# QuanjianSong/UniVST

Measured on AMD Instinct MI355X. Metric: stylized frames/sec, SD-v1.5 16x512x512 @50 DDIM steps, higher is better.
Workload: dtype f16; 1 GPU; sd15_unet_three_branch_pnp_transfer_16x512x512_50ddim; frames=16, branches=3, schedule_steps=53 (wrapping modulo 50), masks=moving disc, blended on steps 0..45, parallelism=single, weights=random-init SD-v1.5 architecture (859M + 201M temporal params), fp16

## Files before the change

### include/univst.h

```cpp
#ifndef UNIVST_H
#define UNIVST_H
#include <stdint.h>
#ifdef __cplusplus
extern "C" {
#endif

#define UNIVST_OK 0
#define UNIVST_ERR_ARG (-1)
#define UNIVST_ERR_HIP (-2)
#define UNIVST_ERR_UNSUPPORTED (-3)
#define UNIVST_ERR_STATE (-4)

#define UNIVST_F16 0
#define UNIVST_F32 1

const char* univst_last_error(void);
#define UNIVST_ABI_VERSION 3
int univst_abi_version(void);

typedef struct univst_unet univst_unet;

typedef struct {
    int in_channels, out_channels;
    int block_out_channels[4];
// ... 27 lines not shown
                                     int64_t off_recv_first, int64_t nbytes);
int univst_unet_set_comm(univst_unet* h, int rank, int world, void* comm_ws, int64_t comm_ws_bytes,
                         univst_allreduce_fn ar, univst_kv_exchange_fn kv, void* user);

typedef struct univst_comm univst_comm;
int univst_comm_create(int rank, int world, int64_t ws_bytes, univst_comm** out);
int univst_comm_handle_bytes(void);
int univst_comm_export(univst_comm* c, void* handle_out);
int univst_comm_connect(univst_comm* c, const void* handles);
int univst_comm_connect_local(univst_comm* c, univst_comm* const* all);
int univst_comm_connect_emulated(univst_comm* c, double link_gbps, double latency_us);
int univst_comm_query(univst_comm* c, const char* name, double* out);
int univst_comm_destroy(univst_comm* c);
int univst_comm_allreduce_f32(univst_comm* c, void* buf, int n, void* stream);
int univst_comm_status(univst_comm* c);
int univst_unet_set_comm_native(univst_unet* h, univst_comm* comm);

int univst_unet_set_option(univst_unet* h, const char* name, int value);
int univst_unet_query(univst_unet* h, const char* name, double* out);

typedef struct univst_vae univst_vae;
typedef struct {
    int in_channels, out_channels, latent_channels;
    int block_out_channels[4];
    int layers_per_block;
    int norm_num_groups;
} univst_vae_cfg;
int univst_vae_create(const univst_vae_cfg* cfg, univst_vae** out);
int univst_vae_destroy(univst_vae* h);
int univst_vae_load_tensor(univst_vae* h, const char* key, const void* dev_ptr, int dtype, const int64_t* shape, int ndim, void* stream);
int univst_vae_finalize(univst_vae* h, void* stream);
int univst_vae_decode(univst_vae* h, const void* z, int64_t imgs, int num_frames, int lat_h, int lat_w, void* out, void* stream);
int univst_vae_encode(univst_vae* h, const void* x, int64_t imgs, int H, int W, void* moments, void* stream);

typedef struct univst_klvae univst_klvae;
typedef struct {
    int in_channels, out_channels, latent_channels;
    int block_out_channels[4];
    int layers_per_block;
    int norm_num_groups;
    int use_quant_conv, use_post_quant_conv;
    int64_t attn_score_bytes, pass_bytes;
} univst_klvae_cfg;
int univst_klvae_create(const univst_klvae_cfg* cfg, univst_klvae** out);
int univst_klvae_destroy(univst_klvae* h);
int univst_klvae_load_tensor(univst_klvae* h, const char* key, const void* dev_ptr, int dtype, const int64_t* shape, int ndim, void* stream);
int univst_klvae_finalize(univst_klvae* h, void* stream);
int univst_klvae_decode(univst_klvae* h, const void* z, int64_t imgs, int lat_h, int lat_w, void* out, void* stream);
int univst_klvae_encode(univst_klvae* h, const void* x, int64_t imgs, int H, int W, void* moments, void* stream);
int univst_klvae_query(univst_klvae* h, const char* name, double* out);

typedef struct univst_raft univst_raft;
int univst_raft_create(univst_raft** out);
int univst_raft_destroy(univst_raft* h);
int univst_raft_load_tensor(univst_raft* h, const char* key, const void* dev_ptr, int dtype, const int64_t* shape, int ndim, void* stream);
int univst_raft_forward(univst_raft* h, const uint8_t* img1, const uint8_t* img2, int H, int W, float* flow, void* stream);
int univst_raft_encode(univst_raft* h, const uint8_t* img1, const uint8_t* img2, int H, int W, void* fmap, float* hidden, void* context, void* stream);
int univst_raft_gru(univst_raft* h, float* hidden, const void* context, const void* motion, int fh, int fw, void* stream);
int64_t univst_raft_pyramid_floats(int fh, int fw);
int univst_raft_corr_pyramid(const void* fmap1, const void* fmap2, int fh, int fw, float* pyramid, void* stream);
int univst_raft_corr_lookup(const float* pyramid, const float* coords, int fh, int fw, float* out_f32, void* out_f16, void* stream);
int univst_raft_convex_upsample(const float* flow, const void* mask, int fh, int fw, float* out, void* stream);

typedef struct univst_clip univst_clip;
typedef struct {
    int vocab_size;
    int hidden_size;
    int intermediate_size;
    int num_layers;
    int num_heads;
    int max_positions;
    int hidden_act;
    float layer_norm_eps;
    int projection_dim;
    int eos_token_id;
} univst_clip_cfg;
int univst_clip_create(const univst_clip_cfg* cfg, univst_clip** out);
int univst_clip_destroy(univst_clip* h);
int univst_clip_load_tensor(univst_clip* h, const char* key, const void* dev_ptr, int dtype, const int64_t* shape, int ndim, void* stream);
int univst_clip_finalize(univst_clip* h, void* stream);
int univst_clip_encode(univst_clip* h, const int64_t* ids, int B, int S, void* last_hidden, void* hidden_states, void* pooled, void* stream);
int univst_clip_query(univst_clip* h, const char* name, double* out);
int univst_clip_attention(const void* qkv, int B, int S, int heads, void* out, void* stream);

typedef struct univst_t5 univst_t5;
typedef struct {
    int vocab_size;
    int d_model;
    int d_ff;
    int num_layers;
    int num_heads;
    int d_kv;
    int num_buckets;
    int max_distance;
    float layer_norm_eps;
} univst_t5_cfg;
int univst_t5_create(const univst_t5_cfg* cfg, univst_t5** out);
int univst_t5_destroy(univst_t5* h);
int univst_t5_load_tensor(univst_t5* h, const char* key, const void* dev_ptr, int dtype, const int64_t* shape, int ndim, void* stream);
int univst_t5_finalize(univst_t5* h, void* stream);
int univst_t5_encode(univst_t5* h, const int64_t* ids, int B, int S, void* last_hidden, void* stream);
int univst_t5_query(univst_t5* h, const char* name, double* out);
int univst_t5_attention(const void* qkv, const float* bias_table, int B, int S, int heads, void* out, void* stream);
int univst_debug_t5_buckets(int num_buckets, int max_distance, int n, int* out);

typedef struct univst_motion univst_motion;
typedef struct {
    int channels;
    int num_heads;
    int num_blocks;
    int attn_per_block;
    int norm_groups;
    int max_len;
    int position_encoding;
    float gn_eps;
    float ln_eps;
} univst_motion_cfg;
int univst_motion_create(const univst_motion_cfg* cfg, univst_motion** out);
int univst_motion_destroy(univst_motion* h);
int univst_motion_load_tensor(univst_motion* h, const char* key, const void* dev_ptr, int dtype, const int64_t* shape, int ndim, void* stream);
int univst_motion_finalize(univst_motion* h, void* stream);
int univst_motion_forward(univst_motion* h, const void* X, void* Y, int B, int F, int N, void* stream);
int univst_motion_query(univst_motion* h, const char* name, double* out);
int univst_temporal_attention(const void* qkv, int64_t ldx, const void* pe_qkv, int B, int F, int N, int heads, int head_dim, void* out, int64_t ldo,
                              void* stream);

int univst_linear(const void* X, int64_t ldx, const void* W, const void* bias, const void* residual, int64_t ldr,
                  void* Y, int64_t ldy, int M, int N, int K, int geglu, void* stream);
int univst_geglu_xres_permute(const void* in, void* out, int rows, int cols, void* stream);
int univst_linear_gated(const void* X, int64_t ldx, const void* W, const void* bias, const void* residual, int64_t ldr, void* Y, int64_t ldy,
                        int M, int N, int K, int act, const void* gate, int64_t ld_gate, int rows_per_gate, void* stream);
int univst_linear_ln(const void* X, int64_t ldx, const void* W, const void* bias, const void* residual, int64_t ldr,
                     void* Y, int64_t ldy, int M, int N, int K, int geglu, const float* ln_stats, float ln_eps,
                     const float* ln_wsum, const float* ln_bias, float* stats_out, void* stream);
int64_t univst_attn2_fused_workspace_bytes(int B, int heads, int head_dim);
int univst_attn2_fused(const void* X, int64_t ldx, const float* ln_stats, float ln_eps, const float* ln_wsum, const float* ln_bias,
                       const void* Wq_frag, int q_prescaled, const void* kv, int B, int T, int64_t rows_per_branch, const void* Wo_frag,
                       const void* bias_o, const void* residual, int64_t ldr, void* Y, int64_t ldy, int64_t M, int C, int heads,
                       float* stats_out, void* workspace, void* stream);
int univst_attn12_fused(const void* attn_out, int64_t ldx, const void* Wp_frag, const void* bias_p, const void* residual_in, int64_t ldr_in, float ln_eps,
                        const float* ln_wsum, const float* ln_bias, const void* Wq_frag, int q_prescaled, const void* kv, int B, int T,
                        int64_t rows_per_branch, const void* Wo_frag, const void* bias_o, void* Y, int64_t ldy, int64_t M, int C, int heads,
                        float* stats_out, void* workspace, void* stream);
int univst_frag_pack(const void* W, void* out, int N, int K, void* stream);
int univst_conv_nhwc(const void* X1, const void* X2, int C1, int C2, int imgs, int Hs, int Ws, int upsample, int stride,
                     int taps, const void* W, const void* bias, const void* rowbias, int rows_per_rowbias,
                     const void* residual, void* Y, int Cout, void* stream);
int univst_conv_nhwc_tapinner(const void* X1, const void* X2, int C1, int C2, int imgs, int Hs, int Ws, int upsample, int stride,
                              const void* W, const void* bias, const void* rowbias, int rows_per_rowbias,
                              const void* residual, void* Y, int Cout, void* stream);
int univst_conv3x3_patch(const void* X1, const void* X2, int C1, int C2, int imgs, int Hs, int Ws, int upsample, const void* W32,
                         const void* bias, const void* rowbias, int rows_per_rowbias, const void* residual, void* Y, int Cout,
                         void* stream);
int univst_groupnorm_fold_linear(const void* X, int C, int64_t rows, int rows_per_stat, int groups, float eps, const void* gamma, const void* beta,
                                 const void* W, const void* bias, int N, void* W_sets, float* bias32, void* workspace, void* stream);
int univst_linear_sets(const void* X, int64_t ldx, const void* W_sets, const float* bias32, int rows_per_set, const void* residual, int64_t ldr,
                       void* Y, int64_t ldy, int M, int N, int K, float* stats_out, void* stream);
int64_t univst_groupnorm_workspace_bytes(int64_t rows, int rows_per_stat, int groups);
int univst_groupnorm_nhwc(const void* X1, const void* X2, int C1, int C2, int64_t rows, int rows_per_stat, int groups,
                          float eps, const void* gamma, const void* beta, int silu, void* Y, void* workspace,
                          void* stream);
int univst_layernorm(const void* X, void* Y, const void* gamma, const void* beta, int64_t rows, int C, float eps,
                     void* stream);
int univst_attention(const void* q, int64_t ldq, const void* k, const void* v, int64_t ldkv, void* out, int64_t ldo,
                     const int32_t* src_idx, const int32_t* src_cnt, const float* src_logw, int nsrc, int BF, int Nq, int Nkv,
                     int heads, int head_dim, int q_prescaled, void* stream);
int univst_attention_phase(const void* q, int64_t ldq, const void* k, const void* v, int64_t ldkv, void* out, int64_t ldo,
                           const int32_t* src_idx, const int32_t* src_cnt, const float* src_logw, int nsrc, int BF, int Nq, int Nkv,
                           int heads, int head_dim, int q_prescaled, float* state_out, const float* state_in, void* stream);
typedef struct {
    const void *to_q, *to_q_bias, *to_k, *to_k_bias, *to_v, *to_v_bias;
    const void *norm_q, *norm_k;
    const void *add_q, *add_q_bias, *add_k, *add_k_bias, *add_v, *add_v_bias;
    const void *norm_added_q, *norm_added_k;
    const void *to_out, *to_out_bias, *to_add_out, *to_add_out_bias;
} univst_sd3_attn_weights;
typedef struct {
    const void *res_img, *gate_img, *res_txt, *gate_txt;
    int64_t ld_gate_img, ld_gate_txt;
} univst_sd3_gated_residual;
int univst_sd3_shift_window(int idx, double eta1, double eta2, int* active, float* beta);
int univst_sd3_joint_attention(const univst_sd3_attn_weights* w, const void* hidden, const void* enc, int B, int N, int Nt, int Cin,
                               int heads, int head_dim, int clip_length, int shift, float beta, float rms_eps,
                               void* out_img, void* out_txt, const univst_sd3_gated_residual* gated_residual ,
                               univst_comm* comm , void* stream);
int univst_sd3_adain_shift(void* qkv, int64_t ld, int F, int N, int C, int heads, float alpha, float beta, float gamma, void* ws,
                           void* stream);
int univst_rmsnorm_heads(void* x, int64_t ld, int64_t rows, int heads, int head_dim, const void* weight, float eps, void* stream);
int univst_adaln_modulate(const void* x, void* y, const void* scale, const void* shift, int64_t ld_mod, int64_t rows, int64_t rows_per_batch,
                          int C, float eps, void* y2, const void* scale2, const void* shift2, void* stream);
int univst_gate_residual(const void* x, const void* gate, int64_t ld_gate, const void* y, void* out, int64_t rows, int64_t rows_per_batch, int C,
                         void* stream);
#define UNIVST_ACT_SILU 0
#define UNIVST_ACT_GELU_TANH 1
#define UNIVST_ACT_NONE (-1)
int univst_activation(const void* x, void* out, int64_t n, int act, void* stream);
int univst_timestep_embedding(const float* t, void* out, int B, int dim, int flip_sin_to_cos, float downscale_freq_shift, float max_period,
                              void* stream);
int univst_sd3_patchify(const void* latents, void* rows, int B, int C, int H, int W, int patch, void* stream);
int univst_sd3_unpatchify(const void* rows, void* latents, int B, int C, int H, int W, int patch, void* stream);
int univst_axpbypcz(const void* x, const void* y, const void* z, void* out, float a, float b, float c, int64_t n, void* stream);

int univst_attention_adain_shift(void* qkv, int64_t ld, int F, int N, int C, float alpha, float beta, float gamma,
                                 void* stats_ws, void* stream);
int univst_latent_adain(const void* cnt, const void* sty, void* out, int C, int F, int HW, void* stream);
int univst_latent_adain_stats(const void* cnt, float* stats2c, int C, int F, int HW, void* stream);
int univst_latent_adain_apply(const void* cnt, const void* sty, const float* stats2c, int64_t n_total, void* out, int C,
                              int F, int HW, void* stream);
int univst_axpby(const void* x, const void* eps, void* out, float cx, float ce, int64_t n, void* stream);
int univst_mask_blend(const void* a, const void* b, const void* m, void* out, int C, int64_t FHW, void* stream);
int univst_mask_resize(const uint8_t* mask, void* out, int F, int H, int W, int h, int w, void* stream);

int64_t univst_maskprop_workspace_bytes(int hw, int Nsrc, int C);
int univst_maskprop_frame(const float* feat_tar, const float* feat_src, const float* segs_src, float* segs_tar, int hw,
                          int Nsrc, int C, int ncls, float temperature, int topk, void* workspace, void* stream);
int univst_maskprop_finalize(const float* segs, uint8_t* mask_out, int ncls, int h, int w, int H, int W, void* workspace,
                             void* stream);

int univst_warp_accumulate(const uint8_t* key, const uint8_t* now, const float* fwd, const float* bwd, float* acc, int H,
                           int W, float threshold, void* stream);
int univst_warp_window_key(uint8_t* frames, const float* const* flows, int nn, int F, int H, int W, int key, int r, float threshold,
                           void* stream);
int univst_latent_window_smooth(void* x0, const float* lflow, int C, int F, int h, int w, int r, float thr, void* stream);
int univst_accumulate_u8(const uint8_t* frame, float* acc, int64_t n, void* stream);
int univst_window_store(const float* acc, float weight, uint8_t* dst, int64_t n, void* stream);

#define UNIVST_PROFILE_CLASSES 13
int univst_profile_enable(int on);
int univst_profile_collect(double* ms, int64_t* count, double* flops, double* bytes, int nclasses);
int univst_profile_collect_aux(double* aux_bytes, int nclasses);
int univst_profile_symbols(int cls, char* buf, int n);

int univst_debug_tr16(float* out256, void* stream);
int univst_debug_delay_us(double us, void* stream);

#define UNIVST_PLAN_BIAS 1
#define UNIVST_PLAN_RESIDUAL 2
#define UNIVST_PLAN_ROWBIAS 4
#define UNIVST_PLAN_LN_STATS 8
#define UNIVST_PLAN_STATS_OUT 16
#define UNIVST_PLAN_ACT 32
#define UNIVST_PLAN_GATE 64
#define UNIVST_PLAN_W32_ONLY 128
#define UNIVST_PLAN_W32 256
#define UNIVST_PLAN_GN_OUT 512
#define UNIVST_PLAN_TAPINNER 1024
#define UNIVST_PLAN_Y_UNALIGNED 2048
#define UNIVST_PLAN_WORKSPACE 4096
#define UNIVST_PLAN_GEOM_3X3 0
#define UNIVST_PLAN_GEOM_PAD_END 1
#define UNIVST_PLAN_GEOM_FRAME 2
int univst_debug_gemm_plan(int ncu, int mode, int M, int N, int K, int geglu, int flags, int rows_per_set, int C1, int C2, int Hs, int Ws, int upsample,
                           int stride, int taps, int geom, char* buf, int n);
#define UNIVST_PLAN_SRC_LOGW 1
#define UNIVST_PLAN_EXTRA_KEYS 2
int univst_debug_attention_plan(int BF, int heads, int Nq, int Nkv, int nsrc, int d, int q_prescaled, int flags, int phase, char* buf, int n);

#define UNIVST_GN_PLAN_INTS 16
int univst_debug_groupnorm_plan(int C1, int C2, int64_t rows, int rows_per_stat, int G, int has_fold, int world, int has_producer_stats, int* out_ints);

#ifdef __cplusplus
}
#endif
#endif
```

### univst_amd/_native.py

```python
import ctypes as C
import os
from typing import Optional

import torch

_LIB_PATH = os.environ.get("UNIVST_LIB") or os.path.join(os.path.dirname(os.path.abspath(__file__)), "lib", "libunivst_hip.so")
_lib = None


class UnetCfg(C.Structure):
    _fields_ = [("in_channels", C.c_int), ("out_channels", C.c_int), ("block_out_channels", C.c_int * 4),
                ("layers_per_block", C.c_int), ("cross_attention_dim", C.c_int), ("attention_heads", C.c_int * 4),
                ("norm_num_groups", C.c_int), ("norm_eps", C.c_float), ("flip_sin_to_cos", C.c_int),
                ("freq_shift", C.c_float)]


class ClipCfg(C.Structure):
    _fields_ = [("vocab_size", C.c_int), ("hidden_size", C.c_int), ("intermediate_size", C.c_int), ("num_layers", C.c_int), ("num_heads", C.c_int),
                ("max_positions", C.c_int), ("hidden_act", C.c_int), ("layer_norm_eps", C.c_float), ("projection_dim", C.c_int), ("eos_token_id", C.c_int)]


class T5Cfg(C.Structure):
    _fields_ = [("vocab_size", C.c_int), ("d_model", C.c_int), ("d_ff", C.c_int), ("num_layers", C.c_int), ("num_heads", C.c_int), ("d_kv", C.c_int),
                ("num_buckets", C.c_int), ("max_distance", C.c_int), ("layer_norm_eps", C.c_float)]


class MotionCfg(C.Structure):
    _fields_ = [("channels", C.c_int), ("num_heads", C.c_int), ("num_blocks", C.c_int), ("attn_per_block", C.c_int), ("norm_groups", C.c_int),
                ("max_len", C.c_int), ("position_encoding", C.c_int), ("gn_eps", C.c_float), ("ln_eps", C.c_float)]


class VaeCfg(C.Structure):
    _fields_ = [("in_channels", C.c_int), ("out_channels", C.c_int), ("latent_channels", C.c_int), ("block_out_channels", C.c_int * 4),
                ("layers_per_block", C.c_int), ("norm_num_groups", C.c_int)]


class KlVaeCfg(C.Structure):
    _fields_ = [("in_channels", C.c_int), ("out_channels", C.c_int), ("latent_channels", C.c_int), ("block_out_channels", C.c_int * 4),
                ("layers_per_block", C.c_int), ("norm_num_groups", C.c_int), ("use_quant_conv", C.c_int), ("use_post_quant_conv", C.c_int),
                ("attn_score_bytes", C.c_int64), ("pass_bytes", C.c_int64)]


class PnP(C.Structure):
    _fields_ = [("registered", C.c_int), ("idx", C.c_int), ("eta1", C.c_float), ("eta2", C.c_float),
                ("alpha", C.c_float), ("gamma", C.c_float)]


class Sd3AttnWeights(C.Structure):
    _NAMES = ("to_q", "to_q_bias", "to_k", "to_k_bias", "to_v", "to_v_bias", "norm_q", "norm_k", "add_q", "add_q_bias", "add_k", "add_k_bias",
              "add_v", "add_v_bias", "norm_added_q", "norm_added_k", "to_out", "to_out_bias", "to_add_out", "to_add_out_bias")
    _fields_ = [(n, C.c_void_p) for n in _NAMES]


class Sd3GatedResidual(C.Structure):
    _fields_ = [("res_img", C.c_void_p), ("gate_img", C.c_void_p), ("res_txt", C.c_void_p), ("gate_txt", C.c_void_p), ("ld_gate_img", C.c_int64),
                ("ld_gate_txt", C.c_int64)]


ALLREDUCE_FN = C.CFUNCTYPE(C.c_int, C.c_void_p, C.c_int64, C.c_int)
KVEXCHANGE_FN = C.CFUNCTYPE(C.c_int, C.c_void_p, C.c_int64, C.c_int64, C.c_int64, C.c_int64, C.c_int64)

_P, _I, _L, _F = C.c_void_p, C.c_int, C.c_int64, C.c_float
SIGNATURES = {
    "univst_last_error": (C.c_char_p, []),
    "univst_abi_version": (_I, []),
    "univst_sd3_shift_window": (_I, [_I, C.c_double, C.c_double, C.POINTER(_I), C.POINTER(_F)]),
    "univst_unet_create": (_I, [C.POINTER(UnetCfg), C.POINTER(_P)]),
    "univst_unet_destroy": (_I, [_P]),
    "univst_unet_load_tensor": (_I, [_P, C.c_char_p, _P, _I, C.POINTER(_L), _I, _P]),
    "univst_unet_finalize": (_I, [_P, _P]),
    "univst_unet_reserve": (_I, [_P, _I, _I, _I, _I]),
    "univst_unet_forward": (_I, [_P, _P, _F, _P, _I, _I, _I, _I, _I, C.POINTER(PnP), _P, _P, _I, _P]),
    "univst_unet_set_comm": (_I, [_P, _I, _I, _P, _L, ALLREDUCE_FN, KVEXCHANGE_FN, _P]),
    "univst_unet_set_option": (_I, [_P, C.c_char_p, _I]),
    "univst_unet_query": (_I, [_P, C.c_char_p, C.POINTER(C.c_double)]),
    "univst_comm_create": (_I, [_I, _I, _L, C.POINTER(_P)]),
    "univst_comm_handle_bytes": (_I, []),
    "univst_comm_export": (_I, [_P, _P]),
    "univst_comm_connect": (_I, [_P, _P]),
    "univst_comm_connect_local": (_I, [_P, C.POINTER(_P)]),
    "univst_comm_connect_emulated": (_I, [_P, C.c_double, C.c_double]),
    "univst_comm_query": (_I, [_P, C.c_char_p, C.POINTER(C.c_double)]),
    "univst_comm_destroy": (_I, [_P]),
    "univst_comm_allreduce_f32": (_I, [_P, _P, _I, _P]),
    "univst_comm_status": (_I, [_P]),
    "univst_unet_set_comm_native": (_I, [_P, _P]),
    "univst_linear": (_I, [_P, _L, _P, _P, _P, _L, _P, _L, _I, _I, _I, _I, _P]),
    "univst_linear_ln": (_I, [_P, _L, _P, _P, _P, _L, _P, _L, _I, _I, _I, _I, _P, _F, _P, _P, _P, _P]),
    "univst_geglu_xres_permute": (_I, [_P, _P, _I, _I, _P]),
    "univst_frag_pack": (_I, [_P, _P, _I, _I, _P]),
    "univst_vae_create": (_I, [_P, C.POINTER(_P)]),
    "univst_vae_destroy": (_I, [_P]),
    "univst_vae_load_tensor": (_I, [_P, C.c_char_p, _P, _I, C.POINTER(C.c_int64), _I, _P]),
    "univst_vae_finalize": (_I, [_P, _P]),
    "univst_vae_decode": (_I, [_P, _P, _L, _I, _I, _I, _P, _P]),
    "univst_vae_encode": (_I, [_P, _P, _L, _I, _I, _P, _P]),
    "univst_klvae_create": (_I, [_P, C.POINTER(_P)]),
    "univst_klvae_destroy": (_I, [_P]),
    "univst_klvae_load_tensor": (_I, [_P, C.c_char_p, _P, _I, C.POINTER(C.c_int64), _I, _P]),
    "univst_klvae_finalize": (_I, [_P, _P]),
    "univst_klvae_decode": (_I, [_P, _P, _L, _I, _I, _P, _P]),
    "univst_klvae_encode": (_I, [_P, _P, _L, _I, _I, _P, _P]),
    "univst_klvae_query": (_I, [_P, C.c_char_p, C.POINTER(C.c_double)]),
    "univst_clip_create": (_I, [_P, C.POINTER(_P)]),
    "univst_clip_destroy": (_I, [_P]),
    "univst_clip_load_tensor": (_I, [_P, C.c_char_p, _P, _I, C.POINTER(C.c_int64), _I, _P]),
    "univst_clip_finalize": (_I, [_P, _P]),
    "univst_clip_encode": (_I, [_P, _P, _I, _I, _P, _P, _P, _P]),
    "univst_clip_query": (_I, [_P, C.c_char_p, C.POINTER(C.c_double)]),
    "univst_clip_attention": (_I, [_P, _I, _I, _I, _P, _P]),
    "univst_t5_create": (_I, [_P, C.POINTER(_P)]),
    "univst_t5_destroy": (_I, [_P]),
    "univst_t5_load_tensor": (_I, [_P, C.c_char_p, _P, _I, C.POINTER(C.c_int64), _I, _P]),
    "univst_t5_finalize": (_I, [_P, _P]),
    "univst_t5_encode": (_I, [_P, _P, _I, _I, _P, _P]),
    "univst_t5_query": (_I, [_P, C.c_char_p, C.POINTER(C.c_double)]),
    "univst_motion_create": (_I, [_P, C.POINTER(_P)]),
    "univst_motion_destroy": (_I, [_P]),
    "univst_motion_load_tensor": (_I, [_P, C.c_char_p, _P, _I, C.POINTER(C.c_int64), _I, _P]),
    "univst_motion_finalize": (_I, [_P, _P]),
    "univst_motion_forward": (_I, [_P, _P, _P, _I, _I, _I, _P]),
    "univst_motion_query": (_I, [_P, C.c_char_p, C.POINTER(C.c_double)]),
    "univst_temporal_attention": (_I, [_P, C.c_int64, _P, _I, _I, _I, _I, _I, _P, C.c_int64, _P]),
    "univst_t5_attention": (_I, [_P, _P, _I, _I, _I, _P, _P]),
    "univst_debug_t5_buckets": (_I, [_I, _I, _I, C.POINTER(_I)]),
    "univst_raft_create": (_I, [C.POINTER(_P)]),
    "univst_raft_destroy": (_I, [_P]),
    "univst_raft_load_tensor": (_I, [_P, C.c_char_p, _P, _I, C.POINTER(C.c_int64), _I, _P]),
    "univst_raft_forward": (_I, [_P, _P, _P, _I, _I, _P, _P]),
    "univst_raft_encode": (_I, [_P, _P, _P, _I, _I, _P, _P, _P, _P]),
    "univst_raft_gru": (_I, [_P, _P, _P, _P, _I, _I, _P]),
    "univst_raft_pyramid_floats": (_L, [_I, _I]),
    "univst_raft_corr_pyramid": (_I, [_P, _P, _I, _I, _P, _P]),
    "univst_raft_corr_lookup": (_I, [_P, _P, _I, _I, _P, _P, _P]),
    "univst_raft_convex_upsample": (_I, [_P, _P, _I, _I, _P, _P]),
    "univst_attn2_fused_workspace_bytes": (_L, [_I, _I, _I]),
    "univst_attn12_fused": (_I, [_P, _L, _P, _P, _P, _L, _F, _P, _P, _P, _I, _P, _I, _I, _L, _P, _P, _P, _L, _L, _I, _I, _P, _P, _P]),
    "univst_attn2_fused": (_I, [_P, _L, _P, _F, _P, _P, _P, _I, _P, _I, _I, _L, _P, _P, _P, _L, _P, _L, _L, _I, _I, _P, _P, _P]),
    "univst_conv_nhwc": (_I, [_P, _P, _I, _I, _I, _I, _I, _I, _I, _I, _P, _P, _P, _I, _P, _P, _I, _P]),
    "univst_conv_nhwc_tapinner": (_I, [_P, _P, _I, _I, _I, _I, _I, _I, _I, _P, _P, _P, _I, _P, _P, _I, _P]),
    "univst_conv3x3_patch": (_I, [_P, _P, _I, _I, _I, _I, _I, _I, _P, _P, _P, _I, _P, _P, _I, _P]),
    "univst_groupnorm_fold_linear": (_I, [_P, _I, _L, _I, _I, _F, _P, _P, _P, _P, _I, _P, _P, _P, _P]),
    "univst_linear_sets": (_I, [_P, _L, _P, _P, _I, _P, _L, _P, _L, _I, _I, _I, _P, _P]),
    "univst_groupnorm_workspace_bytes": (_L, [_L, _I, _I]),
    "univst_groupnorm_nhwc": (_I, [_P, _P, _I, _I, _L, _I, _I, _F, _P, _P, _I, _P, _P, _P]),
    "univst_layernorm": (_I, [_P, _P, _P, _P, _L, _I, _F, _P]),
    "univst_attention": (_I, [_P, _L, _P, _P, _L, _P, _L, _P, _P, _P, _I, _I, _I, _I, _I, _I, _I, _P]),
    "univst_attention_phase": (_I, [_P, _L, _P, _P, _L, _P, _L, _P, _P, _P, _I, _I, _I, _I, _I, _I, _I, _P, _P, _P]),
    "univst_sd3_joint_attention": (_I, [C.POINTER(Sd3AttnWeights), _P, _P, _I, _I, _I, _I, _I, _I, _I, _I, _F, _F, _P, _P,
                                        C.POINTER(Sd3GatedResidual), _P, _P]),
    "univst_sd3_adain_shift": (_I, [_P, _L, _I, _I, _I, _I, _F, _F, _F, _P, _P]),
    "univst_rmsnorm_heads": (_I, [_P, _L, _L, _I, _I, _P, _F, _P]),
    "univst_linear_gated": (_I, [_P, _L, _P, _P, _P, _L, _P, _L, _I, _I, _I, _I, _P, _L, _I, _P]),
    "univst_adaln_modulate": (_I, [_P, _P, _P, _P, _L, _L, _L, _I, _F, _P, _P, _P, _P]),
    "univst_gate_residual": (_I, [_P, _P, _L, _P, _P, _L, _L, _I, _P]),
    "univst_activation": (_I, [_P, _P, _L, _I, _P]),
    "univst_timestep_embedding": (_I, [_P, _P, _I, _I, _I, _F, _F, _P]),
    "univst_sd3_patchify": (_I, [_P, _P, _I, _I, _I, _I, _I, _P]),
    "univst_sd3_unpatchify": (_I, [_P, _P, _I, _I, _I, _I, _I, _P]),
    "univst_axpbypcz": (_I, [_P, _P, _P, _P, _F, _F, _F, _L, _P]),
    "univst_attention_adain_shift": (_I, [_P, _L, _I, _I, _I, _F, _F, _F, _P, _P]),
    "univst_latent_adain": (_I, [_P, _P, _P, _I, _I, _I, _P]),
    "univst_latent_adain_stats": (_I, [_P, _P, _I, _I, _I, _P]),
    "univst_latent_adain_apply": (_I, [_P, _P, _P, _L, _P, _I, _I, _I, _P]),
    "univst_axpby": (_I, [_P, _P, _P, _F, _F, _L, _P]),
    "univst_mask_blend": (_I, [_P, _P, _P, _P, _I, _L, _P]),
    "univst_mask_resize": (_I, [_P, _P, _I, _I, _I, _I, _I, _P]),
    "univst_maskprop_workspace_bytes": (_L, [_I, _I, _I]),
    "univst_maskprop_frame": (_I, [_P, _P, _P, _P, _I, _I, _I, _I, _F, _I, _P, _P]),
    "univst_maskprop_finalize": (_I, [_P, _P, _I, _I, _I, _I, _I, _P, _P]),
    "univst_warp_accumulate": (_I, [_P, _P, _P, _P, _P, _I, _I, _F, _P]),
    "univst_warp_window_key": (_I, [_P, _P, _I, _I, _I, _I, _I, _I, _F, _P]),
    "univst_latent_window_smooth": (_I, [_P, _P, _I, _I, _I, _I, _I, _F, _P]),
    "univst_accumulate_u8": (_I, [_P, _P, _L, _P]),
    "univst_window_store": (_I, [_P, _F, _P, _L, _P]),
    "univst_debug_tr16": (_I, [_P, _P]),
    "univst_debug_delay_us": (_I, [C.c_double, _P]),
    "univst_debug_gemm_plan": (_I, [_I] * 16 + [C.c_char_p, _I]),
    "univst_debug_attention_plan": (_I, [_I] * 9 + [C.c_char_p, _I]),
    "univst_debug_groupnorm_plan": (_I, [_I, _I, _L, _I, _I, _I, _I, _I, _P]),
    "univst_profile_enable": (_I, [_I]),
    "univst_profile_symbols": (_I, [_I, C.c_char_p, _I]),
    "univst_profile_collect": (_I, [C.POINTER(C.c_double), C.POINTER(_L), C.POINTER(C.c_double), C.POINTER(C.c_double), _I]),
    "univst_profile_collect_aux": (_I, [C.POINTER(C.c_double), _I]),
}


ABI_VERSION = 3


def lib_path() -> str:
    return _LIB_PATH


def load():
    global _lib
    if _lib is None:
        if not os.path.exists(_LIB_PATH):
            raise RuntimeError(f"{_LIB_PATH} not found: build it with `python __graft_entry__.py build` (or `make`); "
                               "univst_amd has no CPU or eager-PyTorch fallback")
        lib = C.CDLL(_LIB_PATH)
        for name, (res, args) in SIGNATURES.items():
            fn = getattr(lib, name)
            fn.restype = res
            fn.argtypes = args
        if lib.univst_abi_version() != ABI_VERSION:
            raise RuntimeError(f"{_LIB_PATH} has ABI version {lib.univst_abi_version()}, this binding was written against {ABI_VERSION} "
                               "(include/univst.h UNIVST_ABI_VERSION): rebuild the library (`make`)")
        _lib = lib
    return _lib


def check(rc: int, what: str = ""):
    if rc != 0:
        msg = load().univst_last_error().decode(errors="replace")
        raise RuntimeError(f"libunivst_hip {what} failed (code {rc}): {msg}")


def stream_ptr() -> int:
    return torch.cuda.current_stream().cuda_stream


def ptr(t: Optional[torch.Tensor]):
    return None if t is None else t.data_ptr()


def _f16(t: torch.Tensor, name="tensor"):
    if not (t.is_cuda and t.dtype == torch.float16 and t.is_contiguous()):
        raise ValueError(f"{name}: expected a contiguous fp16 CUDA/HIP tensor, got {t.dtype} {t.device} "
                         f"contiguous={t.is_contiguous()}")
    return t


def temporal_attention(qkv, B, F, N, heads, head_dim, pe_qkv=None, out=None):
    Cw = heads * head_dim
    if out is None:
        out = torch.empty(qkv.shape[0], Cw, device=qkv.device, dtype=torch.float16)
    for name, t in (("qkv", qkv), ("out", out)):
        if not (t.is_cuda and t.dtype == torch.float16 and t.dim() == 2 and t.stride(1) == 1):
            raise ValueError(f"temporal_attention: {name} must be fp16 CUDA/HIP rows with contiguous columns, got {t.dtype} {t.device} strides {t.stride()}")
    if qkv.shape[0] < B * F * N or out.shape[0] < B * F * N:
        raise ValueError(f"temporal_attention: B*F*N = {B * F * N} rows, qkv has {qkv.shape[0]} and out {out.shape[0]}")
    if pe_qkv is not None:
        _f16(pe_qkv, "pe_qkv")
        if tuple(pe_qkv.shape) != (F, 3 * Cw):
            raise ValueError(f"temporal_attention: pe_qkv must be [F, 3*heads*head_dim] = [{F}, {3 * Cw}], got {tuple(pe_qkv.shape)}")
    check(load().univst_temporal_attention(ptr(qkv), qkv.stride(0), ptr(pe_qkv), B, F, N, heads, head_dim, ptr(out), out.stride(0), stream_ptr()),
          "temporal_attention")
    return out


def linear(x, w, bias=None, residual=None, geglu=False, out=None):
    _f16(x), _f16(w)
    M, K = x.shape
    N = w.shape[0]
    No = N // 2 if geglu else N
    if out is None:
        out = torch.empty(M, No, device=x.device, dtype=torch.float16)
    check(load().univst_linear(ptr(x), K, ptr(w), ptr(bias), ptr(residual), No, ptr(out), No, M, N, K, int(geglu),
                               stream_ptr()), "linear")
    return out


def linear_gated(x, w, bias=None, residual=None, act=None, gate=None, rows_per_gate=1, out=None):
    _f16(x), _f16(w)
    M, K = x.shape
    N = w.shape[0]
    if out is None:
        out = torch.empty(M, N, device=x.device, dtype=torch.float16)
    check(load().univst_linear_gated(ptr(x), K, ptr(w), ptr(bias), ptr(residual), N, ptr(out), N, M, N, K, -1 if act is None else act,
                                     ptr(gate), 0 if gate is None else _mod_ld(gate), rows_per_gate, stream_ptr()), "linear_gated")
    return out


def geglu_xres_permute(w):
    _f16(w)
    w = w.contiguous()
    out = torch.empty_like(w)
    check(load().univst_geglu_xres_permute(ptr(w), ptr(out), w.shape[0], 1 if w.dim() == 1 else w.shape[1], stream_ptr()), "geglu_xres_permute")
    return out


def frag_pack(w):
    _f16(w)
    w = w.contiguous()
    out = torch.empty_like(w)
    check(load().univst_frag_pack(ptr(w), ptr(out), w.shape[0], w.shape[1], stream_ptr()), "frag_pack")
    return out


def attn2_fused(x, wq_frag, kv, wo_frag, bias_o, rows_per_branch, heads, residual=None, ln=None, q_prescaled=False, stats_out=None, out=None,
                eps=1e-5):
    _f16(x), _f16(wq_frag), _f16(kv), _f16(wo_frag)
    M, C_ = x.shape
    B = -(-M // rows_per_branch)
    T = kv.shape[0] // B
    residual = x if residual is None else residual
    out = torch.empty(M, C_, device=x.device, dtype=torch.float16) if out is None else out
    st, ws, lb = ln if ln is not None else (None, None, None)
    for t in (st, ws, lb, stats_out):
        assert t is None or (t.dtype == torch.float32 and t.is_contiguous())
    wsb = torch.empty(max(int(load().univst_attn2_fused_workspace_bytes(B, heads, C_ // heads)), 16), device=x.device, dtype=torch.uint8)
    check(load().univst_attn2_fused(ptr(x), x.stride(0), ptr(st), eps, ptr(ws), ptr(lb), ptr(wq_frag), int(q_prescaled), ptr(kv), B, T,
                                    rows_per_branch, ptr(wo_frag), ptr(bias_o), ptr(residual), residual.stride(0), ptr(out), out.stride(0), M, C_,
                                    heads, ptr(stats_out), ptr(wsb), stream_ptr()), "attn2_fused")
    return out


def attn12_fused(attn_out, wp_frag, bias_p, residual_in, wq_frag, wsum, lnb, kv, wo_frag, bias_o, rows_per_branch, heads, q_prescaled=False, stats_out=None,
                 eps=1e-5):
    _f16(attn_out), _f16(wp_frag), _f16(residual_in), _f16(wq_frag), _f16(kv), _f16(wo_frag)
    M, C_ = attn_out.shape
    B = -(-M // rows_per_branch)
    T = kv.shape[0] // B
    out = torch.empty(M, C_, device=attn_out.device, dtype=torch.float16)
    wsb = torch.empty(max(int(load().univst_attn2_fused_workspace_bytes(B, heads, C_ // heads)), 16), device=attn_out.device, dtype=torch.uint8)
    check(load().univst_attn12_fused(ptr(attn_out), attn_out.stride(0), ptr(wp_frag), ptr(bias_p), ptr(residual_in), residual_in.stride(0), eps, ptr(wsum), ptr(lnb),
                                     ptr(wq_frag), int(q_prescaled), ptr(kv), B, T, rows_per_branch, ptr(wo_frag), ptr(bias_o), ptr(out), out.stride(0), M, C_, heads,
                                     ptr(stats_out), ptr(wsb), stream_ptr()), "attn12_fused")
    return out


def linear_ln(x, w, bias=None, residual=None, geglu=False, out=None, ln=None, stats_out=None, eps=1e-5):
    _f16(x), _f16(w)
    M, K = x.shape
    N = w.shape[0]
    No = N // 2 if geglu else N
    if out is None:
        out = torch.empty(M, No, device=x.device, dtype=torch.float16)
    st, ws, lb = ln if ln is not None else (None, None, None)
    for t in (st, ws, lb, stats_out):
        assert t is None or (t.dtype == torch.float32 and t.is_contiguous())
    check(load().univst_linear_ln(ptr(x), K, ptr(w), ptr(bias), ptr(residual), No, ptr(out), No, M, N, K, int(geglu), ptr(st), eps,
                                  ptr(ws), ptr(lb), ptr(stats_out), stream_ptr()), "linear_ln")
    return out


def conv_nhwc(x1, w, bias=None, x2=None, upsample=False, stride=1, rowbias=None, rows_per_rowbias=1, residual=None):
    _f16(x1), _f16(w)
    imgs, Hs, Ws, C1 = x1.shape
    C2 = 0 if x2 is None else x2.shape[-1]
    Cout, taps, _ = w.shape
    He, We = (Hs * 2, Ws * 2) if upsample else (Hs, Ws)
    Ho = (He - 1) // stride + 1 if taps == 9 else He
    Wo = (We - 1) // stride + 1 if taps == 9 else We
    out = torch.empty(imgs, Ho, Wo, Cout, device=x1.device, dtype=torch.float16)
    check(load().univst_conv_nhwc(ptr(x1), ptr(x2), C1, C2, imgs, Hs, Ws, int(upsample), stride, taps, ptr(w), ptr(bias),
                                  ptr(rowbias), rows_per_rowbias, ptr(residual), ptr(out), Cout, stream_ptr()), "conv_nhwc")
    return out


def conv_nhwc_tapinner(x1, w_ti, bias=None, x2=None, upsample=False, stride=1, rowbias=None, rows_per_rowbias=1, residual=None):
    _f16(x1), _f16(w_ti)
    imgs, Hs, Ws, C1 = x1.shape
    C2 = 0 if x2 is None else x2.shape[-1]
    Cout = w_ti.shape[0]
    He, We = (Hs * 2, Ws * 2) if upsample else (Hs, Ws)
    Ho, Wo = (He - 1) // stride + 1, (We - 1) // stride + 1
    out = torch.empty(imgs, Ho, Wo, Cout, device=x1.device, dtype=torch.float16)
    check(load().univst_conv_nhwc_tapinner(ptr(x1), ptr(x2), C1, C2, imgs, Hs, Ws, int(upsample), stride, ptr(w_ti), ptr(bias),
                                           ptr(rowbias), rows_per_rowbias, ptr(residual), ptr(out), Cout, stream_ptr()), "conv_tapinner")
    return out


def conv3x3_patch(x1, w_t32, bias=None, x2=None, rowbias=None, rows_per_rowbias=1, residual=None, upsample=False):
    _f16(x1), _f16(w_t32)
    imgs, Hs, Ws, C1 = x1.shape
    C2 = 0 if x2 is None else x2.shape[-1]
    Cout = w_t32.shape[0]
    He, We = (Hs * 2, Ws * 2) if upsample else (Hs, Ws)
    out = torch.empty(imgs, He, We, Cout, device=x1.device, dtype=torch.float16)
    check(load().univst_conv3x3_patch(ptr(x1), ptr(x2), C1, C2, imgs, Hs, Ws, int(upsample), ptr(w_t32), ptr(bias), ptr(rowbias), rows_per_rowbias,
                                      ptr(residual), ptr(out), Cout, stream_ptr()), "conv3x3_patch")
    return out


def groupnorm_fold_linear(x, gamma, beta, groups, eps, rows_per_stat, w, bias=None):
    _f16(x), _f16(w)
    rows, C_ = x.shape
    S, N = rows // rows_per_stat, w.shape[0]
    ws = torch.empty(max(1, load().univst_groupnorm_workspace_bytes(rows, rows_per_stat, groups) // 4), device=x.device, dtype=torch.float32)
    wsets = torch.empty(S, N, C_, device=x.device, dtype=torch.float16)
    b32 = torch.empty(S, N, device=x.device, dtype=torch.float32)
    check(load().univst_groupnorm_fold_linear(ptr(x), C_, rows, rows_per_stat, groups, eps, ptr(gamma), ptr(beta), ptr(w), ptr(bias), N, ptr(wsets), ptr(b32),
                                              ptr(ws), stream_ptr()), "groupnorm_fold_linear")
    return wsets, b32


def linear_sets(x, wsets, bias32, rows_per_set, residual=None, stats_out=None):
    _f16(x), _f16(wsets)
    M, K = x.shape
    N = wsets.shape[1]
    out = torch.empty(M, N, device=x.device, dtype=torch.float16)
    check(load().univst_linear_sets(ptr(x), K, ptr(wsets), ptr(bias32), rows_per_set, ptr(residual), N, ptr(out), N, M, N, K, ptr(stats_out), stream_ptr()), "linear_sets")
    return out


def groupnorm_nhwc(x1, gamma, beta, groups, eps, rows_per_stat, silu=False, x2=None):
    _f16(x1)
    C1 = x1.shape[-1]
    C2 = 0 if x2 is None else x2.shape[-1]
    rows = x1.numel() // C1
    ws = torch.empty(max(1, load().univst_groupnorm_workspace_bytes(rows, rows_per_stat, groups) // 4), device=x1.device,
                     dtype=torch.float32)
    out = torch.empty(*x1.shape[:-1], C1 + C2, device=x1.device, dtype=torch.float16)
    check(load().univst_groupnorm_nhwc(ptr(x1), ptr(x2), C1, C2, rows, rows_per_stat, groups, eps, ptr(gamma), ptr(beta),
                                       int(silu), ptr(out), ptr(ws), stream_ptr()), "groupnorm")
    return out


def layernorm(x, gamma, beta, eps=1e-5):
    _f16(x)
    C_ = x.shape[-1]
    out = torch.empty_like(x)
    check(load().univst_layernorm(ptr(x), ptr(out), ptr(gamma), ptr(beta), x.numel() // C_, C_, eps, stream_ptr()),
          "layernorm")
    return out


def attention(q, k, v, src_idx, heads, ldq=None, ldkv=None, Nq=None, Nkv=None, C_=None, src_cnt=None, src_logw=None, q_prescaled=False):
    BF, Nq_, Cq = q.shape
    C_ = C_ or Cq
    out = torch.empty(BF, Nq_, C_, device=q.device, dtype=torch.float16)
    check(load().univst_attention(ptr(q), ldq or q.stride(1), ptr(k), ptr(v), ldkv or k.stride(1), ptr(out), C_,
                                  ptr(src_idx), ptr(src_cnt), ptr(src_logw), src_idx.shape[1], BF, Nq_, Nkv or k.shape[1], heads, C_ // heads,
                                  int(bool(q_prescaled)), stream_ptr()), "attention")
    return out


def attention_phase(q, k, v, src_idx, src_cnt, heads, out=None, state_out=None, state_in=None, ldq=None, ldkv=None, Nq=None, Nkv=None, C_=None, src_logw=None,
                    q_prescaled=False):
    BF, Nq_, Cq = q.shape[0], (Nq or q.shape[1]), q.shape[2]
    C_ = C_ or Cq
    if out is None:
        out = torch.empty(BF, Nq_, C_, device=q.device, dtype=torch.float16)
    first = state_in is None
    if first and state_out is None:
        state_out = torch.empty(BF, heads, Nq_, 2, device=q.device, dtype=torch.float32)
    check(load().univst_attention_phase(ptr(q), ldq or q.stride(1), ptr(k), ptr(v), ldkv or k.stride(1), ptr(out), C_,
                                        ptr(src_idx), ptr(src_cnt), ptr(src_logw), src_idx.shape[1], BF, Nq_, Nkv or k.shape[1], heads, C_ // heads,
                                        int(bool(q_prescaled)), ptr(state_out) if first else None, None if first else ptr(state_in), stream_ptr()), "attention_phase")
    return (out, state_out) if first else out


_SD3_KEYS = {"to_q": "to_q.weight", "to_q_bias": "to_q.bias", "to_k": "to_k.weight", "to_k_bias": "to_k.bias", "to_v": "to_v.weight",
             "to_v_bias": "to_v.bias", "norm_q": "norm_q.weight", "norm_k": "norm_k.weight", "add_q": "add_q_proj.weight",
             "add_q_bias": "add_q_proj.bias", "add_k": "add_k_proj.weight", "add_k_bias": "add_k_proj.bias", "add_v": "add_v_proj.weight",
             "add_v_bias": "add_v_proj.bias", "norm_added_q": "norm_added_q.weight", "norm_added_k": "norm_added_k.weight",
             "to_out": "to_out.0.weight", "to_out_bias": "to_out.0.bias", "to_add_out": "to_add_out.weight", "to_add_out_bias": "to_add_out.bias"}


class Sd3AttnParams(dict):

    def __init__(self, state, device):
        super().__init__()
        t = {k: state[v].detach().to(device=device, dtype=torch.float16).contiguous() for k, v in _SD3_KEYS.items() if state.get(v) is not None}
        for trio in (("to_q", "to_k", "to_v"), ("add_q", "add_k", "add_v")):
            for suf in ("", "_bias"):
                names = [n + suf for n in trio]
                if all(n in t for n in names) and len({tuple(t[n].shape) for n in names}) == 1:
                    fused = torch.cat([t[n] for n in names]).contiguous()
                    rows = t[names[0]].shape[0]
                    for i, n in enumerate(names):
                        t[n] = fused[i * rows:(i + 1) * rows]
        self.update(t)


def sd3_joint_attention(params, hidden, enc, heads, clip_length=16, shift=False, idx=-1, eta1=0.0, eta2=0.6, rms_eps=1e-6, fuse=None, comm=None):
    _f16(hidden)
    B, N, Cin = hidden.shape
    keep = params if isinstance(params, Sd3AttnParams) else Sd3AttnParams(params, hidden.device)
    w = Sd3AttnWeights(**{k: (keep[k].data_ptr() if k in keep else None) for k in Sd3AttnWeights._NAMES})
    inner = keep["to_q"].shape[0]
    out_i = torch.empty_like(hidden)
    Nt = 0
    out_t = None
    if enc is not None:
        _f16(enc)
        Nt = enc.shape[1]
        out_t = torch.empty(B, Nt, Cin if "to_add_out" in keep else inner, device=hidden.device, dtype=torch.float16)
    gr = None
    if fuse is not None:
        gt = fuse.get("gate_txt")
        gr = Sd3GatedResidual(ptr(_f16(fuse["res_img"])), ptr(fuse["gate_img"]), ptr(fuse.get("res_txt")), ptr(gt), _mod_ld(fuse["gate_img"]),
                              0 if gt is None else _mod_ld(gt))
    active = bool(shift) and idx >= eta1 * 50 and idx <= eta2 * 50
    beta = ((0.9 - 0.1) / (eta1 * 50 - eta2 * 50) * (idx - eta2 * 50) + 0.1) if active else 0.0
    check(load().univst_sd3_joint_attention(C.byref(w), ptr(hidden), ptr(enc), B, N, Nt, Cin, heads, inner // heads, clip_length, int(active),
                                            float(beta), rms_eps, ptr(out_i), ptr(out_t), C.byref(gr) if gr is not None else None,
                                            comm, stream_ptr()), "sd3_joint_attention")
    return (out_i, out_t) if enc is not None else out_i


def sd3_adain_shift_(qkv, F, N, C_, heads, alpha, beta, gamma):
    _f16(qkv)
    ws = torch.empty(4 * F * 2 * C_ + 2 * F * 2 * heads, device=qkv.device, dtype=torch.float32)
    check(load().univst_sd3_adain_shift(ptr(qkv), qkv.shape[-1], F, N, C_, heads, alpha, beta, gamma, ptr(ws), stream_ptr()), "sd3_adain_shift")
    return qkv


def rmsnorm_heads_(x, heads, weight, eps=1e-6):
    _f16(x)
    rows, Cc = x.shape
    check(load().univst_rmsnorm_heads(ptr(x), x.stride(0), rows, heads, Cc // heads, ptr(weight), eps, stream_ptr()), "rmsnorm_heads")
    return x


def _mod_ld(*ts):
    ld = ts[0].stride(0)
    for t in ts:
        if not (t.is_cuda and t.dtype == torch.float16):
            raise ValueError(f"modulation operand: expected an fp16 CUDA/HIP tensor, got {t.dtype} {t.device}")
        if t.dim() != 2 or t.stride(1) != 1 or t.stride(0) != ld:
            raise ValueError("modulation operands must be [B, C] row views with a common row stride")
    return ld


def adaln_modulate(x, scale, shift, eps=1e-6, scale2=None, shift2=None):
    _f16(x)
    B, N, Cc = x.shape
    if not x.is_contiguous():
        raise ValueError("adaln_modulate: x must be contiguous")
    two = scale2 is not None
    ld = _mod_ld(scale, shift, *([scale2, shift2] if two else []))
    out = torch.empty_like(x)
    out2 = torch.empty_like(x) if two else None
    check(load().univst_adaln_modulate(ptr(x), ptr(out), ptr(scale), ptr(shift), ld, B * N, N, Cc, eps, ptr(out2), ptr(scale2), ptr(shift2),
                                       stream_ptr()), "adaln_modulate")
    return (out, out2) if two else out
# ... 136 lines not shown
```

### univst_amd/csrc/abi.hip

```cpp
#include <math.h>
#include <stdarg.h>
#include <stdlib.h>
#include <string.h>

#include <new>

#include "../../include/univst.h"
#include "comm.h"
#include "kernels.h"
#include "unet.h"
#include "vae.h"
#include "raft.h"
#include "clip.h"
#include "t5.h"
#include "motion.h"

static thread_local char g_err[1024] = "";
void uv_set_error(const char* fmt, ...) {
    va_list ap;
    va_start(ap, fmt);
    vsnprintf(g_err, sizeof(g_err), fmt, ap);
    va_end(ap);
}
const char* uv_get_error() { return g_err; }
// ... 418 lines not shown
    delete h;
    return UV_OK;
}
int univst_raft_load_tensor(univst_raft* h, const char* key, const void* p, int dtype, const int64_t* shape, int ndim, void* s) {
    UV_REQUIRE(h, "null handle");
    return h->impl.load_tensor(key, p, dtype, shape, ndim, S(s));
}
int univst_raft_forward(univst_raft* h, const uint8_t* img1, const uint8_t* img2, int Hh, int W, float* flow, void* s) {
    UV_REQUIRE(h && img1 && img2 && flow, "raft_forward: null argument");
    return h->impl.forward(img1, img2, Hh, W, flow, S(s));
}
int univst_raft_encode(univst_raft* h, const uint8_t* img1, const uint8_t* img2, int Hh, int W, void* fmap, float* hidden, void* context, void* s) {
    UV_REQUIRE(h && img1 && img2, "raft_encode: null argument");
    int rc = h->impl.encode(img1, img2, Hh, W, S(s));
    if (rc) return rc;
    const size_t N = (size_t)(Hh / 8) * (W / 8);
    if (fmap) UV_HIP(hipMemcpyAsync(fmap, h->impl.fmap, 2 * N * 256 * 2, hipMemcpyDeviceToDevice, S(s)));
    if (hidden) UV_HIP(hipMemcpyAsync(hidden, h->impl.h32, N * 128 * 4, hipMemcpyDeviceToDevice, S(s)));
    if (context) UV_HIP(hipMemcpyAsync(context, h->impl.ctx16, N * 128 * 2, hipMemcpyDeviceToDevice, S(s)));
    return UV_OK;
}
int univst_raft_gru(univst_raft* h, float* hidden, const void* context, const void* motion, int fh, int fw, void* s) {
    UV_REQUIRE(h && hidden && context && motion, "raft_gru: null argument");
    UV_REQUIRE(fh >= 16 && fw >= 16 && fh <= 512 && fw <= 512, "raft_gru: feature map %d x %d (at least 16 x 16)", fh, fw);
    if (!h->impl.finalized) {
        int rc = h->impl.finalize(S(s));
        if (rc) return rc;
    }
    int rc = h->impl.reserve(fh * 8, fw * 8);
    if (rc) return rc;
    return h->impl.gru(hidden, h->impl.h16, H(context), H(motion), fh, fw, S(s));
}
int64_t univst_raft_pyramid_floats(int fh, int fw) { return fh > 0 && fw > 0 ? uv_raft_pyramid_floats(fh, fw) : 0; }
int univst_raft_corr_pyramid(const void* f1, const void* f2, int fh, int fw, float* pyr, void* s) {
    UV_REQUIRE(f1 && f2 && pyr, "raft_corr_pyramid: null argument");
    return uv_raft_corr_pyramid(H(f1), H(f2), fh, fw, pyr, S(s));
}
int univst_raft_corr_lookup(const float* pyr, const float* coords, int fh, int fw, float* out32, void* out16, void* s) {
    UV_REQUIRE(pyr && coords, "raft_corr_lookup: null argument");
    return uv_raft_corr_lookup(pyr, coords, fh, fw, out32, HM(out16), S(s));
}
int univst_raft_convex_upsample(const float* flow, const void* mask, int fh, int fw, float* out, void* s) {
    UV_REQUIRE(flow && mask && out, "raft_convex_upsample: null argument");
    return uv_raft_convex_upsample(flow, 0, H(mask), fh, fw, out, S(s));
}
int univst_frag_pack(const void* W, void* out, int N, int K, void* s) {
    UV_REQUIRE(W && out, "frag_pack: null argument");
    return uv_launch_frag_pack(H(W), HM(out), N, K, S(s));
}
int64_t univst_attn2_fused_workspace_bytes(int B, int heads, int head_dim) { return uv_attn2_kvf_halfs(B, heads, head_dim) * (int64_t)sizeof(half_t); }
int univst_attn2_fused(const void* X, int64_t ldx, const float* ln_stats, float ln_eps, const float* ln_wsum, const float* ln_bias, const void* Wq_frag,
                       int q_prescaled, const void* kv, int B, int T, int64_t rows_per_branch, const void* Wo_frag, const void* bias_o,
                       const void* residual, int64_t ldr, void* Y, int64_t ldy, int64_t M, int C, int heads, float* stats_out, void* workspace,
                       void* s) {
    UV_REQUIRE(X && Wq_frag && kv && Wo_frag && residual && Y && workspace, "attn2_fused: null argument");
    UV_REQUIRE(B >= 1 && M >= 1 && M <= (int64_t)B * rows_per_branch && M < (1LL << 31) && C % 160 == 0 && heads > 0 && C % heads == 0,
               "attn2_fused: M=%lld rows exceed B=%d branches of %lld rows (or bad C / heads)", (long long)M, B, (long long)rows_per_branch);
    UV_REQUIRE(!ln_stats || (ln_wsum && ln_bias), "attn2_fused: a folded LayerNorm needs ln_wsum and ln_bias");
    UV_REQUIRE(uv_attn2_fused_ok(C, heads, (int)rows_per_branch, T), "attn2_fused: C=%d heads=%d rows_per_branch=%lld keys=%d is not a shape this kernel serves "
               "(C = 320, 8 heads, rows per branch a multiple of 64, <= 80 keys)", C, heads, (long long)rows_per_branch, T);
    int rc = uv_launch_kv_frag_pack(H(kv), HM(workspace), B, T, C, heads, S(s));
    if (rc) return rc;
    Attn2Params p;
    p.X = H(X); p.ldx = ldx; p.M = (int)M;
    p.ln_stats = ln_stats; p.ln_slots = C / 160; p.ln_eps = ln_eps; p.ln_wsum = ln_wsum; p.ln_bias = ln_bias;
    p.Wq_f = H(Wq_frag); p.kvf = H(workspace);
    p.rows_per_branch = (int)rows_per_branch; p.heads = heads; p.Nkv = T;
    p.q_prescaled = q_prescaled; p.scale_log2e = 1.4426950408889634f / sqrtf((float)(C / heads));
    p.Wo_f = H(Wo_frag); p.bias_o = H(bias_o);
    p.R = H(residual); p.ldr = ldr;
    p.Y = HM(Y); p.ldy = ldy;
    p.stats_out = stats_out;
    return uv_launch_attn2_fused(p, C, S(s));
}
int univst_attn12_fused(const void* attn_out, int64_t ldx, const void* Wp_frag, const void* bias_p, const void* residual_in, int64_t ldr_in, float ln_eps,
                        const float* ln_wsum, const float* ln_bias, const void* Wq_frag, int q_prescaled, const void* kv, int B, int T, int64_t rows_per_branch,
                        const void* Wo_frag, const void* bias_o, void* Y, int64_t ldy, int64_t M, int C, int heads, float* stats_out, void* workspace, void* s) {
    UV_REQUIRE(attn_out && Wp_frag && residual_in && ln_wsum && ln_bias && Wq_frag && kv && Wo_frag && Y && workspace, "attn12_fused: null argument");
    UV_REQUIRE(B >= 1 && M >= 1 && M <= (int64_t)B * rows_per_branch && M < (1LL << 31) && heads > 0 && C % heads == 0, "attn12_fused: M=%lld rows exceed B=%d branches of %lld rows",
               (long long)M, B, (long long)rows_per_branch);
    UV_REQUIRE(uv_attn2_fused_ok(C, heads, (int)rows_per_branch, T), "attn12_fused: C=%d heads=%d rows_per_branch=%lld keys=%d is not a shape this kernel serves "
               "(C = 320, 8 heads, rows per branch a multiple of 64, <= 80 keys)", C, heads, (long long)rows_per_branch, T);
    int rc = uv_launch_kv_frag_pack(H(kv), HM(workspace), B, T, C, heads, S(s));
    if (rc) return rc;
    Attn2Params p;
    p.X = H(attn_out); p.ldx = ldx; p.M = (int)M;
    p.Wp_f = H(Wp_frag); p.bias_p = H(bias_p); p.Rp = H(residual_in); p.ldrp = ldr_in;
    p.ln_slots = C / 160; p.ln_eps = ln_eps; p.ln_wsum = ln_wsum; p.ln_bias = ln_bias;
    p.Wq_f = H(Wq_frag); p.kvf = H(workspace);
    p.rows_per_branch = (int)rows_per_branch; p.heads = heads; p.Nkv = T;
    p.q_prescaled = q_prescaled; p.scale_log2e = 1.4426950408889634f / sqrtf((float)(C / heads));
    p.Wo_f = H(Wo_frag); p.bias_o = H(bias_o);
    p.Y = HM(Y); p.ldy = ldy;
    p.stats_out = stats_out;
    return uv_launch_attn2_fused(p, C, S(s));
}
int univst_linear_ln(const void* X, int64_t ldx, const void* W, const void* bias, const void* R, int64_t ldr, void* Y, int64_t ldy,
                     int M, int N, int K, int geglu, const float* ln_stats, float ln_eps, const float* ln_wsum, const float* ln_bias,
                     float* stats_out, void* s) {
    UV_REQUIRE(X && W && Y, "linear_ln: null argument");
    UV_REQUIRE(!ln_stats || (ln_wsum && ln_bias && K % 160 == 0 && !bias), "linear_ln: a folded LayerNorm needs wsum, lnb (which holds the bias) and K %% 160 == 0");
    UV_REQUIRE((!stats_out || uv_linear_fold_producer_ok(M, N, K)) && (!ln_stats || geglu == 2 || uv_linear_fold_consumer_ok(M, N, K, geglu != 0)),
               "linear_ln: M=%d N=%d K=%d is not taken by the direct 256x320 path (N %% 320 == 0 and >= 150 tiles) nor by the 128-wide path without split-K", M, N, K);
    GemmParams g;
    g.X = H(X); g.ldx = ldx; g.W = H(W); g.bias = H(bias); g.R = H(R); g.ldr = ldr; g.Y = HM(Y); g.ldy = ldy;
    g.M = M; g.N = N; g.K = K; g.geglu = geglu;
    g.ln_stats = ln_stats; g.ln_slots = K / 160; g.ln_eps = ln_eps; g.ln_wsum = ln_wsum; g.ln_bias = ln_bias; g.stats_out = stats_out;
    return uv_launch_gemm(g, 0, S(s));
}
int univst_conv_nhwc(const void* X1, const void* X2, int C1, int C2, int imgs, int Hs, int Ws, int up, int stride, int taps,
                     const void* W, const void* bias, const void* rowbias, int rows_per_rb, const void* R, void* Y, int Cout,
                     void* s) {
    UV_REQUIRE(X1 && W && Y, "conv: null argument");
    UV_REQUIRE((X2 != nullptr) == (C2 > 0), "conv: X2/C2 mismatch");
    UV_REQUIRE(stride == 1 || stride == 2, "conv: stride %d", stride);
    GemmParams g;
    g.X = H(X1); g.X2 = H(X2); g.C1 = C1; g.C2 = C2; g.Hs = Hs; g.Ws = Ws; g.up = up ? 1 : 0; g.stride = stride; g.taps = taps;
    const int He = Hs << g.up, We = Ws << g.up;
    g.Ho = taps == 9 ? (He - 1) / stride + 1 : He;
    g.Wo = taps == 9 ? (We - 1) / stride + 1 : We;
    g.M = imgs * g.Ho * g.Wo; g.N = Cout; g.K = taps * (C1 + C2);
    g.W = H(W); g.bias = H(bias); g.rowbias = H(rowbias); g.rows_per_rb = rows_per_rb > 0 ? rows_per_rb : 1;
    g.R = H(R); g.ldr = Cout; g.Y = HM(Y); g.ldy = Cout;
    return uv_launch_gemm(g, 1, S(s));
}
int univst_conv_nhwc_tapinner(const void* X1, const void* X2, int C1, int C2, int imgs, int Hs, int Ws, int up, int stride,
                              const void* W, const void* bias, const void* rowbias, int rows_per_rb, const void* R, void* Y, int Cout,
                              void* s) {
    UV_REQUIRE(X1 && W && Y, "conv: null argument");
    UV_REQUIRE((X2 != nullptr) == (C2 > 0), "conv: X2/C2 mismatch");
    GemmParams g;
    g.X = H(X1); g.X2 = H(X2); g.C1 = C1; g.C2 = C2; g.Hs = Hs; g.Ws = Ws; g.up = up ? 1 : 0; g.stride = stride; g.taps = 9; g.korder = 1;
    const int He = Hs << g.up, We = Ws << g.up;
    g.Ho = (He - 1) / stride + 1;
    g.Wo = (We - 1) / stride + 1;
    g.M = imgs * g.Ho * g.Wo; g.N = Cout; g.K = 9 * (C1 + C2);
    g.W = H(W); g.bias = H(bias); g.rowbias = H(rowbias); g.rows_per_rb = rows_per_rb > 0 ? rows_per_rb : 1;
    g.R = H(R); g.ldr = Cout; g.Y = HM(Y); g.ldy = Cout;
    return uv_launch_gemm(g, 1, S(s));
}
int univst_conv3x3_patch(const void* X1, const void* X2, int C1, int C2, int imgs, int Hs, int Ws, int upsample, const void* W32,
                         const void* bias, const void* rowbias, int rows_per_rb, const void* R, void* Y, int Cout, void* s) {
    UV_REQUIRE(X1 && W32 && Y, "conv3x3_patch: null argument");
    UV_REQUIRE((X2 != nullptr) == (C2 > 0), "conv3x3_patch: X2/C2 mismatch");
    GemmParams g;
    g.X = H(X1); g.X2 = H(X2); g.C1 = C1; g.C2 = C2; g.Hs = Hs; g.Ws = Ws; g.up = upsample ? 1 : 0; g.stride = 1; g.taps = 9;
    g.Ho = Hs << g.up; g.Wo = Ws << g.up;
    g.M = imgs * g.Ho * g.Wo; g.N = Cout; g.K = 9 * (C1 + C2);
    g.W = nullptr; g.W32 = H(W32);
    g.bias = H(bias); g.rowbias = H(rowbias); g.rows_per_rb = rows_per_rb > 0 ? rows_per_rb : 1;
    g.R = H(R); g.ldr = Cout; g.Y = HM(Y); g.ldy = Cout;
    return uv_launch_gemm(g, 1, S(s));
}
int univst_groupnorm_fold_linear(const void* X, int C, int64_t rows, int rows_per_stat, int groups, float eps, const void* gamma, const void* beta,
                                 const void* W, const void* bias, int N, void* W_sets, float* bias32, void* ws, void* s) {
    UV_REQUIRE(X && gamma && beta && W && W_sets && bias32 && ws && N > 0, "groupnorm_fold_linear: null argument");
    UvGnFold f;
    f.W = H(W); f.bias = H(bias); f.N = N; f.W_out = HM(W_sets); f.bias32 = bias32;
    return uv_launch_groupnorm(H(X), nullptr, C, 0, rows, rows_per_stat, groups, eps, H(gamma), H(beta), 0, nullptr, (float*)ws, S(s), nullptr, nullptr, nullptr, &f);
}
int univst_linear_sets(const void* X, int64_t ldx, const void* W_sets, const float* bias32, int rows_per_set, const void* R, int64_t ldr, void* Y, int64_t ldy,
                       int M, int N, int K, float* stats_out, void* s) {
    UV_REQUIRE(X && W_sets && bias32 && Y && rows_per_set > 0, "linear_sets: null argument");
    GemmParams g;
    g.X = H(X); g.ldx = ldx; g.W = H(W_sets); g.bias32 = bias32; g.w_rows_per_set = rows_per_set;
    g.R = H(R); g.ldr = ldr; g.Y = HM(Y); g.ldy = ldy; g.M = M; g.N = N; g.K = K; g.stats_out = stats_out;
    UV_REQUIRE(uv_linear_takes_big_direct(M, N, K, ldx), "linear_sets: M=%d N=%d K=%d is not a problem the direct 256x320 path takes (N %% 320 == 0, >= 150 tiles)", M, N, K);
    return uv_launch_gemm(g, 0, S(s));
}
int64_t univst_groupnorm_workspace_bytes(int64_t rows, int rows_per_stat, int groups) {
    if (rows_per_stat <= 0) return 0;
    return (int64_t)uv_groupnorm_workspace_floats((int)(rows / rows_per_stat), groups) * 4;
}
int univst_groupnorm_nhwc(const void* X1, const void* X2, int C1, int C2, int64_t rows, int rows_per_stat, int groups, float eps,
                          const void* gamma, const void* beta, int silu, void* Y, void* ws, void* s) {
    UV_REQUIRE(X1 && gamma && beta && Y && ws, "groupnorm: null argument");
    return uv_launch_groupnorm(H(X1), H(X2), C1, C2, rows, rows_per_stat, groups, eps, H(gamma), H(beta), silu, HM(Y), (float*)ws,
                               S(s));
}
int univst_layernorm(const void* X, void* Y, const void* gamma, const void* beta, int64_t rows, int C, float eps, void* s) {
    UV_REQUIRE(X && Y && gamma && beta, "layernorm: null argument");
    return uv_launch_layernorm(H(X), C, HM(Y), C, H(gamma), H(beta), rows, C, eps, S(s));
}
int univst_attention(const void* q, int64_t ldq, const void* k, const void* v, int64_t ldkv, void* out, int64_t ldo,
                     const int32_t* src_idx, const int32_t* src_cnt, const float* src_logw, int nsrc, int BF, int Nq, int Nkv, int heads,
                     int d, int q_prescaled, void* s) {
    UV_REQUIRE(q && k && v && out && src_idx, "attention: null argument");
    AttnParams a;
    a.src_cnt = src_cnt;
    a.src_logw = src_logw;
    a.q = H(q); a.k = H(k); a.v = H(v); a.o = HM(out); a.ldq = ldq; a.ldkv = ldkv; a.ldo = ldo; a.src_idx = src_idx; a.nsrc = nsrc;
    a.BF = BF; a.Nq = Nq; a.Nkv = Nkv; a.heads = heads; a.d = d;
    a.scale_log2e = 1.4426950408889634f / sqrtf((float)d);
    a.q_prescaled = q_prescaled != 0;
    return uv_launch_attention(a, S(s));
}
int univst_attention_phase(const void* q, int64_t ldq, const void* k, const void* v, int64_t ldkv, void* out, int64_t ldo,
                           const int32_t* src_idx, const int32_t* src_cnt, const float* src_logw, int nsrc, int BF, int Nq, int Nkv, int heads,
                           int d, int q_prescaled, float* state_out, const float* state_in, void* s) {
    UV_REQUIRE(q && k && v && out && src_idx && src_cnt, "attention_phase: null argument (src_cnt is required: a phase may leave a frame without sources)");
    UV_REQUIRE((state_out != nullptr) != (state_in != nullptr), "attention_phase: exactly one of state_out (first phase) / state_in (second phase)");
    AttnParams a;
    a.src_cnt = src_cnt;
    a.src_logw = src_logw;
    a.q = H(q); a.k = H(k); a.v = H(v); a.o = HM(out); a.ldq = ldq; a.ldkv = ldkv; a.ldo = ldo; a.src_idx = src_idx; a.nsrc = nsrc;
    a.BF = BF; a.Nq = Nq; a.Nkv = Nkv; a.heads = heads; a.d = d;
    a.scale_log2e = 1.4426950408889634f / sqrtf((float)d);
    a.q_prescaled = q_prescaled != 0;
    a.state_out = state_out;
    a.state_in = state_in;
    return uv_launch_attention(a, S(s));
}
int univst_attention_adain_shift(void* qkv, int64_t ld, int F, int N, int C, float alpha, float beta, float gamma, void* ws, void* s) {
    UV_REQUIRE(qkv && ws, "adain_shift: null argument");
    float* w = (float*)ws;
    return uv_launch_adain_shift(HM(qkv), ld, F, N, C, w, w + (long)F * 2 * C, alpha, beta, gamma, S(s));
}
int univst_latent_adain(const void* cnt, const void* sty, void* out, int C, int F, int HW, void* s) {
    UV_REQUIRE(cnt && sty && out, "latent_adain: null argument");
    return uv_launch_latent_adain(H(cnt), H(sty), HM(out), C, F, HW, S(s));
}
int univst_latent_adain_stats(const void* cnt, float* stats, int C, int F, int HW, void* s) {
    UV_REQUIRE(cnt && stats, "latent_adain_stats: null argument");
    return uv_launch_latent_adain_stats(H(cnt), stats, C, F, HW, S(s));
}
int univst_latent_adain_apply(const void* cnt, const void* sty, const float* stats, int64_t n_total, void* out, int C, int F, int HW,
                              void* s) {
    UV_REQUIRE(cnt && sty && stats && out && n_total > 0, "latent_adain_apply: bad argument");
    return uv_launch_latent_adain_apply(H(cnt), H(sty), stats, n_total, HM(out), C, F, HW, S(s));
}
int univst_axpby(const void* x, const void* e, void* out, float cx, float ce, int64_t n, void* s) {
    UV_REQUIRE(x && e && out, "axpby: null argument");
    return uv_launch_axpby(H(x), H(e), HM(out), cx, ce, n, S(s));
}
int univst_mask_blend(const void* a, const void* b, const void* m, void* out, int C, int64_t FHW, void* s) {
    UV_REQUIRE(a && b && out, "mask_blend: null argument");
    return uv_launch_mask_blend(H(a), H(b), H(m), HM(out), C, FHW, S(s));
}
int univst_mask_resize(const uint8_t* mask, void* out, int F, int Hh, int W, int h, int w, void* s) {
    UV_REQUIRE(mask && out, "mask_resize: null argument");
    return uv_launch_mask_resize(mask, HM(out), F, Hh, W, h, w, S(s));
}
int univst_debug_tr16(float* out, void* s) { return uv_launch_tr16_probe(out, S(s)); }
int univst_debug_delay_us(double us, void* s) { return uv_launch_delay_us(us, S(s)); }
int univst_debug_gemm_plan(int ncu, int mode, int M, int N, int K, int geglu, int flags, int rows_per_set, int C1, int C2, int Hs, int Ws, int upsample,
                           int stride, int taps, int geom, char* buf, int n) {
    UV_REQUIRE(buf && n > 0 && ncu > 0, "debug_gemm_plan: null buffer or ncu <= 0");
    if (M == 0 && N == 0) {
        snprintf(buf, (size_t)n, "%s", uv_gemm_plan_symbols().c_str());
        return UV_OK;
    }
    alignas(16) static float arena[8];
    half_t* const h = (half_t*)arena;
    auto on = [&](int bit) { return (flags & bit) != 0; };
    GemmParams g;
    g.X = h; g.Y = on(UNIVST_PLAN_Y_UNALIGNED) ? h + 4 : h;
    g.W = on(UNIVST_PLAN_W32_ONLY) ? nullptr : h;
    g.W32 = on(UNIVST_PLAN_W32_ONLY) || on(UNIVST_PLAN_W32) ? h : nullptr;
    g.N = N; g.geglu = geglu;
    const int No = geglu ? N / 2 : N;
    if (mode == 0) {
        g.M = M; g.K = K; g.ldx = K;
    } else {
        g.C1 = C1; g.C2 = C2; g.X2 = C2 ? h : nullptr; g.Hs = Hs; g.Ws = Ws; g.up = upsample ? 1 : 0; g.stride = stride; g.taps = taps;
        const int He = Hs << g.up, We = Ws << g.up;
        if (geom == UNIVST_PLAN_GEOM_FRAME) {
            g.tapw = 1; g.pady = 1; g.padx = 0; g.Ho = He; g.Wo = We;
        } else if (geom == UNIVST_PLAN_GEOM_PAD_END) {
            g.tapw = 3; g.pady = g.padx = 0; g.Ho = (He + 1 - 3) / stride + 1; g.Wo = (We + 1 - 3) / stride + 1;
        } else {
            g.Ho = (He - 1) / stride + 1; g.Wo = (We - 1) / stride + 1;
        }
        g.M = M * g.Ho * g.Wo; g.K = taps * (C1 + C2);
        g.korder = on(UNIVST_PLAN_TAPINNER) ? 1 : 0;
    }
    g.ldy = No; g.ldr = No;
    if (on(UNIVST_PLAN_BIAS)) g.bias = h;
    if (on(UNIVST_PLAN_RESIDUAL)) g.R = h;
    if (on(UNIVST_PLAN_ROWBIAS)) g.rowbias = h;
    if (on(UNIVST_PLAN_LN_STATS)) { g.ln_stats = arena; g.ln_wsum = arena; g.ln_bias = arena; g.ln_slots = g.K / 160; }
    if (on(UNIVST_PLAN_STATS_OUT)) g.stats_out = arena;
    if (on(UNIVST_PLAN_ACT)) g.act = 1;
    if (on(UNIVST_PLAN_GATE)) { g.gate = h; g.ld_gate = N; }
    if (on(UNIVST_PLAN_GN_OUT)) { g.gn_out = arena; g.gn_gw = 10; g.gn_G = N / 10; }
    if (on(UNIVST_PLAN_WORKSPACE)) { g.partial = arena; g.partial_bytes = UV_SPLITK_WS_BYTES; }
    if (rows_per_set > 0) { g.w_rows_per_set = rows_per_set; g.bias32 = arena; }
    return uv_gemm_plan_text(g, mode, ncu, buf, n);
}
int univst_debug_attention_plan(int BF, int heads, int Nq, int Nkv, int nsrc, int d, int q_prescaled, int flags, int phase, char* buf, int n) {
    UV_REQUIRE(buf && n > 0 && phase >= 0 && phase <= 2, "debug_attention_plan: null buffer or phase outside 0..2");
    if (Nq == 0 && Nkv == 0) {
        snprintf(buf, (size_t)n, "%s", uv_attention_plan_symbols().c_str());
        return UV_OK;
    }
    alignas(16) static float arena[8];
    half_t* const h = (half_t*)arena;
    AttnParams a;
    a.q = a.k = a.v = h; a.o = h; a.ldq = a.ldkv = a.ldo = (long)heads * d; a.src_idx = (const int*)arena;
    a.nsrc = nsrc; a.BF = BF; a.Nq = Nq; a.Nkv = Nkv; a.heads = heads; a.d = d; a.q_prescaled = q_prescaled != 0;
    if (flags & UNIVST_PLAN_SRC_LOGW) a.src_logw = arena;
    if (flags & UNIVST_PLAN_EXTRA_KEYS) { a.kx = a.vx = h; a.x_idx = (const int*)arena; a.ldkv_x = a.ldkv; a.Nkv_x = 77; }
    if (phase == 1) a.state_out = arena;
    if (phase == 2) a.state_in = arena;
    return uv_attention_plan_text(a, buf, n);
}
int univst_debug_groupnorm_plan(int C1, int C2, int64_t rows, int rows_per_stat, int G, int has_fold, int world, int has_producer_stats, int* out_ints) {
    UV_REQUIRE(out_ints, "debug_groupnorm_plan: null output");
    const GnPlan pl = uv_groupnorm_plan(C1, C2, rows, rows_per_stat, G, has_fold, world, has_producer_stats != 0);
    if (pl.rc != UV_OK) {
        uv_set_error("%s", pl.err);
        return pl.rc;
    }
    const int v[UNIVST_GN_PLAN_INTS] = {pl.route, pl.fold, pl.sharded, pl.block, pl.TR, pl.nchunk, pl.rpc, pl.nblk, pl.rpb, pl.lds_stats, pl.lds_tail,
                                        (int)pl.stats_grid[0], (int)pl.stats_grid[1], (int)pl.reduce_grid, (int)pl.tail_grid[0], (int)pl.tail_grid[1]};
    for (int i = 0; i < UNIVST_GN_PLAN_INTS; ++i) out_ints[i] = v[i];
    return UV_OK;
}
int univst_profile_enable(int on) {
    uv_prof_enable(on);
    return UV_OK;
}
int univst_profile_symbols(int cls, char* buf, int n) {
    UV_REQUIRE(buf && n > 0, "profile_symbols: null buffer");
    const std::string sy = uv_prof_symbols(cls);
    snprintf(buf, (size_t)n, "%s", sy.c_str());
    return UV_OK;
}
int univst_profile_collect(double* ms, int64_t* count, double* flops, double* bytes, int ncls) {
    UV_REQUIRE(ms && count && flops && bytes && ncls >= 1 && ncls <= 16, "profile_collect: bad arguments");
    long c[16];
    int rc = uv_prof_collect(ms, c, flops, bytes, ncls);
    for (int i = 0; i < ncls; ++i) count[i] = c[i];
    return rc;
}

int univst_profile_collect_aux(double* aux_bytes, int ncls) {
    UV_REQUIRE(aux_bytes && ncls >= 1 && ncls <= 16, "profile_collect_aux: bad arguments");
    uv_prof_aux(aux_bytes, ncls);
    return UV_OK;
}

int64_t univst_maskprop_workspace_bytes(int hw, int Nsrc, int C) { return uv_maskprop_workspace_bytes(hw, Nsrc, C); }
int univst_maskprop_frame(const float* feat_tar, const float* feat_src, const float* segs_src, float* segs_tar, int hw, int Nsrc,
                          int C, int ncls, float T, int topk, void* ws, void* s) {
    UV_REQUIRE(feat_tar && feat_src && segs_src && segs_tar && ws, "maskprop_frame: null argument");
    return uv_launch_maskprop_frame(feat_tar, feat_src, segs_src, segs_tar, hw, Nsrc, C, ncls, T, topk, ws, S(s));
}
int univst_maskprop_finalize(const float* segs, uint8_t* out, int ncls, int h, int w, int Hh, int W, void* ws, void* s) {
    UV_REQUIRE(segs && out && ws, "maskprop_finalize: null argument");
    return uv_launch_maskprop_finalize(segs, out, ncls, h, w, Hh, W, ws, S(s));
}
int univst_warp_accumulate(const uint8_t* key, const uint8_t* now, const float* fwd, const float* bwd, float* acc, int Hh, int W,
                           float thr, void* s) {
    UV_REQUIRE(key && now && fwd && bwd && acc, "warp_accumulate: null argument");
    return uv_launch_warp_accumulate(key, now, fwd, bwd, acc, Hh, W, thr, S(s));
}
int univst_warp_window_key(uint8_t* frames, const float* const* flows, int nn, int F, int Hh, int W, int key, int r, float thr, void* s) {
    UV_REQUIRE(frames, "warp_window_key: null argument");
    return uv_launch_warp_window_key(frames, flows, nn, F, Hh, W, key, r, thr, S(s));
}
int univst_latent_window_smooth(void* x0, const float* lflow, int C, int F, int h, int w, int r, float thr, void* s) {
    UV_REQUIRE(x0 && lflow, "latent_window_smooth: null argument");
    return uv_launch_latent_window_smooth(HM(x0), lflow, C, F, h, w, r, thr, S(s));
}
int univst_accumulate_u8(const uint8_t* f, float* acc, int64_t n, void* s) {
    UV_REQUIRE(f && acc, "accumulate_u8: null argument");
    return uv_launch_accumulate_u8(f, acc, n, S(s));
}
int univst_window_store(const float* acc, float weight, uint8_t* dst, int64_t n, void* s) {
    UV_REQUIRE(acc && dst && weight > 0.f, "window_store: bad argument");
    return uv_launch_window_store(acc, weight, dst, n, S(s));
}

}
```

### univst_amd/csrc/gemm.hip

```cpp
#include <string.h>

#include "common.h"
#include "kernels.h"

namespace {

__device__ __attribute__((aligned(256))) half_t uv_zero_page[128];

constexpr int EPC_LNB = 320, EPC_HALFS = 640, EPC_ROWST = 960, EPC_TOTAL = 960 + 512;
template <int LNF>
__device__ __forceinline__ void epi_const_stage(const GemmParams& p, int m0, int n0, int bmb, int tid, float* epc) {
    half_t* hb = reinterpret_cast<half_t*>(epc + EPC_HALFS);
    if (tid < 320) {
        const int n = n0 + tid;
        const bool ok = n < p.N;
        hb[tid] = (p.bias && ok) ? p.bias[n] : (half_t)0.f;
        hb[320 + tid] = (p.bias2 && ok) ? p.bias2[n] : (half_t)0.f;
        if (LNF != 2) epc[EPC_LNB + tid] = (p.bias32 && ok) ? p.bias32[(long)(p.w_rows_per_set ? m0 / p.w_rows_per_set : 0) * p.N + n] : 0.f;
        if (LNF == 2) {
            epc[tid] = ok ? p.ln_wsum[n] : 0.f;
            epc[EPC_LNB + tid] = ok ? p.ln_bias[n] : 0.f;
        }
    }
    if (LNF == 2 && tid < bmb) {
// ... 24 lines not shown
#pragma unroll
            for (int i = 0; i < NF; i += 2) {
                const int nx = nb + i * 16 + g * 4;
                const int ng = nx + 16;
                if (ng >= p.N) continue;
                const int no = nb / 2 + (i / 2) * 16 + g * 4;
                h4 o, bx = {0, 0, 0, 0}, bg = {0, 0, 0, 0};
                if (LNF == 2) {
                    const float* cc = cf + cn + i * 16 + g * 4;
                    const f4 wx = *reinterpret_cast<const f4*>(cc), wg = *reinterpret_cast<const f4*>(cc + 16);
                    const f4 cx = *reinterpret_cast<const f4*>(cc + EPC_LNB), cg = *reinterpret_cast<const f4*>(cc + EPC_LNB + 16);
                    float xv[4], gv[4];
#pragma unroll
                    for (int r = 0; r < 4; ++r) {
                        xv[r] = fmaf(ln.y, fmaf(-ln.x, wx[r], col[i][r]), cx[r]);
                        gv[r] = fmaf(ln.y, fmaf(-ln.x, wg[r], col[i + 1][r]), cg[r]);
                    }
#pragma unroll
                    for (int r = 0; r < 4; r += 2) {
                        const f2 y = geglu_erf2(f2{xv[r], xv[r + 1]}, f2{gv[r], gv[r + 1]});
                        o[r] = (half_t)y.x;
                        o[r + 1] = (half_t)y.y;
                    }
                    *reinterpret_cast<h4*>(p.Y + (long)m * p.ldy + no) = o;
                    continue;
                }
                if (p.bias) {
                    if constexpr (CL) {
                        bx = *reinterpret_cast<const h4*>(hb + i * 16 + g * 4);
                        bg = *reinterpret_cast<const h4*>(hb + i * 16 + g * 4 + 16);
                    } else {
                        bx = *reinterpret_cast<const h4*>(p.bias + nx);
                        bg = *reinterpret_cast<const h4*>(p.bias + ng);
                    }
                }
#pragma unroll
                for (int r = 0; r < 4; r += 2) {
                    const f2 y = geglu_erf2(f2{col[i][r] + (float)bx[r], col[i][r + 1] + (float)bx[r + 1]},
                                            f2{col[i + 1][r] + (float)bg[r], col[i + 1][r + 1] + (float)bg[r + 1]});
                    o[r] = (half_t)y.x;
                    o[r + 1] = (half_t)y.y;
                }
                *reinterpret_cast<h4*>(p.Y + (long)m * p.ldy + no) = o;
            }
        }
        return;
    }
    h4 hres[NF];
#pragma unroll
    for (int i = 0; i < NF; ++i) {
        const int n = nb + i * 16 + g * 4;
        hres[i] = (p.R && n + 3 < p.N) ? *reinterpret_cast<const h4*>(p.R + (long)m * p.ldr + n) : h4{0, 0, 0, 0};
    }
#pragma unroll
    for (int i = 0; i < NF; ++i) {
        const int n = nb + i * 16 + g * 4;
        if (n >= p.N) continue;
        float v[4];
#pragma unroll
        for (int r = 0; r < 4; ++r) v[r] = col[i][r];
        if (n + 3 < p.N) {
            if (LNF == 2) {
                f4 ws, cb;
                if constexpr (CL) {
                    ws = *reinterpret_cast<const f4*>(cf + cn + i * 16 + g * 4);
                    cb = *reinterpret_cast<const f4*>(cf + EPC_LNB + cn + i * 16 + g * 4);
                } else {
                    ws = *reinterpret_cast<const f4*>(p.ln_wsum + n);
                    cb = *reinterpret_cast<const f4*>(p.ln_bias + n);
                }
#pragma unroll
                for (int r = 0; r < 4; ++r) v[r] = fmaf(ln.y, fmaf(-ln.x, ws[r], v[r]), cb[r]);
            }
            if (p.bias) {
                h4 bv;
                if constexpr (CL) bv = *reinterpret_cast<const h4*>(hb + i * 16 + g * 4);
                else bv = *reinterpret_cast<const h4*>(p.bias + n);
#pragma unroll
                for (int r = 0; r < 4; ++r) v[r] += (float)bv[r];
            }
            if (rbias) {
                h4 bv = *reinterpret_cast<const h4*>(rbias + n);
#pragma unroll
                for (int r = 0; r < 4; ++r) v[r] += (float)bv[r];
            }
            if constexpr (LNF == 3) {
                if (p.act) {
#pragma unroll
                    for (int r = 0; r < 4; ++r) v[r] = gelu_tanh_f(v[r]);
                }
                if (p.gate) {
                    const h4 gv = *reinterpret_cast<const h4*>(p.gate + (long)(m / p.rows_per_gate) * p.ld_gate + n);
#pragma unroll
                    for (int r = 0; r < 4; ++r) v[r] *= (float)gv[r];
                }
            }
            if (p.R) {
                const h4 rv = hres[i];
#pragma unroll
                for (int r = 0; r < 4; ++r) v[r] += (float)rv[r];
            }
            h4 o;
            if (p.bias2) {
                h4 bv;
                if constexpr (CL) bv = *reinterpret_cast<const h4*>(hb + 320 + i * 16 + g * 4);
                else bv = *reinterpret_cast<const h4*>(p.bias2 + n);
#pragma unroll
                for (int r = 0; r < 4; ++r) o[r] = (half_t)((float)(half_t)v[r] + (float)bv[r]);
            } else {
#pragma unroll
                for (int r = 0; r < 4; ++r) o[r] = (half_t)v[r];
            }
            if constexpr (LNF == 1 && !CL) {
                if (st) {
#pragma unroll
                    for (int r = 0; r < 4; ++r) {
                        const float t = (float)o[r];
                        st->x += t;
                        st->y = fmaf(t, t, st->y);
                    }
                }
            }
            *reinterpret_cast<h4*>(p.Y + (long)m * p.ldy + n) = o;
        } else {
            for (int r = 0; r < 4 && n + r < p.N; ++r) {
                float t = v[r];
                if (p.bias) t += (float)p.bias[n + r];
                if (rbias) t += (float)rbias[n + r];
                if constexpr (LNF == 3) {
                    if (p.act) t = gelu_tanh_f(t);
                    if (p.gate) t *= (float)p.gate[(long)(m / p.rows_per_gate) * p.ld_gate + n + r];
                }
                if (p.R) t += (float)p.R[(long)m * p.ldr + n + r];
                half_t o = (half_t)t;
                if (p.bias2) o = (half_t)((float)o + (float)p.bias2[n + r]);
                p.Y[(long)m * p.ldy + n + r] = o;
            }
        }
    }
}

typedef __fp16 fh2 __attribute__((ext_vector_type(2)));
__device__ __forceinline__ float row16_sum(float v) {
#define UV_ROW_SHR_ADD(n) v += __builtin_bit_cast(float, __builtin_amdgcn_update_dpp(0, __builtin_bit_cast(int, v), 0x110 + (n), 0xf, 0xf, true))
    UV_ROW_SHR_ADD(1);
    UV_ROW_SHR_ADD(2);
    UV_ROW_SHR_ADD(4);
    UV_ROW_SHR_ADD(8);
#undef UV_ROW_SHR_ADD
    return v;
}
constexpr int EPI_LDW = 164;
constexpr int EPI_STAT_SCRATCH = 90112;
template <int MJ, int LNF = 0>
__device__ __forceinline__ void gemm_epilogue_lds(const GemmParams& p, const f4 (&acc)[10][MJ], float* slab, int mw, int nb, int lane,
                                                  const float* cf, int cn, int rw = 0, float2* scratch = nullptr, half_t* hs = nullptr) {
    const int l15 = lane & 15, g = lane >> 4;
    const half_t* hb = reinterpret_cast<const half_t*>(cf + EPC_HALFS) + cn;
#pragma unroll
    for (int j = 0; j < MJ; ++j) {
#pragma unroll
        for (int i = 0; i < 10; ++i) *reinterpret_cast<f4*>(&slab[l15 * EPI_LDW + i * 16 + g * 4]) = acc[i][j];
        __builtin_amdgcn_fence(__ATOMIC_RELEASE, "wavefront");
        __builtin_amdgcn_wave_barrier();
        const int mrow0 = mw + j * 16;
        if (!p.geglu) {
            h8 rres[5];
            const bool hoist_rb = !p.R && p.rowbias;
            if (p.R || hoist_rb) {
#pragma unroll
                for (int it = 0; it < 5; ++it) {
                    const int id = it * 64 + lane;
                    const int row = id / 20, c = (id - row * 20) * 8;
                    const int m = mrow0 + row < p.M ? mrow0 + row : p.M - 1;
                    const half_t* src = p.R ? p.R + (long)m * p.ldr : p.rowbias + (long)(m / p.rows_per_rb) * (p.ldrb ? p.ldrb : p.N);
                    rres[it] = nb + c < p.N ? *reinterpret_cast<const h8*>(src + nb + c) : h8{0, 0, 0, 0, 0, 0, 0, 0};
                }
            }
#pragma unroll
            for (int it = 0; it < 5; ++it) {
                const int id = it * 64 + lane;
                const int row = id / 20, c = (id - row * 20) * 8;
                const int m = mrow0 + row, n = nb + c;
                const f4 v0 = *reinterpret_cast<const f4*>(&slab[row * EPI_LDW + c]);
                const f4 v1 = *reinterpret_cast<const f4*>(&slab[row * EPI_LDW + c + 4]);
                if (m >= p.M || n >= p.N) continue;
                float v[8] = {v0[0], v0[1], v0[2], v0[3], v1[0], v1[1], v1[2], v1[3]};
                if (LNF == 2) {
                    const float2 ln = reinterpret_cast<const float2*>(cf + EPC_ROWST)[rw + j * 16 + row];
                    const f4 w0 = *reinterpret_cast<const f4*>(cf + cn + c), w1 = *reinterpret_cast<const f4*>(cf + cn + c + 4);
                    const f4 c0 = *reinterpret_cast<const f4*>(cf + EPC_LNB + cn + c), c1 = *reinterpret_cast<const f4*>(cf + EPC_LNB + cn + c + 4);
                    const float ws[8] = {w0[0], w0[1], w0[2], w0[3], w1[0], w1[1], w1[2], w1[3]};
                    const float cb[8] = {c0[0], c0[1], c0[2], c0[3], c1[0], c1[1], c1[2], c1[3]};
#pragma unroll
                    for (int r = 0; r < 8; ++r) v[r] = fmaf(ln.y, fmaf(-ln.x, ws[r], v[r]), cb[r]);
                }
                if (p.bias) {
                    const h8 bv = *reinterpret_cast<const h8*>(hb + c);
#pragma unroll
                    for (int r = 0; r < 8; ++r) v[r] += (float)bv[r];
                }
                if (LNF != 2 && p.bias32) {
                    const f4 b0 = *reinterpret_cast<const f4*>(cf + EPC_LNB + cn + c), b1 = *reinterpret_cast<const f4*>(cf + EPC_LNB + cn + c + 4);
                    v[0] += b0[0]; v[1] += b0[1]; v[2] += b0[2]; v[3] += b0[3];
                    v[4] += b1[0]; v[5] += b1[1]; v[6] += b1[2]; v[7] += b1[3];
                }
                if (p.rowbias) {
                    const h8 bv = hoist_rb ? rres[it] : *reinterpret_cast<const h8*>(p.rowbias + (long)(m / p.rows_per_rb) * (p.ldrb ? p.ldrb : p.N) + n);
#pragma unroll
                    for (int r = 0; r < 8; ++r) v[r] += (float)bv[r];
                }
                if constexpr (LNF == 3) {
                    if (p.act) {
#pragma unroll
                        for (int r = 0; r < 8; ++r) v[r] = gelu_tanh_f(v[r]);
                    }
                    if (p.gate) {
                        const h8 gv = *reinterpret_cast<const h8*>(p.gate + (long)(m / p.rows_per_gate) * p.ld_gate + n);
#pragma unroll
                        for (int r = 0; r < 8; ++r) v[r] *= (float)gv[r];
                    }
                }
                if (p.R) {
                    const h8 rv = rres[it];
#pragma unroll
                    for (int r = 0; r < 8; ++r) v[r] += (float)rv[r];
                }
                h8 o;
                if (p.bias2) {
                    const h8 bv = *reinterpret_cast<const h8*>(hb + 320 + c);
#pragma unroll
                    for (int r = 0; r < 8; ++r) o[r] = (half_t)((float)(half_t)v[r] + (float)bv[r]);
                } else {
#pragma unroll
                    for (int r = 0; r < 8; ++r) o[r] = (half_t)v[r];
                }
                *reinterpret_cast<h8*>(p.Y + (long)m * p.ldy + n) = o;
                if (LNF != 1 && p.gn_out) *reinterpret_cast<h8*>(&hs[row * 160 + c]) = o;
                if (LNF == 1) {
                    float s1 = 0.f, s2 = 0.f;
#pragma unroll
                    for (int r = 0; r < 8; ++r) {
                        const float t = (float)o[r];
                        s1 += t;
                        s2 = fmaf(t, t, s2);
                    }
                    scratch[id] = float2{s1, s2};
                }
            }
            if (LNF == 1) {
                __builtin_amdgcn_fence(__ATOMIC_RELEASE, "wavefront");
                __builtin_amdgcn_wave_barrier();
                const int row = lane >> 2, q = lane & 3;
                float s1 = 0.f, s2 = 0.f;
#pragma unroll
                for (int e = 0; e < 5; ++e) {
                    const float2 t = scratch[row * 20 + q * 5 + e];
                    s1 += t.x;
                    s2 += t.y;
                }
                s1 += __shfl_xor(s1, 1, 64);
                s2 += __shfl_xor(s2, 1, 64);
                s1 += __shfl_xor(s1, 2, 64);
                s2 += __shfl_xor(s2, 2, 64);
                const int m = mrow0 + row;
                if (q == 0 && m < p.M) *reinterpret_cast<float2*>(p.stats_out + ((long)m * (p.N / 160) + nb / 160) * 2) = float2{s1, s2};
            }
            if (LNF != 1 && p.gn_out) {
                __builtin_amdgcn_fence(__ATOMIC_RELEASE, "wavefront");
                __builtin_amdgcn_wave_barrier();
                __builtin_amdgcn_fence(__ATOMIC_ACQUIRE, "wavefront");
                const fh2 one2 = {(__fp16)1.f, (__fp16)1.f};
                union { fh2 h[20]; h8 v[5]; } u;
#pragma unroll
                for (int e = 0; e < 5; ++e) u.v[e] = *reinterpret_cast<const h8*>(&hs[l15 * 160 + g * 40 + e * 8]);
                float a1[4] = {0.f, 0.f, 0.f, 0.f}, a2[4] = {0.f, 0.f, 0.f, 0.f};
                const int hp = p.gn_gw >> 1;
#pragma unroll
                for (int k = 0; k < 20; ++k) {
                    const int gi = hp == 5 ? k / 5 : (hp == 10 ? k / 10 : 0);
                    a1[gi] = __builtin_amdgcn_fdot2(u.h[k], one2, a1[gi], false);
                    a2[gi] = __builtin_amdgcn_fdot2(u.h[k], u.h[k], a2[gi], false);
                }
                const int ngpl = 20 / hp;
#pragma unroll
                for (int gi = 0; gi < 4; ++gi) {
                    if (gi < ngpl) {
                        a1[gi] = row16_sum(a1[gi]);
                        a2[gi] = row16_sum(a2[gi]);
                    }
                }
                if (l15 == 15 && mrow0 < p.M) {
                    float2* dst = reinterpret_cast<float2*>(p.gn_out) + (long)(nb / p.gn_gw + g * ngpl) * (p.M >> 4) + (mrow0 >> 4);
#pragma unroll
                    for (int gi = 0; gi < 4; ++gi)
                        if (gi < ngpl) dst[(long)gi * (p.M >> 4)] = float2{a1[gi], a2[gi]};
                }
            }
        } else {
#pragma unroll
            for (int it = 0; it < 3; ++it) {
                const int id = it * 64 + lane;
                if (id >= 160) continue;
                const int row = id / 10, cq = id - row * 10;
                const int cx = (cq >> 1) * 32 + (cq & 1) * 8;
                const int m = mrow0 + row;
                if (m >= p.M) continue;
                const float* sr = &slab[row * EPI_LDW + cx];
                const f4 x0 = *reinterpret_cast<const f4*>(sr), x1 = *reinterpret_cast<const f4*>(sr + 4);
                const f4 g0 = *reinterpret_cast<const f4*>(sr + 16), g1 = *reinterpret_cast<const f4*>(sr + 20);
                float xv[8] = {x0[0], x0[1], x0[2], x0[3], x1[0], x1[1], x1[2], x1[3]};
                float gv[8] = {g0[0], g0[1], g0[2], g0[3], g1[0], g1[1], g1[2], g1[3]};
                if (p.bias) {
                    const h8 bx = *reinterpret_cast<const h8*>(hb + cx);
                    const h8 bg = *reinterpret_cast<const h8*>(hb + cx + 16);
#pragma unroll
                    for (int r = 0; r < 8; ++r) { xv[r] += (float)bx[r]; gv[r] += (float)bg[r]; }
                }
                h8 o;
#pragma unroll
                for (int r = 0; r < 8; r += 2) {
                    const f2 y = geglu_erf2(f2{xv[r], xv[r + 1]}, f2{gv[r], gv[r + 1]});
                    o[r] = (half_t)y.x;
                    o[r + 1] = (half_t)y.y;
                }
                *reinterpret_cast<h8*>(p.Y + (long)m * p.ldy + nb / 2 + cq * 8) = o;
            }
        }
        __builtin_amdgcn_fence(__ATOMIC_ACQUIRE, "wavefront");
        __builtin_amdgcn_wave_barrier();
    }
}


constexpr int GEGLU_SLD = 88;
template <int MJ, int LNF>
__device__ __forceinline__ void gemm_epilogue_geglu_slab(const GemmParams& p, const f4 (&acc)[10][MJ], half_t* slab, int mw, int nb, int lane,
                                                         const float* cf, int cn, int rw) {
    const int l15 = lane & 15, g = lane >> 4;
    const half_t* hb = reinterpret_cast<const half_t*>(cf + EPC_HALFS) + cn;
#pragma unroll
    for (int j = 0; j < MJ; ++j) {
        float2 ln = float2{0.f, 1.f};
        if (LNF == 2) ln = reinterpret_cast<const float2*>(cf + EPC_ROWST)[rw + j * 16 + l15];
#pragma unroll
        for (int i = 0; i < 10; i += 2) {
            float xv[4], gv[4];
            if (LNF == 2) {
                const float* cc = cf + cn + i * 16 + g * 4;
                const f4 wx = *reinterpret_cast<const f4*>(cc), wg = *reinterpret_cast<const f4*>(cc + 16);
                const f4 cx = *reinterpret_cast<const f4*>(cc + EPC_LNB), cg = *reinterpret_cast<const f4*>(cc + EPC_LNB + 16);
#pragma unroll
                for (int r = 0; r < 4; ++r) {
                    xv[r] = fmaf(ln.y, fmaf(-ln.x, wx[r], acc[i][j][r]), cx[r]);
                    gv[r] = fmaf(ln.y, fmaf(-ln.x, wg[r], acc[i + 1][j][r]), cg[r]);
                }
            } else {
                const h4 bx = *reinterpret_cast<const h4*>(hb + i * 16 + g * 4);
                const h4 bg = *reinterpret_cast<const h4*>(hb + i * 16 + g * 4 + 16);
#pragma unroll
                for (int r = 0; r < 4; ++r) {
                    xv[r] = acc[i][j][r] + (float)bx[r];
                    gv[r] = acc[i + 1][j][r] + (float)bg[r];
                }
            }
            h4 o;
#ifdef UV_GEGLU_X1
#pragma unroll
            for (int r = 0; r < 4; r += 2) {
                const f2 y = geglu_erf2(f2{xv[r], xv[r + 1]}, f2{gv[r], gv[r + 1]});
                o[r] = (half_t)y.x;
                o[r + 1] = (half_t)y.y;
            }
#else
            f2 y0, y1;
            geglu_erf2x2(f2{xv[0], xv[1]}, f2{gv[0], gv[1]}, f2{xv[2], xv[3]}, f2{gv[2], gv[3]}, y0, y1);
            o[0] = (half_t)y0.x; o[1] = (half_t)y0.y; o[2] = (half_t)y1.x; o[3] = (half_t)y1.y;
#endif
            *reinterpret_cast<h4*>(&slab[(j * 16 + l15) * GEGLU_SLD + (i / 2) * 16 + g * 4]) = o;
        }
    }
    __builtin_amdgcn_fence(__ATOMIC_RELEASE, "wavefront");
    __builtin_amdgcn_wave_barrier();
    __builtin_amdgcn_fence(__ATOMIC_ACQUIRE, "wavefront");
    constexpr int NCH = MJ * 16 * 10;
#pragma unroll
    for (int it = 0; it < (NCH + 63) / 64; ++it) {
        const int id = it * 64 + lane;
        if (id >= NCH) continue;
        const int row = id / 10, c = id - row * 10;
        const int m = mw + row, n = nb / 2 + c * 8;
        const h8 v = *reinterpret_cast<const h8*>(&slab[row * GEGLU_SLD + c * 8]);
        if (m < p.M && n < p.N / 2) *reinterpret_cast<h8*>(p.Y + (long)m * p.ldy + n) = v;
    }
}

constexpr int XR_BM = 128, XR_BN = 256, XR_K = 320, XR_NKT = XR_K / 64;
constexpr int XR_XS = XR_NKT * XR_BM * 64, XR_WT = XR_BN * 64, XR_SLAB = 16 * 40;
__host__ __device__ inline int geglu_xres_source_row(int n, int N) {
    const int nt = n / 256, wn = (n % 256) / 64, i = (n % 64) / 16, g = (n % 16) / 4, r = n % 4;
    const int h = nt * 128 + wn * 32 + i * 8 + g * 2 + (r & 1);
    return r < 2 ? h : N / 2 + h;
}
template <int LNF>
__global__ __launch_bounds__(512, 2) void geglu_xres_kernel(GemmParams p) {
    __shared__ __attribute__((aligned(16))) half_t smem[XR_XS + 2 * XR_WT + 8 * XR_SLAB];
    half_t* const Xs = smem;
    half_t* const Wb = smem + XR_XS;
    const int tid = threadIdx.x, lane = tid & 63, wave = tid >> 6;
    const int wm = wave >> 2, wn = wave & 3;
    const int l15 = lane & 15, g = lane >> 4;
    half_t* const slab = smem + XR_XS + 2 * XR_WT + wave * XR_SLAB;
    const int m0 = blockIdx.x * XR_BM;
    const int NT = p.N / XR_BN;
    const int wave_u = __builtin_amdgcn_readfirstlane(wave);
    auto glds16 = [&](const half_t* src, half_t* dst) {
        __builtin_amdgcn_global_load_lds((const __attribute__((address_space(1))) void*)src, (__attribute__((address_space(3))) void*)dst, 16, 0, 0);
    };
    const int rb = tid >> 3, kc = (tid & 7) ^ (rb & 7);
#pragma unroll
    for (int kt = 0; kt < XR_NKT; ++kt)
#pragma unroll
        for (int i = 0; i < 2; ++i) {
            const int m = m0 + rb + 64 * i;
            glds16(m < p.M ? p.X + (long)m * p.ldx + kt * 64 + kc * 8 : uv_zero_page, Xs + kt * XR_BM * 64 + (64 * i + wave_u * 8) * 64);
        }
    auto issue_w = [&](int nt, int kt, int buf) {
#pragma unroll
        for (int i = 0; i < 4; ++i) glds16(p.W + (long)(nt * XR_BN + rb + 64 * i) * XR_K + kt * 64 + kc * 8, Wb + buf * XR_WT + (64 * i + wave_u * 8) * 64);
    };
    issue_w(0, 0, 0);
    float2 lnrow[LNF == 2 ? 4 : 1];
    if constexpr (LNF == 2) {
#pragma unroll
        for (int j = 0; j < 4; ++j) {
            const int m = m0 + wm * 64 + j * 16 + l15;
            float s1 = 0.f, s2 = 0.f;
            if (m < p.M) {
                const float2* sp = reinterpret_cast<const float2*>(p.ln_stats) + (long)m * p.ln_slots;
                for (int e = 0; e < p.ln_slots; ++e) {
                    const float2 t = sp[e];
                    s1 += t.x;
                    s2 += t.y;
                }
            }
            const float mean = s1 * (1.f / XR_K);
// ... 408 lines not shown
        woff[i] = (unsigned)(wset + (long)n * p.K + kc * 8);
    }
    const int Cin = p.C1 + p.C2;
    int tap = 0, cc = kc * 8;
    if (MODE == 1) {
        if (p.korder) {
            tap = kt0 % 9;
            cc += (kt0 / 9) * 64;
        } else {
            cc += kt0 * BK;
            tap = cc / Cin;
            cc -= tap * Cin;
        }
    }
    const int wave_u = __builtin_amdgcn_readfirstlane(tid >> 6);
    const half_t* zp = uv_zero_page;
    auto glds16 = [&](const half_t* src, half_t* dst) {
        __builtin_amdgcn_global_load_lds((const __attribute__((address_space(1))) void*)src,
                                         (__attribute__((address_space(3))) void*)dst, 16, 0, 0);
    };
    auto issue_tile = [&](int k0, int buf, int parts = 3) {
        half_t* Xd = smem + buf * TILE + wave_u * 8 * LDSH;
        half_t* Wd = Xd + BMB * LDSH;
        const bool kok = (k0 + kc * 8) < p.K;
        if (!(parts & 1)) {
        } else if (MODE == 0) {
#pragma unroll
            for (int i = 0; i < MJ; ++i) glds16((x_ok[i] && kok) ? p.X + xoff[i] + k0 : zp, Xd + 64 * i * LDSH);
        } else if (fast_conv) {
            const int tap_u = __builtin_amdgcn_readfirstlane(tap);
            const int slab_u = __builtin_amdgcn_readfirstlane(cc - kc * 8);
            const bool src2 = slab_u >= p.C1;
            const half_t* base = src2 ? p.X2 : p.X;
            const int cs = src2 ? p.C2 : p.C1;
            const int ky = tap_u / 3, kx = tap_u - 3 * ky;
            const long delta = (long)(ky * p.Ws + kx) * cs + (src2 ? slab_u - p.C1 : slab_u) + kc * 8;
#pragma unroll
            for (int i = 0; i < MJ; ++i) {
                const bool ok = kok && ((x_mask[i] >> tap_u) & 1u);
                glds16(ok ? base + (long)x_pix0[i] * cs + delta : zp, Xd + 64 * i * LDSH);
            }
        } else {
            const int ky = (p.tapw == 3) ? tap / 3 : tap;
            const int kx = (p.tapw == 3) ? tap - 3 * ky : 0;
            const int He = p.Hs << p.up, We = p.Ws << p.up;
            const bool src2 = cc >= p.C1;
            const half_t* base = src2 ? p.X2 : p.X;
            const int cs = src2 ? p.C2 : p.C1;
            const int co = src2 ? cc - p.C1 : cc;
#pragma unroll
            for (int i = 0; i < MJ; ++i) {
                int iy = x_iy0[i] + ky, ix = x_ix0[i] + kx;
                bool ok = x_ok[i] && kok && iy >= 0 && iy < He && ix >= 0 && ix < We;
                long pix = (long)(x_img[i] + (iy >> p.up)) * p.Ws + (ix >> p.up);
                glds16(ok ? base + pix * cs + co : zp, Xd + 64 * i * LDSH);
            }
        }
        if (!(parts & 2)) return;
#pragma unroll
        for (int i = 0; i < 5; ++i) glds16((w_ok[i] && kok) ? p.W + woff[i] + k0 : zp, Wd + 64 * i * LDSH);
        if (MODE == 1) {
            if (p.korder) {
                if (++tap == 9) { tap = 0; cc += 64; }
            } else {
                cc += BK;
                while (cc >= Cin) { cc -= Cin; ++tap; }
            }
        }
    };

    const int nk = kt1 - kt0;
    issue_tile(kt0 * BK, 0);
    if (p.splits <= 1) epi_const_stage<LNF>(p, m0, n0, BMB, tid, epc);
    f4 acc[NF][MJ];
#pragma unroll
    for (int i = 0; i < NF; ++i)
#pragma unroll
        for (int j = 0; j < MJ; ++j) acc[i][j] = f4{0.f, 0.f, 0.f, 0.f};
    const int sw = l15 & 7;
    for (int kt = 0; kt < nk; ++kt) {
        __syncthreads();
        const bool more = kt + 1 < nk;
        if (more) issue_tile((kt0 + kt + 1) * BK, (kt + 1) & 1, 1);
        const half_t* Xs = smem + (kt & 1) * TILE;
        const half_t* Ws = Xs + BMB * LDSH;
#pragma unroll
        for (int ks = 0; ks < 2; ++ks) {
            if (ks == 1 && more) issue_tile((kt0 + kt + 1) * BK, (kt + 1) & 1, 2);
            const int ch = ((ks * 4 + g) ^ sw) * 8;
            h8 a[NF];
#pragma unroll
            for (int i = 0; i < NF; ++i) a[i] = *reinterpret_cast<const h8*>(&Ws[(wn * 160 + i * 16 + l15) * LDSH + ch]);
#pragma unroll
            for (int j = 0; j < MJ; ++j) {
                h8 b = *reinterpret_cast<const h8*>(&Xs[(wm * 16 * MJ + j * 16 + l15) * LDSH + ch]);
#pragma unroll
                for (int i = 0; i < NF; ++i) acc[i][j] = __builtin_amdgcn_mfma_f32_16x16x32_f16(a[i], b, acc[i][j], 0, 0, 0);
            }
        }
    }
    if (p.splits > 1) {
#pragma unroll
        for (int j = 0; j < MJ; ++j) {
            const int m = m0 + wm * 16 * MJ + j * 16 + l15;
            if (m >= p.M) continue;
            float* row = p.partial + ((long)split * p.M + m) * p.N + n0 + wn * 160 + g * 4;
#pragma unroll
            for (int i = 0; i < NF; ++i) *reinterpret_cast<f4*>(row + i * 16) = acc[i][j];
        }
        return;
    }
    if (p.epi_lds == 3) {
        if constexpr (MODE == 0 && (LNF == 0 || LNF == 2)) {
            __syncthreads();
            gemm_epilogue_geglu_slab<MJ, LNF>(p, acc, smem + wave * (64 * GEGLU_SLD), m0 + wm * 16 * MJ, n0 + wn * 160, lane, epc, wn * 160, wm * 16 * MJ);
        }
        return;
    }
    if (p.epi_lds) {
        __syncthreads();
        gemm_epilogue_lds<MJ, LNF>(p, acc, reinterpret_cast<float*>(smem) + wave * (16 * EPI_LDW), m0 + wm * 16 * MJ, n0 + wn * 160, lane, epc, wn * 160,
                                   wm * 16 * MJ, reinterpret_cast<float2*>(reinterpret_cast<char*>(smem) + EPI_STAT_SCRATCH) + wave * 320,
                                   reinterpret_cast<half_t*>(reinterpret_cast<char*>(smem) + EPI_STAT_SCRATCH) + wave * 2560);
        return;
    }
#pragma unroll
    for (int j = 0; j < MJ; ++j) {
        f4 col[NF];
#pragma unroll
        for (int i = 0; i < NF; ++i) col[i] = acc[i][j];
        gemm_epilogue_row<NF, LNF, true>(p, col, m0 + wm * 16 * MJ + j * 16 + l15, n0 + wn * 160, g, epc, wn * 160,
                                   (LNF == 2) ? reinterpret_cast<const float2*>(epc + EPC_ROWST)[wm * 16 * MJ + j * 16 + l15] : float2{0.f, 1.f});
    }
}


template <int MJ>
__global__ __launch_bounds__(512, 2) void conv_patch_kernel(GemmParams p) {
    constexpr int NF = 10, BMB = 64 * MJ, BNB = 320, LDSH = 64;
    constexpr int PROUNDS = 4;
    constexpr int PBUF = PROUNDS * 512 * 8;
    constexpr int WT = BNB * LDSH;
    __shared__ __attribute__((aligned(16))) half_t smem[2 * PBUF + 2 * WT + 2 * EPC_TOTAL];
    float* const epc = reinterpret_cast<float*>(smem + 2 * PBUF + 2 * WT);
    half_t* const Pb = smem;
    half_t* const Wb = smem + 2 * PBUF;

    const int tid = threadIdx.x;
    const int lane = tid & 63, wave = tid >> 6;
    const int wn = wave & 1, wm = wave >> 1;
    const int l15 = lane & 15, g = lane >> 4;
    const int nt_n = p.N / BNB;
    int lid = xcd_remap(blockIdx.x, gridDim.x);
    const int ntiles = nt_n * ((p.M + BMB - 1) / BMB);
    const int split = lid / ntiles;
    lid -= split * ntiles;
    const int tn = lid % nt_n, tm = lid / nt_n;
    const int m0 = tm * BMB, n0 = tn * BNB;
    const int Wd = p.Wo, PW = Wd + 2, Himg = p.Ho;
    const int rows_total = p.M / Wd;
    const int R = BMB / Wd;
    const int gr0 = m0 / Wd;
    const int r0 = gr0 % Himg;
    const int nsep = (gr0 + R - 1) / Himg - gr0 / Himg;
    const int nprow = R + 2 + nsep;
    const int npieces = nprow * PW * 4;
    const int wave_u = __builtin_amdgcn_readfirstlane(wave);
    const half_t* zp = uv_zero_page;
    auto glds16 = [&](const half_t* src, half_t* dst) {
        __builtin_amdgcn_global_load_lds((const __attribute__((address_space(1))) void*)src,
                                         (__attribute__((address_space(3))) void*)dst, 16, 0, 0);
    };

    int ppix[PROUNDS], pch[PROUNDS];
#pragma unroll
    for (int i = 0; i < PROUNDS; ++i) {
        const int q = i * 512 + tid;
        const int pp = q >> 2, cst = q & 3;
        const int py = pp / PW, px = pp - py * PW;
        const int sq = py - 1 + r0;
        const int seg = sq >= 0 ? sq / (Himg + 1) : 0, pos = sq >= 0 ? sq - seg * (Himg + 1) : Himg;
        const int gr = gr0 - r0 + seg * Himg + pos;
        const bool ok = q < npieces && px >= 1 && px <= Wd && pos != Himg && gr < rows_total;
        const int img = gr / Himg, yy = gr - img * Himg;
        ppix[i] = ok ? (img * p.Hs + (yy >> p.up)) * p.Ws + ((px - 1) >> p.up) : -1;
        pch[i] = (cst ^ (((pp >> 2) & 1) << 1)) * 8;
    }
    auto issue_patch = [&](int slab) {
        const int c0 = slab * 32;
        const bool src2 = c0 >= p.C1;
        const half_t* base = src2 ? p.X2 : p.X;
        const int cs = src2 ? p.C2 : p.C1;
        const int co = src2 ? c0 - p.C1 : c0;
        half_t* dst = Pb + (slab & 1) * PBUF + wave_u * 64 * 8;
#pragma unroll
        for (int i = 0; i < PROUNDS; ++i)
            if (i * 512 < npieces) glds16(ppix[i] >= 0 ? base + (long)ppix[i] * cs + co + pch[i] : zp, dst + i * 512 * 8);
    };
    const int rb = tid >> 3;
    const int kc = (tid & 7) ^ (rb & 7);
    unsigned woff[5];
#pragma unroll
    for (int i = 0; i < 5; ++i) woff[i] = (unsigned)((long)(n0 + rb + 64 * i) * p.K + kc * 8);
    auto issue_w = [&](int t) {
        half_t* dst = Wb + (t & 1) * WT + wave_u * 8 * LDSH;
#pragma unroll
        for (int i = 0; i < 5; ++i) glds16(p.W32 + woff[i] + t * 64, dst + 64 * i * LDSH);
    };

    int pbase[MJ];
#pragma unroll
    for (int j = 0; j < MJ; ++j) {
        const int ml = wm * 16 * MJ + j * 16 + l15;
        const int ry = ml / Wd, rx = ml - ry * Wd;
        const int seps = (gr0 + ry) / Himg - gr0 / Himg;
        pbase[j] = (ry + seps) * PW + rx;
    }

    const int nslab_all = (p.C1 + p.C2) / 32;
    const int s_begin = p.splits > 1 ? split * (p.ktps / 9) * 2 : 0;
    const int s_end = p.splits > 1 ? (s_begin + (p.ktps / 9) * 2 < nslab_all ? s_begin + (p.ktps / 9) * 2 : nslab_all) : nslab_all;
    const int nslab = s_end - s_begin;
    const int T = nslab * 9 / 2;
    const int t_off = s_begin * 9 / 2;
    issue_patch(s_begin);
    if (nslab > 1) issue_patch(s_begin + 1);
    issue_w(t_off);
    if (p.splits <= 1) epi_const_stage<0>(p, m0, n0, BMB, tid, epc);
    f4 acc[NF][MJ];
#pragma unroll
    for (int i = 0; i < NF; ++i)
#pragma unroll
        for (int j = 0; j < MJ; ++j) acc[i][j] = f4{0.f, 0.f, 0.f, 0.f};
    int next_patch = 2;
    int u_slab = s_begin, u_tap = 0;
    const int sw = l15 & 7;
    for (int t = 0; t < T; ++t) {
        __syncthreads();
        if (next_patch < nslab && 9 * (next_patch - 1) <= 2 * t) {
            issue_patch(s_begin + next_patch);
            ++next_patch;
        }
        const half_t* Ws = Wb + ((t_off + t) & 1) * WT;
#pragma unroll
        for (int ks = 0; ks < 2; ++ks) {
            if (ks == 1 && t + 1 < T) issue_w(t_off + t + 1);
            const half_t* Ps = Pb + (u_slab & 1) * PBUF;
            const int ky = u_tap / 3, kx = u_tap - 3 * ky;
            const int delta = ky * PW + kx;
            const int ch = ((ks * 4 + g) ^ sw) * 8;
            h8 a[NF];
#pragma unroll
            for (int i = 0; i < NF; ++i) a[i] = *reinterpret_cast<const h8*>(&Ws[(wn * 160 + i * 16 + l15) * LDSH + ch]);
#pragma unroll
            for (int j = 0; j < MJ; ++j) {
                const int pp = pbase[j] + delta;
                const h8 b = *reinterpret_cast<const h8*>(&Ps[pp * 32 + ((g ^ (((pp >> 2) & 1) << 1)) << 3)]);
#pragma unroll
                for (int i = 0; i < NF; ++i) acc[i][j] = __builtin_amdgcn_mfma_f32_16x16x32_f16(a[i], b, acc[i][j], 0, 0, 0);
            }
            if (++u_tap == 9) { u_tap = 0; ++u_slab; }
        }
    }
    if (p.splits > 1) {
#pragma unroll
        for (int j = 0; j < MJ; ++j) {
            const int m = m0 + wm * 16 * MJ + j * 16 + l15;
            if (m >= p.M) continue;
            float* row = p.partial + ((long)split * p.M + m) * p.N + n0 + wn * 160 + g * 4;
#pragma unroll
            for (int i = 0; i < NF; ++i) *reinterpret_cast<f4*>(row + i * 16) = acc[i][j];
        }
        return;
    }
    if (p.epi_lds) {
        __syncthreads();
        gemm_epilogue_lds<MJ>(p, acc, reinterpret_cast<float*>(smem) + wave * (16 * EPI_LDW), m0 + wm * 16 * MJ, n0 + wn * 160, lane, epc, wn * 160, 0, nullptr,
                              reinterpret_cast<half_t*>(reinterpret_cast<char*>(smem) + EPI_STAT_SCRATCH) + wave * 2560);
        return;
    }
#pragma unroll
    for (int j = 0; j < MJ; ++j) {
        f4 col[NF];
#pragma unroll
        for (int i = 0; i < NF; ++i) col[i] = acc[i][j];
        gemm_epilogue_row<NF, 0, true>(p, col, m0 + wm * 16 * MJ + j * 16 + l15, n0 + wn * 160, g, epc, wn * 160);
    }
}


__global__ __launch_bounds__(256) void linear_small_kernel(const half_t* __restrict__ x, const half_t* __restrict__ W,
                                                           const half_t* __restrict__ b, half_t* __restrict__ y,
                                                           int M, int N, int K, int silu_in) {
    const int lane = threadIdx.x & 63;
    const int n = blockIdx.x * 4 + (threadIdx.x >> 6);
    if (n >= N) return;
    float acc[8];
#pragma unroll
    for (int m = 0; m < 8; ++m) acc[m] = 0.f;
    for (int k = lane * 8; k < K; k += 64 * 8) {
        h8 w = *reinterpret_cast<const h8*>(W + (long)n * K + k);
#pragma unroll
        for (int m = 0; m < 8; ++m) {
            if (m < M) {
                h8 xv = *reinterpret_cast<const h8*>(x + (long)m * K + k);
#pragma unroll
                for (int e = 0; e < 8; ++e) {
                    float xf = (float)xv[e];
                    if (silu_in) xf = silu_f(xf);
                    acc[m] += xf * (float)w[e];
                }
            }
        }
    }
#pragma unroll
    for (int m = 0; m < 8; ++m) {
        float s = wave_sum(acc[m]);
        if (lane == 0 && m < M) y[(long)m * N + n] = (half_t)(s + (b ? (float)b[n] : 0.f));
    }
}

}

int uv_num_cus() {
    static int n = 0;
    if (n == 0) {
        int dev = 0;
        n = 256;
        hipDeviceProp_t pr;
        if (hipGetDevice(&dev) == hipSuccess && hipGetDeviceProperties(&pr, dev) == hipSuccess && pr.multiProcessorCount > 0)
            n = pr.multiProcessorCount;
    }
    return n;
}

struct GemmKernel {
    void (*fn)(GemmParams);
    const char* sym;
};
#define UV_KERNEL(...) {__VA_ARGS__, #__VA_ARGS__}
static const GemmKernel GEMM_KERNELS[] = {
    UV_KERNEL(geglu_xres_kernel<0>),   UV_KERNEL(geglu_xres_kernel<2>),
    UV_KERNEL(conv_patch_kernel<3>),   UV_KERNEL(conv_patch_kernel<4>),
    UV_KERNEL(gemm_big_kernel<0,3,0>), UV_KERNEL(gemm_big_kernel<0,4,0>), UV_KERNEL(gemm_big_kernel<1,3,0>), UV_KERNEL(gemm_big_kernel<1,4,0>),
    UV_KERNEL(gemm_big_kernel<0,3,1>), UV_KERNEL(gemm_big_kernel<0,4,1>), UV_KERNEL(gemm_big_kernel<0,3,2>), UV_KERNEL(gemm_big_kernel<0,4,2>),
    UV_KERNEL(gemm_big_kernel<0,3,3>),
    UV_KERNEL(gemm_kernel<4,0,4,0>),   UV_KERNEL(gemm_kernel<5,0,4,0>),   UV_KERNEL(gemm_kernel<4,1,4,0>),   UV_KERNEL(gemm_kernel<5,1,4,0>),
    UV_KERNEL(gemm_kernel<4,0,2,0>),   UV_KERNEL(gemm_kernel<4,1,2,0>),   UV_KERNEL(gemm_kernel<5,0,4,1>),
    UV_KERNEL(gemm_kernel<4,0,4,2>),   UV_KERNEL(gemm_kernel<5,0,4,2>),   UV_KERNEL(gemm_kernel<4,0,2,2>),
};
#undef UV_KERNEL


static int uv_pick_splits(long ntiles, int nk, long slots, int min_ktps, int max_s, double us_per_ktile, double mn_bytes) {
    int best_s = 1;
    double best = (double)((ntiles + slots - 1) / slots) * nk * us_per_ktile;
    for (int s = 2; s <= max_s; ++s) {
        const int ktps = (nk + s - 1) / s;
        if (ktps < min_ktps) break;
        const double t = (double)((ntiles * s + slots - 1) / slots) * ktps * us_per_ktile + 2.0 * s * mn_bytes / 4.0e6;
        if (t < best * 0.95) { best = t; best_s = s; }
    }
    return best_s;
}

static bool uv_conv_patch_eligible(const GemmParams& p, int bmb) {
    return p.W32 && p.taps == 9 && p.stride == 1 && p.C1 % 32 == 0 && p.C2 % 32 == 0 && (p.C1 + p.C2) % 64 == 0 && p.N % 320 == 0 && (p.Wo % 16 == 0 || 16 % p.Wo == 0) &&
           bmb % p.Wo == 0 && (bmb / p.Wo + 2 + bmb / p.Wo / p.Ho + 1) * (p.Wo + 2) <= 512 && !p.geglu;
}

constexpr long BIG_MIN_TILES = 150;

static bool big_shape_ok(int N, int K, long x_elems, bool ragged = false, int ragged_min = 640) {
    return (N % 320 == 0 || (ragged && N % 8 == 0 && N >= ragged_min)) && (long)N * K < (1L << 31) && x_elems < (1L << 31);
}
static long big_tiles(long M, int N, int rows) { return ((M + rows - 1) / rows) * ((N + 319) / 320); }
static bool big_would_split(long ntiles, int K) { return ntiles < BIG_MIN_TILES && ntiles >= 8 && K >= 128 * 64; }

struct SmallPlan {
    bool nf5, small_m;
    int bn, nt, splits;
};
static SmallPlan small_plan(long M, int N, int K, bool geglu, int mode, bool want_stats, int ncu) {
    SmallPlan sp;
    sp.nf5 = !geglu && (N % 160 == 0) && ((N % 128 != 0) || want_stats);
    sp.bn = sp.nf5 ? 160 : 128;
    sp.nt = (int)(((M + BM_DEFAULT - 1) / BM_DEFAULT) * ((N + sp.bn - 1) / sp.bn));
    sp.small_m = !sp.nf5 && sp.nt < 2 * ncu && M > 64 && (mode == 0 || geglu || (K + 63) / 64 < 16);
    if (sp.small_m) sp.nt = (int)(((M + 63) / 64) * ((N + sp.bn - 1) / sp.bn));
    sp.splits = 1;
    if (!geglu && N % 4 == 0 && sp.nt < 384) {
        const int nk = (K + 63) / 64;
        const int s = uv_pick_splits(sp.nt, nk, 2L * ncu, 4, 16, 1.0, (double)M * N * 4.0);
        if (s >= 2) sp.splits = s;
    }
    return sp;
}


static bool takes_big_direct(long M, int N, int K, long ldx) {
    return big_shape_ok(N, K, M * (ldx ? ldx : (long)K)) && big_tiles(M, N, 256) >= BIG_MIN_TILES && big_tiles(M, N, 192) >= BIG_MIN_TILES;
}
bool uv_linear_takes_big_direct(long M, int N, int K, long ldx) { return takes_big_direct(M, N, K, ldx); }

static bool fold_small_ok(long M, int N, int K, bool want_stats, int ncu) {
    if (big_shape_ok(N, K, M * (long)K) && big_would_split(big_tiles(M, N, 256), K)) return false;
    return small_plan(M, N, K, false, 0, want_stats, ncu).splits == 1;
}
static bool fold_producer_ok(long M, int N, int K, int ncu) {
    if (takes_big_direct(M, N, K, 0)) return true;
    return N % 160 == 0 && K % 8 == 0 && fold_small_ok(M, N, K, true, ncu);
}
static bool fold_consumer_ok(long M, int N, int K, bool geglu, int ncu) {
    if (takes_big_direct(M, N, K, 0)) return true;
    return !geglu && N % 4 == 0 && K % 160 == 0 && fold_small_ok(M, N, K, false, ncu);
}
bool uv_linear_fold_producer_ok(long M, int N, int K) { return fold_producer_ok(M, N, K, uv_num_cus()); }
bool uv_linear_fold_consumer_ok(long M, int N, int K, bool geglu) { return fold_consumer_ok(M, N, K, geglu, uv_num_cus()); }

int uv_launch_geglu_xres_permute(const half_t* in, half_t* out, int rows, int cols, hipStream_t stream) {
    UV_REQUIRE(rows % 256 == 0 && cols >= 1, "geglu_xres_permute: %d rows must be a multiple of 256", rows);
    hipLaunchKernelGGL(geglu_xres_permute_kernel, dim3((unsigned)(((long)rows * cols + 255) / 256)), dim3(256), 0, stream, in, out, rows, cols);
    UV_LAUNCH_CHECK();
    return UV_OK;
}
static bool geglu_xres_ok(int N, int K, long M, long ncu) {
    if (K != XR_K || N % XR_BN != 0) return false;
    if (M <= 0) return true;
    const long blocks = (M + XR_BM - 1) / XR_BM, rounds = (blocks + ncu - 1) / ncu;
    return blocks >= 2 * ncu && blocks * 10 >= rounds * ncu * 8;
}
bool uv_geglu_xres_ok(int N, int K, long M) { return geglu_xres_ok(N, K, M, uv_num_cus()); }

static inline void uv_gemm_bytes(const GemmParams& p, int mode, double* compulsory, double* expanded) {
    const double out = (double)p.M * (p.geglu ? p.N / 2 : p.N), w = (double)p.N * p.K, res = p.R ? (double)p.M * p.N : 0.0;
    const double a_exp = (double)p.M * p.K;
    double a = a_exp;
    if (mode == 1 && p.Ho > 0 && p.Wo > 0) a = (double)(p.M / ((long)p.Ho * p.Wo)) * p.Hs * p.Ws * (p.C1 + p.C2);
    *compulsory = 2.0 * (a + w + out + res);
    *expanded = 2.0 * (a_exp + w + out + res);
}

static GemmParams with_conv_defaults(GemmParams p, int mode) {
    if (mode == 1 && p.tapw == 0) {
        p.tapw = p.taps == 9 ? 3 : 1;
        p.pady = p.padx = p.taps == 9 ? 1 : 0;
    }
    return p;
}

#define PLAN_REQUIRE(cond, ...) UV_PLAN_REQUIRE(pl, cond, __VA_ARGS__)
GemmPlan uv_gemm_plan(const GemmParams& p, int mode, int ncu) {
    GemmPlan pl;
    auto al16 = [](const void* q) { return (reinterpret_cast<uintptr_t>(q) & 15) == 0; };
    PLAN_REQUIRE(p.M > 0 && p.N > 0 && p.K > 0, "gemm: empty problem M=%d N=%d K=%d", p.M, p.N, p.K);
    pl.block = 512;
    pl.flops = 2.0 * p.M * (double)p.N * p.K;
    if (p.geglu == 2) {
        PLAN_REQUIRE(mode == 0 && p.K == XR_K && p.N % XR_BN == 0 && p.ldx % 8 == 0 && p.ldy % 8 == 0 && al16(p.X) && al16(p.W) && al16(p.Y) && al16(p.bias) &&
                     !p.R && !p.rowbias && !p.bias2 && !p.stats_out && !p.act && !p.gate && !p.gn_out && (long)p.M * p.ldx < (1L << 31) &&
                     (!p.ln_stats || (p.ln_wsum && p.ln_bias && p.ln_slots > 0 && !p.bias)),
                     "geglu (X-resident order): needs K = 320, N %% 256 == 0, 16-byte aligned rows, no residual / second bias (M=%d N=%d K=%d)", p.M, p.N, p.K);
        pl.cls = UV_CLS_GEMM_BIG;
        pl.bytes = 2.0 * ((double)p.M * p.K + (double)p.N * p.K + (double)p.M * (p.N / 2));
        pl.prof_sym = true;
        snprintf(pl.sym, sizeof pl.sym, "geglu_xres_kernel<%d>", p.ln_stats ? 2 : 0);
        pl.grid = (p.M + XR_BM - 1) / XR_BM;
        return pl;
    }
    const bool lnf = p.ln_stats || p.stats_out;
    PLAN_REQUIRE(p.K % 8 == 0, "gemm: K=%d must be a multiple of 8", p.K);
    PLAN_REQUIRE(!(p.act || p.gate) || (!p.geglu && !lnf && mode == 0), "gemm: the activation / gate epilogue is for plain linears (no GEGLU, LayerNorm fold, conv)");
    PLAN_REQUIRE(!p.gate || (p.rows_per_gate >= 1 && p.ld_gate % 8 == 0 && p.N % 8 == 0 && al16(p.gate)),
                 "gemm: gate rows must be 16-byte aligned (ld_gate %% 8 == 0, N %% 8 == 0)");
    if (mode == 0) {
        PLAN_REQUIRE(p.ldx % 8 == 0, "gemm: ldx=%ld must be a multiple of 8", p.ldx);
    } else {
        PLAN_REQUIRE(p.C1 % 8 == 0 && p.C2 % 8 == 0, "conv: channel counts must be multiples of 8 (C1=%d C2=%d)", p.C1, p.C2);
        PLAN_REQUIRE((p.taps == 1 && p.tapw == 1) || (p.taps == 9 && p.tapw == 3) || (p.taps == 3 && p.tapw == 1), "conv: taps=%d with %d per row (1x1, 3x3 or the 3x1 frame conv)", p.taps, p.tapw);
        PLAN_REQUIRE(p.K == p.taps * (p.C1 + p.C2), "conv: K=%d != taps*(C1+C2)", p.K);
        const bool sym3 = p.taps == 9 && p.pady == 1 && p.padx == 1;
        PLAN_REQUIRE(!p.korder || (sym3 && p.C1 % 64 == 0 && p.C2 % 64 == 0), "conv: tap-inner k order needs the 3x3 / padding-1 kernel and 64-channel slabs");
        PLAN_REQUIRE(!p.W32 || sym3, "conv: the LDS-patch weight copy is for the 3x3 / padding-1 kernel");
    }
    uv_gemm_bytes(p, mode, &pl.bytes, &pl.aux_bytes);
    const int nk = (p.K + 63) / 64;
    const size_t mn_f32 = (size_t)p.M * p.N * sizeof(float);
    const unsigned reduce_grid = (unsigned)(((long)p.M * (p.N / 4) + 255) / 256);

    const bool conv_rag = mode == 1 && !p.gn_out && p.N % 64 == 0 && p.N >= 256 && (p.N % 320 == 0 || p.N % 320 >= 192);
    const bool ragged = (mode == 0 && !p.geglu && !lnf) || conv_rag;
    const long n256 = big_tiles(p.M, p.N, 256), n192 = big_tiles(p.M, p.N, 192);
    const double c256 = (double)((n256 + ncu - 1) / ncu) * 256.0, c192 = (double)((n192 + ncu - 1) / ncu) * 192.0 * (mode == 1 ? 1.03 : 1.05);
    const bool mmdit_epi = mode == 0 && (p.act || p.gate);
    bool use192 = mmdit_epi || (c192 < c256 && n192 >= BIG_MIN_TILES);
    if (p.w_rows_per_set) {
        PLAN_REQUIRE(mode == 0 && p.bias32 && !p.geglu && !p.ln_stats && !mmdit_epi && p.M % p.w_rows_per_set == 0 && (p.w_rows_per_set % 256 == 0 || p.w_rows_per_set % 192 == 0) &&
                     (long)(p.M / p.w_rows_per_set) * p.N * p.K + (long)p.N * p.K < (1L << 31),
                     "linear: weight sets need a plain linear, an fp32 bias per set and %d rows per set that a 256- or 192-row tile divides", p.w_rows_per_set);
        if (p.w_rows_per_set % (use192 ? 192 : 256) != 0) use192 = !use192;
    }
    const long nblk = use192 ? n192 : n256;
    const long xmax = (mode == 0) ? (long)p.M * p.ldx : (long)p.M * (p.C1 > p.C2 ? p.C1 : p.C2) * 4;
    int bsplits = 1;
    if (!p.geglu && p.N % 320 == 0 && big_would_split(nblk, p.K)) {
        int sp = uv_pick_splits(nblk, nk, ncu, 24, 8, 2.2, (double)p.M * p.N * 4.0);
        while (sp >= 2 && sp * mn_f32 > UV_SPLITK_WS_BYTES) --sp;
        if (sp >= 2 && nblk * sp >= 128) bsplits = sp;
    }
    const bool fills = nblk >= BIG_MIN_TILES || bsplits > 1;
    const bool use_patch = mode == 1 && fills && uv_conv_patch_eligible(p, use192 ? 192 : 256);
    PLAN_REQUIRE(p.W || use_patch, "conv: only the [Cin/32][9][32] weight copy was given but the problem is not eligible for the LDS-patch kernel "
                 "(3x3, stride 1, whole image rows per 256/192-row tile, >= 150 tiles or a reduction long enough for split-K)");
    if (fills && big_shape_ok(p.N, p.K, xmax, ragged, conv_rag ? 256 : 640)) {
        const int mj = use192 ? 3 : 4;
        const int ntn = (p.N + 319) / 320;
        if (mode == 0 && ntn > 4 && (long)p.N * p.K * 2 > (3L << 20)) {
            pl.tile_gn = ntn % 2 == 0 ? 2 : 0;
            pl.tile_gm = 8;
        }
        pl.epi_lds = !p.geglu && p.ldy % 8 == 0 && al16(p.Y) && al16(p.bias) && al16(p.bias2) && al16(p.rowbias) && p.ldrb % 8 == 0 &&
                     (!p.R || (p.ldr % 8 == 0 && al16(p.R)));
        if (p.geglu && mode == 0 && p.ldy % 8 == 0 && al16(p.Y) && al16(p.bias) && p.N % 16 == 0) pl.epi_lds = 3;
        PLAN_REQUIRE(!p.bias32 || (pl.epi_lds == 1 && bsplits <= 1), "linear: the fp32 bias needs the LDS row epilogue of the direct path (16-byte aligned Y / R / bias rows, no split-K)");
        if (bsplits > 1) {
            pl.ktps = (nk + bsplits - 1) / bsplits;
            if (use_patch) pl.ktps = (pl.ktps + 8) / 9 * 9;
            pl.splits = (nk + pl.ktps - 1) / pl.ktps;
            pl.ws_bytes = pl.splits * mn_f32;
        }
        PLAN_REQUIRE(!p.w_rows_per_set || (pl.epi_lds == 1 && pl.splits == 1), "linear: weight sets run on the direct 256x320 path with the LDS epilogue only");
        pl.gn_emit = p.gn_out && pl.epi_lds == 1 && pl.splits == 1 && !p.geglu && !p.stats_out && !p.act && !p.gate && p.N % 320 == 0 && p.M % 16 == 0 &&
                     p.gn_G > 0 && p.gn_gw * p.gn_G == p.N && (p.gn_gw == 10 || p.gn_gw == 20 || p.gn_gw == 40);
        if (lnf && !use_patch) {
            PLAN_REQUIRE(mode == 0 && pl.splits == 1 && (pl.epi_lds || !p.stats_out) && (!p.ln_stats || (p.ln_wsum && p.ln_bias && p.ln_slots > 0)) &&
                         (!p.stats_out || (!p.geglu && p.N % 160 == 0)), "linear: LayerNorm fold on a problem the direct 256x320 path does not take");
            PLAN_REQUIRE(!(p.ln_stats && p.stats_out), "linear: a LayerNorm-folded linear cannot also emit row statistics");
        }
        pl.cls = mode == 0 ? UV_CLS_GEMM_BIG : (use_patch ? UV_CLS_CONV_PATCH : UV_CLS_CONV_BIG);
        pl.prof_sym = true;
        if (use_patch) snprintf(pl.sym, sizeof pl.sym, "conv_patch_kernel<%d>", mj);
        else snprintf(pl.sym, sizeof pl.sym, "gemm_big_kernel<%d,%d,%d>", mode, mj, p.ln_stats ? 2 : (p.stats_out ? 1 : (mmdit_epi ? 3 : 0)));
        pl.grid = (unsigned)(nblk * pl.splits);
        pl.reduce_grid = pl.splits > 1 ? reduce_grid : 0;
        return pl;
    }

    PLAN_REQUIRE(!p.w_rows_per_set && !p.bias32, "linear: weight sets / an fp32 bias exist on the direct 256x320 path only (M=%d N=%d K=%d does not take it)", p.M, p.N, p.K);
    const SmallPlan sp = small_plan(p.M, p.N, p.K, p.geglu != 0, mode, p.stats_out != nullptr, ncu);
    if (lnf) {
        PLAN_REQUIRE(mode == 0 && !p.geglu && !p.act && !p.gate && sp.splits == 1 && !(p.ln_stats && p.stats_out) &&
                     (!p.stats_out || (sp.nf5 && p.N % 160 == 0)) &&
                     (!p.ln_stats || (p.ln_wsum && p.ln_bias && p.ln_slots > 0 && p.N % 4 == 0)),
                     "linear: LayerNorm fold requested for M=%d N=%d K=%d, which neither the direct 256x320 path nor the 128-wide path without split-K takes "
                     "(uv_linear_fold_producer_ok / uv_linear_fold_consumer_ok)", p.M, p.N, p.K);
    }
    if (p.geglu) PLAN_REQUIRE(p.N % 32 == 0, "geglu: N=%d must be a multiple of 32", p.N);
    if (sp.splits >= 2) {
        pl.ktps = (nk + sp.splits - 1) / sp.splits;
        pl.splits = (nk + pl.ktps - 1) / pl.ktps;
        pl.ws_bytes = pl.splits * mn_f32;
        if (!(p.partial && p.partial_bytes >= pl.ws_bytes) && pl.ws_bytes > UV_SPLITK_WS_BYTES) {
            pl.splits = 1;
            pl.ktps = 0;
            pl.ws_bytes = 0;
        }
    }
    pl.cls = mode == 0 ? UV_CLS_GEMM : UV_CLS_CONV;
    snprintf(pl.sym, sizeof pl.sym, "gemm_kernel<%d,%d,%d,%d>", sp.nf5 ? 5 : 4, mode, sp.small_m ? 2 : 4, p.stats_out ? 1 : (p.ln_stats ? 2 : 0));
    pl.grid = (unsigned)(sp.nt * pl.splits);
    pl.block = 256;
    pl.reduce_grid = pl.splits > 1 ? reduce_grid : 0;
    return pl;
}
#undef PLAN_REQUIRE

int uv_launch_gemm(const GemmParams& p0, int mode, hipStream_t stream) {
    GemmParams q = with_conv_defaults(p0, mode);
    const GemmPlan pl = uv_gemm_plan(q, mode, uv_num_cus());
    if (pl.rc != UV_OK) {
        uv_set_error("%s", pl.err);
        return pl.rc;
    }
    const GemmKernel* kern = nullptr;
    for (const GemmKernel& k : GEMM_KERNELS)
        if (!strcmp(k.sym, pl.sym)) kern = &k;
    if (!kern) {
        uv_set_error("gemm: the plan names %s, which the launch table does not hold", pl.sym);
        return UV_ERR_STATE;
    }
    q.splits = pl.splits;
    q.ktps = pl.ktps;
    q.epi_lds = pl.epi_lds;
    q.tile_gn = pl.tile_gn;
    q.tile_gm = pl.tile_gm;
    if (!pl.gn_emit) q.gn_out = nullptr;
    else if (q.gn_emitted) *q.gn_emitted = 1;
    const bool own_ws = pl.ws_bytes && !(q.partial && q.partial_bytes >= pl.ws_bytes);
    if (own_ws) UV_HIP(hipMallocAsync((void**)&q.partial, pl.ws_bytes, stream));
    uv_prof_begin(pl.cls, pl.flops, pl.bytes, stream, pl.prof_sym ? pl.sym : nullptr, pl.aux_bytes);
    hipLaunchKernelGGL(kern->fn, dim3(pl.grid), dim3(pl.block), 0, stream, q);
    if (pl.reduce_grid) hipLaunchKernelGGL(splitk_reduce_kernel, dim3(pl.reduce_grid), dim3(256), 0, stream, q);
    if (own_ws) UV_HIP(hipFreeAsync(q.partial, stream));
    uv_prof_end(stream);
    UV_LAUNCH_CHECK();
    return UV_OK;
}

std::string uv_gemm_plan_symbols() {
    std::string out;
    for (const GemmKernel& k : GEMM_KERNELS) out += (out.empty() ? "" : ";") + std::string(k.sym);
    return out;
}
int uv_gemm_plan_text(const GemmParams& p0, int mode, int ncu, char* buf, int n) {
    const GemmParams p = with_conv_defaults(p0, mode);
    const GemmPlan pl = uv_gemm_plan(p, mode, ncu);
    if (pl.rc != UV_OK) {
        snprintf(buf, (size_t)n, "%s", pl.err);
        uv_set_error("%s", pl.err);
        return pl.rc;
    }
    snprintf(buf, (size_t)n, "%s grid=%u block=%u splits=%d%s big_direct=%d fold_producer=%d fold_consumer=%d geglu_consumer=%d geglu_xres=%d", pl.sym, pl.grid,
             pl.block, pl.splits, pl.reduce_grid ? " +splitk_reduce" : "", (int)takes_big_direct(p.M, p.N, p.K, p.ldx), (int)fold_producer_ok(p.M, p.N, p.K, ncu),
             (int)fold_consumer_ok(p.M, p.N, p.K, false, ncu), (int)fold_consumer_ok(p.M, p.N, p.K, true, ncu), (int)geglu_xres_ok(p.N, p.K, p.M, ncu));
    return UV_OK;
}

int uv_launch_linear_small(const half_t* x, const half_t* W, const half_t* b, half_t* y, int M, int N, int K,
                           int silu_in, hipStream_t stream) {
    UV_REQUIRE(M >= 1 && M <= 8, "linear_small: M=%d must be in 1..8", M);
    UV_REQUIRE(K % 8 == 0, "linear_small: K=%d must be a multiple of 8", K);
    hipLaunchKernelGGL(linear_small_kernel, dim3((N + 3) / 4), dim3(256), 0, stream, x, W, b, y, M, N, K, silu_in);
    UV_LAUNCH_CHECK();
    return UV_OK;
}
```

### univst_amd/csrc/kernels.h

```cpp
#pragma once
#include "common.h"
#include <string>

struct GemmParams {
    const half_t* X = nullptr;
    const half_t* X2 = nullptr;
    const half_t* W = nullptr;
    const half_t* W32 = nullptr;
    half_t* Y = nullptr;
    long ldx = 0, ldy = 0;
    int M = 0, N = 0, K = 0;
    int C1 = 0, C2 = 0, Hs = 1, Ws = 1, up = 0, Ho = 1, Wo = 1, stride = 1, taps = 1;
    int tapw = 0, pady = 0, padx = 0;
    int korder = 0;
    const half_t* bias = nullptr;
    const half_t* rowbias = nullptr;
    int rows_per_rb = 1;
    long ldrb = 0;
    const half_t* R = nullptr;
    long ldr = 0;
    const half_t* bias2 = nullptr;
    int geglu = 0;
    int act = 0;
    const half_t* gate = nullptr;
    long ld_gate = 0;
    int rows_per_gate = 1;
    int epi_lds = 0;
    float* partial = nullptr;
    size_t partial_bytes = 0;
    int splits = 1, ktps = 0;
    int tile_gn = 0, tile_gm = 0;
    int issue_mode = 0;
    float* gn_out = nullptr;
    int gn_G = 0, gn_gw = 0;
    int* gn_emitted = nullptr;
    int w_rows_per_set = 0;
    const float* bias32 = nullptr;
    float* stats_out = nullptr;
    const float* ln_stats = nullptr;
    int ln_slots = 0;
    float ln_eps = 0.f;
    const float* ln_wsum = nullptr;
    const float* ln_bias = nullptr;
};

struct AttnParams {
    const half_t* q = nullptr;
    const half_t* k = nullptr;
    const half_t* v = nullptr;
    half_t* o = nullptr;
    long ldq = 0, ldkv = 0, ldo = 0;
    const int* src_idx = nullptr;
    const int* src_cnt = nullptr;
    const float* src_logw = nullptr;
    int nsrc = 1, BF = 0, Nq = 0, Nkv = 0, heads = 0, d = 0;
    float scale_log2e = 0.f;
    int q_prescaled = 0;
    int order = 1;
    const half_t* kx = nullptr;
    const half_t* vx = nullptr;
    const int* x_idx = nullptr;
    long ldkv_x = 0;
    int Nkv_x = 0;
    float* state_out = nullptr;
    const float* state_in = nullptr;
};

struct Attn2Params {
    const half_t* X = nullptr;
    long ldx = 0;
    int M = 0;
    const float* ln_stats = nullptr;
    int ln_slots = 0;
    float ln_eps = 1e-5f;
    const float* ln_wsum = nullptr;
    const float* ln_bias = nullptr;
    const half_t* Wq_f = nullptr;
    const half_t* kvf = nullptr;
    int rows_per_branch = 0, heads = 0, Nkv = 0;
    int q_prescaled = 0;
    float scale_log2e = 0.f;
    const half_t* Wo_f = nullptr;
    const half_t* bias_o = nullptr;
    const half_t* R = nullptr;
    long ldr = 0;
    half_t* Y = nullptr;
    long ldy = 0;
    float* stats_out = nullptr;
    const half_t* Wp_f = nullptr;
    const half_t* bias_p = nullptr;
    const half_t* Rp = nullptr;
    long ldrp = 0;
#ifdef UV_A2_TRACE
    long long* trace = nullptr;
#endif
};
bool uv_attn2_fused_ok(int C, int heads, int rows_per_branch, int Nkv);
long uv_attn2_kvf_halfs(int B, int heads, int D);
int uv_launch_frag_pack(const half_t* W, half_t* out, int N, int K, hipStream_t s);
int uv_launch_kv_frag_pack(const half_t* kv, half_t* out, int B, int T, int C, int heads, hipStream_t s);
int uv_launch_attn2_fused(const Attn2Params& p, int C, hipStream_t s);

struct UvLaunchPlan {
    int rc = UV_OK;
    char err[400] = "";
    char sym[48] = "";
    unsigned grid = 0, block = 256;
    int cls = 0;
    double flops = 0.0, bytes = 0.0, aux_bytes = 0.0;
};
struct GemmPlan : UvLaunchPlan {
    bool prof_sym = false;
    int splits = 1, ktps = 0, epi_lds = 0, tile_gn = 0, tile_gm = 0;
    bool gn_emit = false;
    size_t ws_bytes = 0;
    unsigned reduce_grid = 0;
};
struct AttnPlan : UvLaunchPlan {};
GemmPlan uv_gemm_plan(const GemmParams& p, int mode, int ncu);
AttnPlan uv_attention_plan(const AttnParams& p);
int uv_gemm_plan_text(const GemmParams& p, int mode, int ncu, char* buf, int n);
int uv_attention_plan_text(const AttnParams& p, char* buf, int n);
std::string uv_gemm_plan_symbols();
std::string uv_attention_plan_symbols();

int uv_num_cus();
int uv_launch_gemm(const GemmParams& p, int mode, hipStream_t stream);
bool uv_linear_takes_big_direct(long M, int N, int K, long ldx = 0);
bool uv_linear_fold_producer_ok(long M, int N, int K);
bool uv_linear_fold_consumer_ok(long M, int N, int K, bool geglu);
bool uv_geglu_xres_ok(int N, int K, long M = 0);
int uv_launch_geglu_xres_permute(const half_t* in, half_t* out, int rows, int cols, hipStream_t stream);
constexpr size_t UV_SPLITK_WS_BYTES = 128u << 20;
int uv_launch_linear_small(const half_t* x, const half_t* W, const half_t* b, half_t* y, int M, int N, int K, int silu_in,
                           hipStream_t stream);
struct UvGnComm {
    int world = 1;
    float* red = nullptr;
    long byte_off = 0;
    int (*allreduce)(void* user, int64_t byte_off, int count_f32) = nullptr;
    void* user = nullptr;
};
int uv_groupnorm_workspace_floats(int S, int G);
struct UvGnFold {
    const half_t* W = nullptr;
    const half_t* bias = nullptr;
    int N = 0;
    half_t* W_out = nullptr;
    float* bias32 = nullptr;
};
enum { UV_GN_SMALL = 0, UV_GN_STREAM = 1, UV_GN_STREAM_PRODUCER = 2 };
struct GnPlan {
    int rc = UV_OK;
    char err[200] = "";
    int route = UV_GN_STREAM;
    bool fold = false;
    bool sharded = false;
    int S = 0;
    int block = 0, TR = 0;
    int nchunk = 0, rpc = 0;
    int nblk = 0, rpb = 0;
    int lds_stats = 0, lds_tail = 0;
    unsigned stats_grid[2] = {0, 0}, reduce_grid = 0, tail_grid[2] = {0, 0};
    double bytes = 0.0;
};
GnPlan uv_groupnorm_plan(int C1, int C2, long rows, int rows_per_stat, int G, int fold_N, int world, bool producer_stats);
int uv_launch_groupnorm(const half_t* s1, const half_t* s2, int C1, int C2, long rows, int rows_per_stat, int G, float eps,
                        const half_t* gamma, const half_t* beta, int silu, half_t* out, float* part, hipStream_t stream,
                        const UvGnComm* comm = nullptr, const float* pre_part = nullptr, const float* pre_part2 = nullptr, const UvGnFold* fold = nullptr);
int uv_launch_layernorm(const half_t* x, long ldx, half_t* y, long ldy, const half_t* gamma, const half_t* beta, long rows,
                        int C, float eps, hipStream_t stream);
int uv_launch_attention(const AttnParams& p, hipStream_t stream);
int uv_launch_tr16_probe(float* out, hipStream_t stream);
int uv_launch_colstats(const half_t* x, long ld, int F, int N, int ncols, float* mean, float* stdv, hipStream_t stream);
int uv_launch_adain_shift(half_t* qkv, long ld, int F, int N, int C, float* mean, float* stdv, float alpha, float beta,
                          float gamma, hipStream_t stream);
int uv_launch_latent_adain(const half_t* cnt, const half_t* sty, half_t* out, int Cl, int F, int HW, hipStream_t stream);
int uv_launch_latent_adain_stats(const half_t* cnt, float* st, int Cl, int F, int HW, hipStream_t stream);
int uv_launch_latent_adain_apply(const half_t* cnt, const half_t* sty, const float* st, long n_total, half_t* out, int Cl, int F, int HW,
                                 hipStream_t stream);
int uv_launch_rows_pack(const half_t* src, long ld, int col0, int width, int N, int B, int frames_per_branch, int frame, half_t* dst, hipStream_t s);
int uv_launch_ncfhw_to_nhwc(const half_t* x, half_t* y, int B, int Cl, int F, int HW, int CP, hipStream_t s);
int uv_launch_nhwc_to_ncfhw(const half_t* x, int ldx, half_t* y, int B, int Cl, int F, int HW, hipStream_t s);
int uv_launch_timestep_embed(float t, half_t* out, int B, int dim, int flip, float shift, hipStream_t s);
int uv_launch_axpby(const half_t* x, const half_t* e, half_t* out, float cx, float ce, long n, hipStream_t s);
int uv_launch_mask_blend(const half_t* a, const half_t* b, const half_t* m, half_t* out, int Cl, long FHW, hipStream_t s);
int uv_launch_mask_resize(const uint8_t* mask, half_t* out, int F, int H, int W, int h, int w, hipStream_t s);
int uv_launch_add_bias_rows(half_t* x, const half_t* b, long rows, int C, hipStream_t s);
int64_t uv_maskprop_workspace_bytes(int hw, int Nsrc, int C);
int uv_launch_maskprop_frame(const float* feat_tar, const float* feat_src, const float* segs_src, float* segs_tar, int hw,
                             int Nsrc, int C, int ncls, float T, int topk, void* ws, hipStream_t s);
int uv_launch_maskprop_finalize(const float* segs, uint8_t* out, int ncls, int h, int w, int H, int W, void* ws, hipStream_t s);
int uv_launch_warp_accumulate(const uint8_t* key, const uint8_t* now, const float* fwd, const float* bwd, float* acc, int H, int W,
                              float thr, hipStream_t s);
int uv_launch_warp_window_key(uint8_t* est, const float* const* flows, int nn, int F, int H, int W, int key, int r, float thr, hipStream_t s);
int uv_launch_latent_window_smooth(half_t* x0, const float* lflow, int C, int F, int h, int w, int r, float thr, hipStream_t s);
int uv_launch_delay_us(double us, hipStream_t s);
int uv_launch_accumulate_u8(const uint8_t* f, float* acc, long n, hipStream_t s);
int uv_launch_window_store(const float* acc, float weight, uint8_t* dst, long n, hipStream_t s);

enum {
    UV_CLS_GEMM_BIG = 0,
    UV_CLS_CONV_BIG = 1,
    UV_CLS_GEMM = 2,
    UV_CLS_CONV = 3,
    UV_CLS_ATTN_D40 = 4,
    UV_CLS_ATTN_D80 = 5,
    UV_CLS_ATTN_OTHER = 6,
    UV_CLS_GROUPNORM = 7,
    UV_CLS_LAYERNORM = 8,
    UV_CLS_ADAIN = 9,
    UV_CLS_ATTN_TEXT = 10,
    UV_CLS_CONV_PATCH = 11,
    UV_CLS_ATTN2_FUSED = 12,
    UV_NCLS = 13
};
void uv_prof_enable(int on);
bool uv_prof_on();
void uv_prof_begin(int cls, double flops, double bytes, hipStream_t s, const char* sym = nullptr, double aux_bytes = 0.0);
void uv_prof_end(hipStream_t s);
void uv_prof_aux(double* aux, int ncls);
int uv_prof_collect(double* ms, long* count, double* flops, double* bytes, int ncls);
std::string uv_prof_symbols(int cls);
```

### univst_amd/csrc/unet.hip

```cpp
#include <math.h>
#include <string.h>

#include <map>
#include <string>
#include <unordered_map>
#include <vector>

#include "comm.h"
#include "kernels.h"
#include "unet.h"

namespace {

__global__ void permute_conv_weight_t32_kernel(const half_t* __restrict__ in, half_t* __restrict__ out, int Co, int Ci) {
    long i = (long)blockIdx.x * blockDim.x + threadIdx.x;
    long total = (long)Co * Ci * 9;
    if (i >= total) return;
    int j = (int)(i % 32);
    int t = (int)((i / 32) % 9);
    int q = (int)((i / (32 * 9)) % (Ci / 32));
    int o = (int)(i / ((long)Ci * 9));
    out[i] = in[((long)o * Ci + q * 32 + j) * 9 + t];
}
__global__ void geglu_interleave_kernel(const half_t* __restrict__ in, half_t* __restrict__ out, int rows, int cols) {
// ... 55 lines not shown
    const long row = i / C;
    const int f = (int)((row / HW) % F);
    float acc = (float)bias[co];
    for (int t = 0; t < 3; ++t) {
        const int ff = f + t - 1;
        if (ff < 0 || ff >= F) continue;
        const half_t* xr = x + (row + (long)(t - 1) * HW) * C;
        for (int ci = 0; ci < C; ++ci) acc += (float)w[((long)co * C + ci) * 3 + t] * (float)xr[ci];
    }
    y[i] = (half_t)acc;
}
template <int D8>
__global__ __launch_bounds__(256) void temporal_attn_kernel(const half_t* __restrict__ qkv, half_t* __restrict__ out, int B, int F, int N, int C,
                                                            int heads, float scale) {
    const long i = (long)blockIdx.x * 256 + threadIdx.x;
    if (i >= (long)B * N * heads * F) return;
    const int n = (int)(i % N);
    const int f = (int)((i / N) % F);
    const int h = (int)((i / ((long)N * F)) % heads);
    const int b = (int)(i / ((long)N * F * heads));
    const long ld = 3L * C;
    const half_t* base = qkv + ((long)b * F * N + n) * ld + h * (D8 * 8);
    const long fs = (long)N * ld;
    h8 q[D8];
#pragma unroll
    for (int c = 0; c < D8; ++c) q[c] = *reinterpret_cast<const h8*>(base + f * fs + c * 8);
    float p[32];
    float mx = -INFINITY;
#pragma unroll
    for (int g = 0; g < 32; ++g) {
        p[g] = -INFINITY;
        if (g < F) {
            float s = 0.f;
#pragma unroll
            for (int c = 0; c < D8; ++c) {
                const h8 k8 = *reinterpret_cast<const h8*>(base + g * fs + C + c * 8);
#pragma unroll
                for (int e = 0; e < 8; ++e) s += (float)q[c][e] * (float)k8[e];
            }
            p[g] = s * scale;
            mx = fmaxf(mx, p[g]);
        }
    }
    float l = 0.f;
#pragma unroll
    for (int g = 0; g < 32; ++g) {
        p[g] = g < F ? __expf(p[g] - mx) : 0.f;
        l += p[g];
    }
    const float inv = 1.f / l;
    half_t* op = out + (((long)b * F + f) * N + n) * C + h * (D8 * 8);
#pragma unroll 1
    for (int c = 0; c < D8; ++c) {
        float o[8] = {0.f, 0.f, 0.f, 0.f, 0.f, 0.f, 0.f, 0.f};
#pragma unroll
        for (int g = 0; g < 32; ++g) {
            if (g < F) {
                const h8 v8 = *reinterpret_cast<const h8*>(base + g * fs + 2 * C + c * 8);
#pragma unroll
                for (int e = 0; e < 8; ++e) o[e] += p[g] * (float)v8[e];
            }
        }
        h8 r;
#pragma unroll
        for (int e = 0; e < 8; ++e) r[e] = (half_t)(o[e] * inv);
        *reinterpret_cast<h8*>(op + c * 8) = r;
    }
}

}

UNet::~UNet() {
    for (auto& kv : idx_tables) (void)hipFree(kv.second);
    if (arena.base) (void)hipFree(arena.base);
    if (d_counter) (void)hipFree(d_counter);
    if (ev_fork) (void)hipEventDestroy(ev_fork);
    if (ev_join) (void)hipEventDestroy(ev_join);
    if (xstream) (void)hipStreamDestroy(xstream);
    if (emu_flag) (void)hipFree(emu_flag);
}

int UNet::comm_streams() {
    if (xstream) return UV_OK;
    int lo = 0, hi = 0;
    UV_HIP(hipDeviceGetStreamPriorityRange(&lo, &hi));
    UV_HIP(hipStreamCreateWithPriority(&xstream, hipStreamNonBlocking, hi));
    UV_HIP(hipEventCreateWithFlags(&ev_fork, hipEventDisableTiming));
    UV_HIP(hipEventCreateWithFlags(&ev_join, hipEventDisableTiming));
    return UV_OK;
}

int UNet::load_tensor(const char* key, const void* dev_ptr, int dtype, const int64_t* shape, int ndim, hipStream_t s) {
    UV_RUN(load(key, dev_ptr, dtype, shape, ndim, s));
    finalized = false;
    return UV_OK;
}

int UNet::finalize(hipStream_t s) {
    clear_derived();
    std::vector<std::string> keys;
    for (auto& kv : weights) keys.push_back(kv.first);
    std::vector<std::pair<std::string, int>> tunits;
    std::unordered_map<std::string, int> tslot;
    for (const std::string& k : keys) {
        size_t pos;
        if ((pos = k.find(".conv_temporal.")) != std::string::npos) {
            const std::string pre = k.substr(0, pos);
            if (!tslot.count(pre)) { tslot[pre] = (int)tunits.size(); tunits.push_back({pre, 0}); }
        } else if ((pos = k.find(".attn_temporal.to_out.0.weight")) != std::string::npos) {
            const std::string pre = k.substr(0, pos);
            if (!tslot.count(pre + "#a")) { tslot[pre + "#a"] = (int)tunits.size(); tunits.push_back({pre, 1}); }
        }
    }
    const size_t ncnt = tunits.size() + 1;
    if (d_counter) (void)hipFree(d_counter);
    d_counter = nullptr;
    UV_HIP(hipMalloc(&d_counter, ncnt * sizeof(unsigned)));
    UV_HIP(hipMemsetAsync(d_counter, 0, ncnt * sizeof(unsigned), s));
    temporal_conv_active.clear();
    temporal_attn_active.clear();
    auto ends = [](const std::string& a, const char* suf) {
        size_t n = strlen(suf);
        return a.size() >= n && a.compare(a.size() - n, n, suf) == 0;
    };
    auto level_of = [](const std::string& a) {
        int i = 0;
        if (sscanf(a.c_str(), "down_blocks.%d.", &i) == 1) return i;
        if (sscanf(a.c_str(), "up_blocks.%d.", &i) == 1) return 3 - i;
        return 3;
    };
    for (const std::string& k : keys) {
        const WTensor& t = weights[k];
        if (k.find("conv_temporal.weight") != std::string::npos) {
            UV_REQUIRE(t.shape.size() == 3 && t.shape[0] == t.shape[1] && t.shape[2] == 3, "%s: expected a [C,C,3] Conv1d weight", k.c_str());
            long n = t.shape[0] * t.shape[1] * t.shape[2];
            hipLaunchKernelGGL(count_not_dirac_slot_kernel, dim3(nb(n)), dim3(256), 0, s, t.ptr, (int)t.shape[0], (int)t.shape[1],
                               (int)t.shape[2], d_counter + tslot[k.substr(0, k.find(".conv_temporal."))]);
        } else if (k.find("conv_temporal.bias") != std::string::npos) {
            long n = t.shape[0];
            hipLaunchKernelGGL(count_nonzero_kernel, dim3(nb(n)), dim3(256), 0, s, t.ptr, n, d_counter + tslot[k.substr(0, k.find(".conv_temporal."))]);
        } else if (ends(k, "attn_temporal.to_out.0.weight")) {
            long n = 1;
            for (long v : t.shape) n *= v;
            hipLaunchKernelGGL(count_nonzero_kernel, dim3(nb(n)), dim3(256), 0, s, t.ptr, n,
                               d_counter + tslot[k.substr(0, k.find(".attn_temporal.to_out.0.weight")) + "#a"]);
        } else if (t.shape.size() == 4 && k.find("_temporal") == std::string::npos) {
            int Co = (int)t.shape[0], Ci = (int)t.shape[1], taps = (int)(t.shape[2] * t.shape[3]);
            UV_REQUIRE(taps == 1 || taps == 9, "%s: only 1x1 / 3x3 convs are supported", k.c_str());
            UV_RUN(uv_derive_conv_layouts(*this, k, s));
            if (taps == 9 && Ci % 64 == 0 && Co % 320 == 0 && k.find("downsamplers") == std::string::npos) {
                half_t* d3;
                UV_RUN(derive(k + "#t32", {Co, Ci / 32, 9, 32}, &d3));
                hipLaunchKernelGGL(permute_conv_weight_t32_kernel, dim3(nb((long)Co * Ci * 9)), dim3(256), 0, s, t.ptr, d3, Co, Ci);
            }
        } else if (ends(k, ".attn1.to_q.weight")) {
            std::string p = k.substr(0, k.size() - strlen("to_q.weight"));
            const WTensor *tk = find(p + "to_k.weight"), *tv = find(p + "to_v.weight");
            UV_REQUIRE(tk && tv, "%s: to_k / to_v missing", p.c_str());
            long C = t.shape[0], K = t.shape[1];
            half_t* d;
            UV_RUN(derive(p + "qkv#fused", {3 * C, K}, &d));
            UV_HIP(hipMemcpyAsync(d, t.ptr, C * K * 2, hipMemcpyDeviceToDevice, s));
            UV_HIP(hipMemcpyAsync(d + C * K, tk->ptr, C * K * 2, hipMemcpyDeviceToDevice, s));
            UV_HIP(hipMemcpyAsync(d + 2 * C * K, tv->ptr, C * K * 2, hipMemcpyDeviceToDevice, s));
            const int hd = (int)C / cfg.attention_heads[level_of(k)];
            if (hd == 40 || hd == 64 || hd == 80 || hd == 160) {
                half_t* d2;
                UV_RUN(derive(p + "qkv#fused#qs", {3 * C, K}, &d2));
                UV_RUN(uv_launch_scale_f16(t.ptr, d2, C * K, 1.4426950408889634f / sqrtf((float)hd), s));
                UV_HIP(hipMemcpyAsync(d2 + C * K, tk->ptr, C * K * 2, hipMemcpyDeviceToDevice, s));
                UV_HIP(hipMemcpyAsync(d2 + 2 * C * K, tv->ptr, C * K * 2, hipMemcpyDeviceToDevice, s));
            }
        } else if (ends(k, ".attn2.to_q.weight")) {
            const long C = t.shape[0], K = t.shape[1];
            const int hd = (int)C / cfg.attention_heads[level_of(k)];
            if (hd == 40) {
                half_t* d2;
                UV_RUN(derive(k + "#qs", {C, K}, &d2));
                UV_RUN(uv_launch_scale_f16(t.ptr, d2, C * K, 1.4426950408889634f / sqrtf((float)hd), s));
            }
        } else if (ends(k, ".attn2.to_k.weight")) {
            std::string p = k.substr(0, k.size() - strlen("to_k.weight"));
            const WTensor* tv = find(p + "to_v.weight");
            UV_REQUIRE(tv, "%s: to_v missing", p.c_str());
            long C = t.shape[0], K = t.shape[1];
            half_t* d;
            UV_RUN(derive(p + "kv#fused", {2 * C, K}, &d));
            UV_HIP(hipMemcpyAsync(d, t.ptr, C * K * 2, hipMemcpyDeviceToDevice, s));
            UV_HIP(hipMemcpyAsync(d + C * K, tv->ptr, C * K * 2, hipMemcpyDeviceToDevice, s));
        } else if (ends(k, ".ff.net.0.proj.weight") || ends(k, ".ff.net.0.proj.bias")) {
            int rows = (int)t.shape[0], cols = t.shape.size() > 1 ? (int)t.shape[1] : 1;
            UV_REQUIRE(rows % 32 == 0, "%s: GEGLU width %d must be a multiple of 32", k.c_str(), rows);
            half_t* d;
            UV_RUN(derive(k + "#geglu", {rows, cols}, &d));
            hipLaunchKernelGGL(geglu_interleave_kernel, dim3(nb((long)rows * cols)), dim3(256), 0, s, t.ptr, d, rows, cols);
            int kdim = cols;
            if (!ends(k, ".weight")) {
                const WTensor* wt = find(k.substr(0, k.size() - strlen("bias")) + "weight");
                UV_REQUIRE(wt && wt->shape.size() == 2, "%s: the projection's weight is missing", k.c_str());
                kdim = (int)wt->shape[1];
            }
            if (uv_geglu_xres_ok(rows, kdim)) {
                half_t* dx;
                UV_RUN(derive(k + "#xres", {rows, cols}, &dx));
                UV_RUN(uv_launch_geglu_xres_permute(t.ptr, dx, rows, cols, s));
            }
        }
    }
    for (const std::string& k : keys) {
        if (!ends(k, ".transformer_blocks.0.norm1.weight")) continue;
        const std::string b = k.substr(0, k.size() - strlen(".norm1.weight"));
        struct FoldJob { const char* norm; std::string w; std::string bias; };
        std::vector<FoldJob> jobs = {
            {".norm1", b + (find(b + ".attn1.qkv#fused#qs") ? ".attn1.qkv#fused#qs" : ".attn1.qkv#fused"), ""},
            {".norm2", b + (find(b + ".attn2.to_q.weight#qs") ? ".attn2.to_q.weight#qs" : ".attn2.to_q.weight"), ""},
            {".norm3", b + ".ff.net.0.proj.weight#geglu", b + ".ff.net.0.proj.bias#geglu"}};
        if (find(b + ".ff.net.0.proj.weight#xres")) jobs.push_back({".norm3", b + ".ff.net.0.proj.weight#xres", b + ".ff.net.0.proj.bias#xres"});
        for (auto& j : jobs) {
            const WTensor *w = find(j.w), *gm = find(b + j.norm + ".weight"), *bt = find(b + j.norm + ".bias");
            const WTensor* bi = j.bias.empty() ? nullptr : find(j.bias);
            UV_REQUIRE(w && gm && bt && (j.bias.empty() || bi) && w->shape.size() == 2 && gm->shape[0] == w->shape[1],
                       "%s: LayerNorm / linear pair incomplete", (b + j.norm).c_str());
            const long N = w->shape[0], K = w->shape[1];
            half_t *wo, *ws, *lb;
            int rc = derive(j.w + "#ln", {N, K}, &wo);
            if (!rc) rc = derive(j.w + "#ln.wsum", {2 * N}, &ws);
            if (!rc) rc = derive(j.w + "#ln.bias", {2 * N}, &lb);
            if (rc) return rc;
            hipLaunchKernelGGL(ln_fold_weight_kernel, dim3((unsigned)N), dim3(64), 0, s, w->ptr, gm->ptr, bt->ptr, bi ? bi->ptr : nullptr, wo,
                               (float*)ws, (float*)lb, (int)K);
        }
    }
    for (const std::string& k : keys) {
        if (!ends(k, ".attn2.to_out.0.weight")) continue;
        const std::string b = k.substr(0, k.size() - strlen(".attn2.to_out.0.weight"));
        const WTensor& t = weights[k];
        if (t.shape.size() != 2 || t.shape[0] != t.shape[1] || !uv_attn2_fused_ok((int)t.shape[0], cfg.attention_heads[level_of(k)], 64, 77)) continue;
        const std::string wq = b + (find(b + ".attn2.to_q.weight#qs") ? ".attn2.to_q.weight#qs" : ".attn2.to_q.weight");
        for (const std::string& src : {k, wq, wq + "#ln", b + ".attn1.to_out.0.weight"}) {
            const WTensor* w = find(src);
            if (!w) continue;
            half_t* d;
            UV_RUN(derive(src + "#frag", {w->shape[0], w->shape[1]}, &d));
            UV_RUN(uv_launch_frag_pack(w->ptr, d, (int)w->shape[0], (int)w->shape[1], s));
        }
    }
    {
        std::vector<std::string> tk;
        for (const std::string& k : keys)
            if (ends(k, ".time_emb_proj.weight")) tk.push_back(k);
        std::sort(tk.begin(), tk.end());
        temb_off.clear();
        temb_total = 0;
        for (const std::string& k : tk) {
            temb_off[k.substr(0, k.size() - strlen(".time_emb_proj.weight"))] = temb_total;
            temb_total += weights[k].shape[0];
        }
        if (!tk.empty()) {
            const long K = weights[tk[0]].shape[1];
            half_t *wa, *ba;
            UV_RUN(derive("time_emb_proj#all.weight", {temb_total, K}, &wa));
            UV_RUN(derive("time_emb_proj#all.bias", {temb_total}, &ba));
            for (const std::string& k : tk) {
                const std::string pre = k.substr(0, k.size() - strlen(".time_emb_proj.weight"));
                const WTensor& wt = weights[k];
                const WTensor* bt = find(pre + ".time_emb_proj.bias");
                UV_REQUIRE(bt && wt.shape[1] == K, "%s: time_emb_proj bias missing or width mismatch", pre.c_str());
                UV_HIP(hipMemcpyAsync(wa + temb_off[pre] * K, wt.ptr, wt.shape[0] * K * sizeof(half_t), hipMemcpyDeviceToDevice, s));
                UV_HIP(hipMemcpyAsync(ba + temb_off[pre], bt->ptr, wt.shape[0] * sizeof(half_t), hipMemcpyDeviceToDevice, s));
            }
        }
    }
    UV_LAUNCH_CHECK();
    std::vector<unsigned> hc(ncnt, 0);
    UV_HIP(hipMemcpyAsync(hc.data(), d_counter, ncnt * sizeof(unsigned), hipMemcpyDeviceToHost, s));
    UV_HIP(hipStreamSynchronize(s));
    for (size_t i = 0; i < tunits.size(); ++i) {
        if (!hc[i]) continue;
        const std::string& pre = tunits[i].first;
        if (tunits[i].second == 0) {
            const WTensor* w = find(pre + ".conv_temporal.weight");
            UV_REQUIRE(w && find(pre + ".conv_temporal.bias"), "%s: conv_temporal weight / bias incomplete", pre.c_str());
            const int C = (int)w->shape[0];
            if (C % 8 == 0) {
                half_t* d;
                UV_RUN(derive(pre + ".conv_temporal.weight#t3x3", {C, 9, C}, &d));
                hipLaunchKernelGGL(embed_temporal_weight_kernel, dim3(nb((long)C * 9 * C)), dim3(256), 0, s, w->ptr, d, C);
            }
            temporal_conv_active[pre] = 1;
        } else {
            const WTensor *tq = find(pre + ".attn_temporal.to_q.weight"), *tk = find(pre + ".attn_temporal.to_k.weight"),
                          *tv = find(pre + ".attn_temporal.to_v.weight");
            UV_REQUIRE(tq && tk && tv && find(pre + ".norm_temporal.weight") && find(pre + ".norm_temporal.bias") &&
                       find(pre + ".attn_temporal.to_out.0.bias"), "%s: attn_temporal / norm_temporal parameters incomplete", pre.c_str());
            const long C = tq->shape[0], K = tq->shape[1];
            half_t* d;
            UV_RUN(derive(pre + ".attn_temporal.qkv#fused", {3 * C, K}, &d));
            UV_HIP(hipMemcpyAsync(d, tq->ptr, C * K * 2, hipMemcpyDeviceToDevice, s));
            UV_HIP(hipMemcpyAsync(d + C * K, tk->ptr, C * K * 2, hipMemcpyDeviceToDevice, s));
            UV_HIP(hipMemcpyAsync(d + 2 * C * K, tv->ptr, C * K * 2, hipMemcpyDeviceToDevice, s));
            temporal_attn_active[pre] = 1;
        }
    }
    UV_LAUNCH_CHECK();
    UV_HIP(hipStreamSynchronize(s));
    finalized = true;
    return UV_OK;
}

int UNet::reserve(int B, int F, int H, int Wd) {
    const long rows0 = (long)B * F * H * Wd;
    size_t need = (size_t)rows0 * cfg.block_out_channels[0] * 2 * 28 + (64u << 20) + UV_SPLITK_WS_BYTES + (gn_producer ? (size_t)rows0 * 1024 : 0);
    UV_RUN(arena.ensure(need));
    long key = ((long)B << 20) | F | ((long)rank << 40) | ((long)world << 50);
    if (!idx_tables.count(key)) {
        std::vector<int> t;
        const bool ext = world > 1 && rank > 0;
        auto prev = [&](int b, int f) { return f > 0 ? b * F + f - 1 : (ext ? B * F + b : b * F); };
        auto first = [&](int b) { return ext ? B * F + B + b : b * F; };
        std::vector<int> cnt;
        std::vector<float> lw;
        auto emit = [&](std::vector<int> srcs, int width) {
            std::vector<int> uniq;
            std::vector<int> mult;
            for (int sidx : srcs) {
                size_t j = 0;
                for (; j < uniq.size(); ++j)
                    if (uniq[j] == sidx) break;
                if (j == uniq.size()) { uniq.push_back(sidx); mult.push_back(1); }
                else mult[j]++;
            }
            cnt.push_back((int)uniq.size());
            for (int j = 0; j < width; ++j) {
                t.push_back(j < (int)uniq.size() ? uniq[j] : uniq[0]);
                lw.push_back(j < (int)uniq.size() ? log2f((float)mult[j]) : 0.f);
            }
        };
        auto emit_split = [&](std::vector<int> local, std::vector<int> halo, int width, std::vector<int>& t2, std::vector<int>& cnt2, int self) {
            cnt.push_back((int)local.size());
            for (int j = 0; j < width; ++j) {
                t.push_back(j < (int)local.size() ? local[j] : self);
                lw.push_back(0.f);
            }
            cnt2.push_back((int)halo.size());
            for (int j = 0; j < width; ++j) t2.push_back(j < (int)halo.size() ? halo[j] : self);
        };
        std::vector<int> t2s, t2p, c2s, c2p;
        for (int b = 0; b < B; ++b)
            for (int f = 0; f < F; ++f) {
                if (!ext) emit({prev(b, f), b * F + f, first(b)}, 3);
                else if (f == 0) emit_split({b * F + f}, {prev(b, f), first(b)}, 3, t2s, c2s, b * F + f);
                else emit_split({prev(b, f), b * F + f}, {first(b)}, 3, t2s, c2s, b * F + f);
            }
        for (int b = 0; b < B; ++b)
            for (int f = 0; f < F; ++f) {
                if (!ext) emit({prev(b, f), first(b)}, 2);
                else if (f == 0) emit_split({}, {prev(b, f), first(b)}, 2, t2p, c2p, b * F + f);
                else emit_split({prev(b, f)}, {first(b)}, 2, t2p, c2p, b * F + f);
            }
        for (int b = 0; b < B; ++b)
            for (int f = 0; f < F; ++f) t.push_back(b);
        for (int v : cnt) t.push_back(v);
        for (float v : lw) {
            int bits;
            memcpy(&bits, &v, 4);
            t.push_back(bits);
        }
        for (auto* v : {&t2s, &t2p, &c2s, &c2p})
            for (int x : *v) t.push_back(x);
        int* d;
        UV_HIP(hipMalloc(&d, t.size() * sizeof(int)));
        UV_HIP(hipMemcpy(d, t.data(), t.size() * sizeof(int), hipMemcpyHostToDevice));
        idx_tables[key] = d;
    }
    return UV_OK;
}

struct Fwd {
    UNet& u;
    hipStream_t s;
    int B, F, text_len;
    const univst_pnp* pnp;
    half_t* emb = nullptr;
    const half_t* text = nullptr;
    const int *idx_stock = nullptr, *idx_pnp = nullptr, *idx_text = nullptr, *cnt_stock = nullptr, *cnt_pnp = nullptr;
    const float *lw_stock = nullptr, *lw_pnp = nullptr;
    const int *idx2_stock = nullptr, *idx2_pnp = nullptr, *cnt2_stock = nullptr, *cnt2_pnp = nullptr;
    float* gn_ws = nullptr;
    float* sk_ws = nullptr;
    half_t* temb_all = nullptr;
    float* ad_ws = nullptr;
    float* gst_pool = nullptr;
    size_t gst_left = 0;

    float* gst_take(long rows, int C) {
        const size_t n = (size_t)(rows / 16) * (C / 10) * 2;
        if (!u.gn_producer || !gst_pool || rows % 16 != 0 || C % 10 != 0 || n > gst_left) return nullptr;
        float* p = gst_pool;
        gst_pool += n;
        gst_left -= n;
        return p;
    }
    void gst_give_back(long rows, int C) {
        const size_t n = (size_t)(rows / 16) * (C / 10) * 2;
        gst_pool -= n;
        gst_left += n;
    }

    half_t* alloc(long elems) {
        half_t* p = (half_t*)u.arena.alloc((size_t)elems * sizeof(half_t));
        if (!p) uv_set_error("unet: activation arena exhausted (%zu bytes); call univst_unet_reserve with the right geometry", u.arena.size);
        return p;
    }
    void free(void* p) { u.arena.release(p); }
    half_t* W(const std::string& k) { return u.W(k); }

    int groupnorm(const Act& a, const Act* b, int rows_per_stat, float eps, const std::string& p, int silu, half_t* out,
                  bool cross_frame = false, const UvGnFold* fold = nullptr) {
        UvGnComm gc;
        const bool sharded = cross_frame && u.world > 1;
        if (sharded) {
            gc.world = u.world;
            gc.red = (float*)u.comm_ws;
            gc.byte_off = 0;
            gc.allreduce = u.allreduce;
            gc.user = u.comm_user;
        }
        half_t *gm = W(p + ".weight"), *bt = W(p + ".bias");
        if (!gm || !bt) return u.missing_error("unet");
        return uv_launch_groupnorm(a.p, b ? b->p : nullptr, a.C, b ? b->C : 0, a.rows(), rows_per_stat, u.cfg.norm_num_groups,
                                   eps, gm, bt, silu, out, gn_ws, s, sharded ? &gc : nullptr,
                                   rows_per_stat % 16 == 0 ? a.gst : nullptr, b ? b->gst : nullptr, fold);
    }
    int conv(const Act& a, const Act* b, const std::string& p, int Cout, int taps, int stride, int up, const half_t* rowbias,
             const half_t* R, Act* out, long ldrb = 0, bool want_gst = false) {
        GemmParams g;
        g.X = a.p;
        g.X2 = b ? b->p : nullptr;
        g.C1 = a.C;
        g.C2 = b ? b->C : 0;
        g.Hs = a.H;
        g.Ws = a.W;
        g.up = up;
        g.stride = stride;
        g.taps = taps;
        const int He = a.H << up, We = a.W << up;
        g.Ho = (taps == 9) ? (He + 2 - 3) / stride + 1 : He;
        g.Wo = (taps == 9) ? (We + 2 - 3) / stride + 1 : We;
        g.M = a.imgs * g.Ho * g.Wo;
        g.N = Cout;
        g.K = taps * (g.C1 + g.C2);
        g.korder = (taps == 9 && g.C1 % 64 == 0 && g.C2 % 64 == 0 && u.find(p + ".weight#ti")) ? 1 : 0;
        g.W = W(p + (g.korder ? ".weight#ti" : ".weight#nhwc"));
        if (taps == 9 && stride == 1 && u.find(p + ".weight#t32")) g.W32 = W(p + ".weight#t32");
        g.bias = W(p + ".bias");
        g.rowbias = rowbias;
        g.ldrb = ldrb;
        g.rows_per_rb = F * g.Ho * g.Wo;
        g.R = R;
        g.ldr = Cout;
        out->imgs = a.imgs;
        out->H = g.Ho;
        out->W = g.Wo;
        out->C = Cout;
        out->p = alloc(out->rows() * Cout);
        if (!out->p) return UV_ERR_STATE;
        g.Y = out->p;
        g.ldy = Cout;
        if (!g.W || !g.bias) return u.missing_error("unet");
        g.partial = sk_ws;
        g.partial_bytes = UV_SPLITK_WS_BYTES;
        out->gst = nullptr;
        if (taps != 9 || !u.temporal_conv_active.count(p)) {
            int emitted = 0;
            if (want_gst && (g.gn_out = gst_take(out->rows(), Cout))) {
                g.gn_G = Cout / 10;
                g.gn_gw = 10;
                g.gn_emitted = &emitted;
            }
            UV_RUN(uv_launch_gemm(g, 1, s));
            if (g.gn_out) {
                if (emitted) out->gst = g.gn_out;
                else gst_give_back(out->rows(), Cout);
            }
            return UV_OK;
        }
        half_t* mid = alloc(out->rows() * Cout);
        if (!mid) return UV_ERR_STATE;
        g.Y = mid;
        g.rowbias = nullptr;
        g.R = nullptr;
        UV_RUN(uv_launch_gemm(g, 1, s));
        half_t *tw = W(p + ".conv_temporal.weight"), *tb = W(p + ".conv_temporal.bias");
        if (!tw || !tb) return u.missing_error("unet");
        const long HWo = (long)g.Ho * g.Wo;
        if (Cout % 8 != 0) {
            UV_REQUIRE(!rowbias && !R, "%s: temporal conv on %d channels cannot carry a fused epilogue", p.c_str(), Cout);
            hipLaunchKernelGGL(temporal_conv_small_kernel, dim3(nb(out->rows() * Cout)), dim3(256), 0, s, mid, out->p, tw, tb, B, F, HWo, Cout);
            UV_LAUNCH_CHECK();
        } else {
            GemmParams t;
            t.X = mid;
            t.C1 = Cout;
            t.Hs = F;
            t.Ws = (int)HWo;
            t.taps = 9;
            t.Ho = F;
            t.Wo = (int)HWo;
            t.M = (int)out->rows();
            t.N = Cout;
            t.K = 9 * Cout;
            t.W = W(p + ".conv_temporal.weight#t3x3");
            t.bias = tb;
            t.rowbias = rowbias;
            t.ldrb = ldrb;
            t.rows_per_rb = (int)(F * HWo);
            t.R = R;
            t.ldr = Cout;
            t.Y = out->p;
            t.ldy = Cout;
            if (!t.W) return u.missing_error("unet");
            t.partial = sk_ws;
            t.partial_bytes = UV_SPLITK_WS_BYTES;
            UV_RUN(uv_launch_gemm(t, 1, s));
        }
        free(mid);
        return UV_OK;
    }
    int linear(const half_t* X, long ldx, long M, int K, const std::string& wkey, const std::string& bkey, int N, half_t* Y,
               long ldy, const half_t* R = nullptr, long ldr = 0, const half_t* bias2 = nullptr, int geglu = 0, float* stats_out = nullptr,
               const float* ln_in = nullptr, const float** gst_out = nullptr, const half_t* wsets = nullptr, const float* bias32 = nullptr, int rows_per_set = 0) {
        GemmParams g;
        if (wsets) {
            g.w_rows_per_set = rows_per_set;
            g.bias32 = bias32;
        }
        int emitted = 0;
        if (gst_out) {
            *gst_out = nullptr;
            if ((g.gn_out = gst_take(M, N))) {
                g.gn_G = N / 10;
                g.gn_gw = 10;
                g.gn_emitted = &emitted;
            }
        }
        g.stats_out = stats_out;
        if (ln_in) {
            g.ln_stats = ln_in;
            g.ln_slots = K / 160;
            g.ln_eps = 1e-5f;
            g.ln_wsum = (const float*)W(wkey + ".wsum");
            g.ln_bias = (const float*)W(wkey + ".bias");
            if (!g.ln_wsum || !g.ln_bias) return u.missing_error("unet");
        }
        g.X = X;
        g.ldx = ldx;
        g.M = (int)M;
        g.K = K;
        g.N = N;
        g.W = wsets ? wsets : W(wkey);
        g.bias = (bkey.empty() || ln_in || wsets) ? nullptr : W(bkey);
        g.Y = Y;
        g.ldy = ldy;
        g.R = R;
        g.ldr = ldr;
        g.bias2 = bias2;
        g.geglu = geglu;
        if (!g.W || (!bkey.empty() && !ln_in && !wsets && !g.bias)) return u.missing_error("unet");
        g.partial = sk_ws;
        g.partial_bytes = UV_SPLITK_WS_BYTES;
        UV_RUN(uv_launch_gemm(g, 0, s));
        if (g.gn_out) {
            if (emitted) *gst_out = g.gn_out;
            else gst_give_back(M, N);
        }
        return UV_OK;
    }

    struct KvSlots {
        long o_send = 0, o_first = 0, o_prev = 0, o_rfirst = 0, nbytes = 0;
        bool emu = false;
    } kvs;
    int kv_post(const half_t* h, int C, int N) {
        kvs = KvSlots();
        kvs.nbytes = (long)B * N * C * sizeof(half_t);
        const int nslot = u.native_comm ? 6 : 4;
        const long slot = ((u.comm_ws_bytes - 65536) / nslot) & ~255L;
        UV_REQUIRE(kvs.nbytes <= slot, "kv_exchange: comm workspace too small (%ld B per slot, need %ld)", slot, kvs.nbytes);
        const long par = u.native_comm ? uv_comm_kv_parity(u.native_comm) : 0;
        kvs.o_send = 65536;
        kvs.o_first = kvs.o_send + slot;
        kvs.o_prev = kvs.o_first + slot * (1 + 2 * par);
        kvs.o_rfirst = kvs.o_prev + slot;
        if (u.rank < u.world - 1) UV_RUN(uv_launch_rows_pack(h, C, 0, C, N, B, F, F - 1, (half_t*)(u.comm_ws + kvs.o_send), s));
        if (u.rank == 0) UV_RUN(uv_launch_rows_pack(h, C, 0, C, N, B, F, 0, (half_t*)(u.comm_ws + kvs.o_first), s));
        kvs.emu = !u.native_comm && u.emu_wire_gbps > 0;
        if (!u.native_comm && !kvs.emu) return UV_OK;
        const bool sends = u.rank < u.world - 1 || kvs.emu;
        hipStream_t x = s;
        if (u.kv_overlap && sends) {
            UV_RUN(u.comm_streams());
            x = u.xstream;
            UV_HIP(hipEventRecord(u.ev_fork, s));
            UV_HIP(hipStreamWaitEvent(x, u.ev_fork, 0));
            u.x_dirty = true;
        }
        if (u.native_comm) {
// ... 462 lines not shown
```

Baseline: 5.850 frames/s.

## Compute nearest-2x-upsample 3x3 convs as four 2x2 phase convolutions

Nearest-neighbour upsampling followed by a 3x3 conv is rewritten as four sub-pixel phase convolutions. Each uses a 2x2 kernel built by summing the original 3x3 taps and runs on the source-resolution patch. This cuts the reduction length from 9*C to 4*C per output and avoids reading the upsampled image. The epilogue scatters each phase's rows to interleaved output positions and remaps the GroupNorm statistics. It adds a derived weight copy per upsampler and a stricter eligibility plan, and summing taps in fp16 slightly changes rounding.

```diff
diff --git a/include/univst.h b/include/univst.h
--- a/include/univst.h
+++ b/include/univst.h
@@ -203,6 +203,9 @@
 int univst_conv3x3_patch(const void* X1, const void* X2, int C1, int C2, int imgs, int Hs, int Ws, int upsample, const void* W32,
                          const void* bias, const void* rowbias, int rows_per_rowbias, const void* residual, void* Y, int Cout,
                          void* stream);
+int univst_conv_up2_phase_weights(const void* W_oihw, int Cout, int Cin, void* W4, void* stream);
+int univst_conv3x3_up2_phase(const void* X, int C, int imgs, int Hs, int Ws, const void* W4, const void* bias, void* Y, int Cout, float* gn_out,
+                             int gn_group_width, void* stream);
 int univst_groupnorm_fold_linear(const void* X, int C, int64_t rows, int rows_per_stat, int groups, float eps, const void* gamma, const void* beta,
                                  const void* W, const void* bias, int N, void* W_sets, float* bias32, void* workspace, void* stream);
 int univst_linear_sets(const void* X, int64_t ldx, const void* W_sets, const float* bias32, int rows_per_set, const void* residual, int64_t ldr,
@@ -298,6 +301,7 @@
 #define UNIVST_PLAN_TAPINNER 1024
 #define UNIVST_PLAN_Y_UNALIGNED 2048
 #define UNIVST_PLAN_WORKSPACE 4096
+#define UNIVST_PLAN_W4 8192
 #define UNIVST_PLAN_GEOM_3X3 0
 #define UNIVST_PLAN_GEOM_PAD_END 1
 #define UNIVST_PLAN_GEOM_FRAME 2
diff --git a/univst_amd/_native.py b/univst_amd/_native.py
--- a/univst_amd/_native.py
+++ b/univst_amd/_native.py
@@ -140,6 +140,8 @@
     "univst_conv_nhwc": (_I, [_P, _P, _I, _I, _I, _I, _I, _I, _I, _I, _P, _P, _P, _I, _P, _P, _I, _P]),
     "univst_conv_nhwc_tapinner": (_I, [_P, _P, _I, _I, _I, _I, _I, _I, _I, _P, _P, _P, _I, _P, _P, _I, _P]),
     "univst_conv3x3_patch": (_I, [_P, _P, _I, _I, _I, _I, _I, _I, _P, _P, _P, _I, _P, _P, _I, _P]),
+    "univst_conv_up2_phase_weights": (_I, [_P, _I, _I, _P, _P]),
+    "univst_conv3x3_up2_phase": (_I, [_P, _I, _I, _I, _I, _P, _P, _P, _I, _P, _I, _P]),
     "univst_groupnorm_fold_linear": (_I, [_P, _I, _L, _I, _I, _F, _P, _P, _P, _P, _I, _P, _P, _P, _P]),
     "univst_linear_sets": (_I, [_P, _L, _P, _P, _I, _P, _L, _P, _L, _I, _I, _I, _P, _P]),
     "univst_groupnorm_workspace_bytes": (_L, [_L, _I, _I]),
@@ -375,6 +377,25 @@
     return out
 
 
+def conv_up2_phase_weights(w):
+    _f16(w)
+    Co, Ci = w.shape[:2]
+    w4 = torch.empty(4, Co, Ci // 32, 4, 32, device=w.device, dtype=torch.float16)
+    check(load().univst_conv_up2_phase_weights(ptr(w.contiguous()), Co, Ci, ptr(w4), stream_ptr()), "conv_up2_phase_weights")
+    return w4
+
+
+def conv3x3_up2_phase(x, w4, bias=None, gn_group_width=0):
+    _f16(x), _f16(w4)
+    imgs, Hs, Ws, C_ = x.shape
+    Cout = w4.shape[1]
+    out = torch.empty(imgs, 2 * Hs, 2 * Ws, Cout, device=x.device, dtype=torch.float16)
+    gst = torch.zeros(Cout // gn_group_width, imgs * 4 * Hs * Ws // 16, 2, device=x.device, dtype=torch.float32) if gn_group_width else None
+    check(load().univst_conv3x3_up2_phase(ptr(x), C_, imgs, Hs, Ws, ptr(w4), ptr(bias), ptr(out), Cout, ptr(gst), gn_group_width, stream_ptr()),
+          "conv3x3_up2_phase")
+    return (out, gst) if gn_group_width else out
+
+
 def groupnorm_fold_linear(x, gamma, beta, groups, eps, rows_per_stat, w, bias=None):
     _f16(x), _f16(w)
     rows, C_ = x.shape
diff --git a/univst_amd/csrc/abi.hip b/univst_amd/csrc/abi.hip
--- a/univst_amd/csrc/abi.hip
+++ b/univst_amd/csrc/abi.hip
@@ -594,6 +594,27 @@
     g.R = H(R); g.ldr = Cout; g.Y = HM(Y); g.ldy = Cout;
     return uv_launch_gemm(g, 1, S(s));
 }
+int univst_conv_up2_phase_weights(const void* W_oihw, int Cout, int Cin, void* W4, void* s) {
+    UV_REQUIRE(W_oihw && W4, "conv_up2_phase_weights: null argument");
+    return uv_launch_conv_up2_phase_weights(H(W_oihw), HM(W4), Cout, Cin, S(s));
+}
+int univst_conv3x3_up2_phase(const void* X, int C, int imgs, int Hs, int Ws, const void* W4, const void* bias, void* Y, int Cout, float* gn_out,
+                             int gn_group_width, void* s) {
+    UV_REQUIRE(X && W4 && Y, "conv3x3_up2_phase: null argument");
+    UV_REQUIRE(!gn_out || (gn_group_width > 0 && Cout % gn_group_width == 0), "conv3x3_up2_phase: gn_group_width=%d must divide Cout=%d", gn_group_width, Cout);
+    GemmParams g;
+    g.X = H(X); g.C1 = C; g.Hs = Hs; g.Ws = Ws; g.up = 1; g.stride = 1; g.taps = 9;
+    g.Ho = 2 * Hs; g.Wo = 2 * Ws;
+    g.M = imgs * g.Ho * g.Wo; g.N = Cout; g.K = 9 * C;
+    g.W4 = H(W4); g.bias = H(bias); g.Y = HM(Y); g.ldy = Cout;
+    g.tapw = 3; g.pady = g.padx = 1;
+    int emitted = 0;
+    if (gn_out) { g.gn_out = gn_out; g.gn_gw = gn_group_width; g.gn_G = Cout / gn_group_width; g.gn_emitted = &emitted; }
+    const GemmPlan pl = uv_gemm_plan(g, 1, uv_num_cus());
+    UV_REQUIRE(pl.rc != UV_OK || (pl.phase && (!gn_out || pl.gn_emit)), "conv3x3_up2_phase: the problem does not take the phase form with these statistics "
+               "(C %% 64, Cout %% 320, whole source rows per tile, >= 150 tiles, statistics of 10 / 20 / 40-channel groups)");
+    return uv_launch_gemm(g, 1, S(s));
+}
 int univst_groupnorm_fold_linear(const void* X, int C, int64_t rows, int rows_per_stat, int groups, float eps, const void* gamma, const void* beta,
                                  const void* W, const void* bias, int N, void* W_sets, float* bias32, void* ws, void* s) {
     UV_REQUIRE(X && gamma && beta && W && W_sets && bias32 && ws && N > 0, "groupnorm_fold_linear: null argument");
@@ -699,6 +720,7 @@
     g.X = h; g.Y = on(UNIVST_PLAN_Y_UNALIGNED) ? h + 4 : h;
     g.W = on(UNIVST_PLAN_W32_ONLY) ? nullptr : h;
     g.W32 = on(UNIVST_PLAN_W32_ONLY) || on(UNIVST_PLAN_W32) ? h : nullptr;
+    g.W4 = on(UNIVST_PLAN_W4) ? h : nullptr;
     g.N = N; g.geglu = geglu;
     const int No = geglu ? N / 2 : N;
     if (mode == 0) {
diff --git a/univst_amd/csrc/gemm.hip b/univst_amd/csrc/gemm.hip
--- a/univst_amd/csrc/gemm.hip
+++ b/univst_amd/csrc/gemm.hip
@@ -200,9 +200,10 @@
 }
 constexpr int EPI_LDW = 164;
 constexpr int EPI_STAT_SCRATCH = 90112;
-template <int MJ, int LNF = 0>
+template <int MJ, int LNF = 0, bool PH = false>
 __device__ __forceinline__ void gemm_epilogue_lds(const GemmParams& p, const f4 (&acc)[10][MJ], float* slab, int mw, int nb, int lane,
-                                                  const float* cf, int cn, int rw = 0, float2* scratch = nullptr, half_t* hs = nullptr) {
+                                                  const float* cf, int cn, int rw = 0, float2* scratch = nullptr, half_t* hs = nullptr,
+                                                  int ph = 0, int phw = 1) {
     const int l15 = lane & 15, g = lane >> 4;
     const half_t* hb = reinterpret_cast<const half_t*>(cf + EPC_HALFS) + cn;
 #pragma unroll
@@ -283,7 +284,12 @@
 #pragma unroll
                     for (int r = 0; r < 8; ++r) o[r] = (half_t)v[r];
                 }
-                *reinterpret_cast<h8*>(p.Y + (long)m * p.ldy + n) = o;
+                long mo = m;
+                if constexpr (PH) {
+                    const int r = m / phw;
+                    mo = ((long)(2 * r + (ph >> 1)) * (2 * phw)) + 2 * (m - r * phw) + (ph & 1);
+                }
+                *reinterpret_cast<h8*>(p.Y + mo * p.ldy + n) = o;
                 if (LNF != 1 && p.gn_out) *reinterpret_cast<h8*>(&hs[row * 160 + c]) = o;
                 if (LNF == 1) {
                     float s1 = 0.f, s2 = 0.f;
@@ -339,7 +345,7 @@
                     }
                 }
                 if (l15 == 15 && mrow0 < p.M) {
-                    float2* dst = reinterpret_cast<float2*>(p.gn_out) + (long)(nb / p.gn_gw + g * ngpl) * (p.M >> 4) + (mrow0 >> 4);
+                    float2* dst = reinterpret_cast<float2*>(p.gn_out) + (long)(nb / p.gn_gw + g * ngpl) * (p.M >> 4) + (PH ? 4 * (mrow0 >> 4) + ph : mrow0 >> 4);
 #pragma unroll
                     for (int gi = 0; gi < 4; ++gi)
                         if (gi < ngpl) dst[(long)gi * (p.M >> 4)] = float2{a1[gi], a2[gi]};
@@ -1054,13 +1060,17 @@
     const int l15 = lane & 15, g = lane >> 4;
     const int nt_n = p.N / BNB;
     int lid = xcd_remap(blockIdx.x, gridDim.x);
-    const int ntiles = nt_n * ((p.M + BMB - 1) / BMB);
+    const bool ph4 = p.W4 != nullptr;
+    const int Mg = ph4 ? p.M >> 2 : p.M;
+    const int ntiles = nt_n * ((Mg + BMB - 1) / BMB);
     const int split = lid / ntiles;
     lid -= split * ntiles;
+    const int ph = ph4 ? split : 0;
     const int tn = lid % nt_n, tm = lid / nt_n;
     const int m0 = tm * BMB, n0 = tn * BNB;
-    const int Wd = p.Wo, PW = Wd + 2, Himg = p.Ho;
-    const int rows_total = p.M / Wd;
+    const int up = ph4 ? 0 : p.up;
+    const int Wd = ph4 ? p.Ws : p.Wo, PW = Wd + 2, Himg = ph4 ? p.Hs : p.Ho;
+    const int rows_total = Mg / Wd;
     const int R = BMB / Wd;
     const int gr0 = m0 / Wd;
     const int r0 = gr0 % Himg;
@@ -1085,7 +1095,7 @@
         const int gr = gr0 - r0 + seg * Himg + pos;
         const bool ok = q < npieces && px >= 1 && px <= Wd && pos != Himg && gr < rows_total;
         const int img = gr / Himg, yy = gr - img * Himg;
-        ppix[i] = ok ? (img * p.Hs + (yy >> p.up)) * p.Ws + ((px - 1) >> p.up) : -1;
+        ppix[i] = ok ? (img * p.Hs + (yy >> up)) * p.Ws + ((px - 1) >> up) : -1;
         pch[i] = (cst ^ (((pp >> 2) & 1) << 1)) * 8;
     }
     auto issue_patch = [&](int slab) {
@@ -1101,13 +1111,16 @@
     };
     const int rb = tid >> 3;
     const int kc = (tid & 7) ^ (rb & 7);
+    const int NT = ph4 ? 4 : 9, TW = ph4 ? 2 : 3;
+    const int Kw = ph4 ? 4 * (p.C1 + p.C2) : p.K;
+    const half_t* const Wsrc = ph4 ? p.W4 + (long)ph * p.N * Kw : p.W32;
     unsigned woff[5];
 #pragma unroll
-    for (int i = 0; i < 5; ++i) woff[i] = (unsigned)((long)(n0 + rb + 64 * i) * p.K + kc * 8);
+    for (int i = 0; i < 5; ++i) woff[i] = (unsigned)((long)(n0 + rb + 64 * i) * Kw + kc * 8);
     auto issue_w = [&](int t) {
         half_t* dst = Wb + (t & 1) * WT + wave_u * 8 * LDSH;
 #pragma unroll
-        for (int i = 0; i < 5; ++i) glds16(p.W32 + woff[i] + t * 64, dst + 64 * i * LDSH);
+        for (int i = 0; i < 5; ++i) glds16(Wsrc + woff[i] + t * 64, dst + 64 * i * LDSH);
     };
 
     int pbase[MJ];
@@ -1123,8 +1136,8 @@
     const int s_begin = p.splits > 1 ? split * (p.ktps / 9) * 2 : 0;
     const int s_end = p.splits > 1 ? (s_begin + (p.ktps / 9) * 2 < nslab_all ? s_begin + (p.ktps / 9) * 2 : nslab_all) : nslab_all;
     const int nslab = s_end - s_begin;
-    const int T = nslab * 9 / 2;
-    const int t_off = s_begin * 9 / 2;
+    const int T = nslab * NT / 2;
+    const int t_off = s_begin * NT / 2;
     issue_patch(s_begin);
     if (nslab > 1) issue_patch(s_begin + 1);
     issue_w(t_off);
@@ -1135,11 +1148,12 @@
 #pragma unroll
         for (int j = 0; j < MJ; ++j) acc[i][j] = f4{0.f, 0.f, 0.f, 0.f};
     int next_patch = 2;
-    int u_slab = s_begin, u_tap = 0;
+    const int delta0 = ph4 ? (ph >> 1) * PW + (ph & 1) : 0;
+    int u_slab = s_begin, u_tap = 0, u_kx = 0, u_delta = delta0;
     const int sw = l15 & 7;
     for (int t = 0; t < T; ++t) {
         __syncthreads();
-        if (next_patch < nslab && 9 * (next_patch - 1) <= 2 * t) {
+        if (next_patch < nslab && NT * (next_patch - 1) <= 2 * t) {
             issue_patch(s_begin + next_patch);
             ++next_patch;
         }
@@ -1148,8 +1162,7 @@
         for (int ks = 0; ks < 2; ++ks) {
             if (ks == 1 && t + 1 < T) issue_w(t_off + t + 1);
             const half_t* Ps = Pb + (u_slab & 1) * PBUF;
-            const int ky = u_tap / 3, kx = u_tap - 3 * ky;
-            const int delta = ky * PW + kx;
+            const int delta = u_delta;
             const int ch = ((ks * 4 + g) ^ sw) * 8;
             h8 a[NF];
 #pragma unroll
@@ -1161,7 +1174,9 @@
 #pragma unroll
                 for (int i = 0; i < NF; ++i) acc[i][j] = __builtin_amdgcn_mfma_f32_16x16x32_f16(a[i], b, acc[i][j], 0, 0, 0);
             }
-            if (++u_tap == 9) { u_tap = 0; ++u_slab; }
+            ++u_delta;
+            if (++u_kx == TW) { u_kx = 0; u_delta += PW - TW; }
+            if (++u_tap == NT) { u_tap = 0; u_delta = delta0; ++u_slab; }
         }
     }
     if (p.splits > 1) {
@@ -1173,6 +1188,12 @@
 #pragma unroll
             for (int i = 0; i < NF; ++i) *reinterpret_cast<f4*>(row + i * 16) = acc[i][j];
         }
+        return;
+    }
+    if (ph4) {
+        __syncthreads();
+        gemm_epilogue_lds<MJ, 0, true>(p, acc, reinterpret_cast<float*>(smem) + wave * (16 * EPI_LDW), m0 + wm * 16 * MJ, n0 + wn * 160, lane, epc, wn * 160, 0, nullptr,
+                                       reinterpret_cast<half_t*>(reinterpret_cast<char*>(smem) + EPI_STAT_SCRATCH) + wave * 2560, ph, Wd);
         return;
     }
     if (p.epi_lds) {
@@ -1190,6 +1211,20 @@
     }
 }
 
+
+__global__ void conv_up2_phase_weight_kernel(const half_t* __restrict__ in, half_t* __restrict__ out, int Co, int Ci) {
+    const long i = (long)blockIdx.x * blockDim.x + threadIdx.x;
+    const long per = (long)Co * Ci * 4;
+    if (i >= 4 * per) return;
+    const int j = (int)(i % 32), t = (int)((i / 32) % 4), q = (int)((i / 128) % (Ci / 32)), o = (int)((i / (4L * Ci)) % Co), ph = (int)(i / per);
+    const int a = ph >> 1, b = ph & 1, ti = t >> 1, tj = t & 1;
+    const int y0 = ti == 0 ? 0 : 1 + a, y1 = ti == 0 ? a : 2, x0 = tj == 0 ? 0 : 1 + b, x1 = tj == 0 ? b : 2;
+    const half_t* w = in + ((long)o * Ci + q * 32 + j) * 9;
+    float acc = 0.f;
+    for (int ky = y0; ky <= y1; ++ky)
+        for (int kx = x0; kx <= x1; ++kx) acc += (float)w[ky * 3 + kx];
+    out[i] = (half_t)acc;
+}
 
 __global__ __launch_bounds__(256) void linear_small_kernel(const half_t* __restrict__ x, const half_t* __restrict__ W,
                                                            const half_t* __restrict__ b, half_t* __restrict__ y,
@@ -1267,8 +1302,14 @@
 }
 
 static bool uv_conv_patch_eligible(const GemmParams& p, int bmb) {
-    return p.W32 && p.taps == 9 && p.stride == 1 && p.C1 % 32 == 0 && p.C2 % 32 == 0 && (p.C1 + p.C2) % 64 == 0 && p.N % 320 == 0 && (p.Wo % 16 == 0 || 16 % p.Wo == 0) &&
+    return (p.W32 || p.W4) && p.taps == 9 && p.stride == 1 && p.C1 % 32 == 0 && p.C2 % 32 == 0 && (p.C1 + p.C2) % 64 == 0 && p.N % 320 == 0 && (p.Wo % 16 == 0 || 16 % p.Wo == 0) &&
            bmb % p.Wo == 0 && (bmb / p.Wo + 2 + bmb / p.Wo / p.Ho + 1) * (p.Wo + 2) <= 512 && !p.geglu;
+}
+
+static bool uv_conv_patch_phase_eligible(const GemmParams& p, int bmb) {
+    return p.W4 && p.up == 1 && p.taps == 9 && p.stride == 1 && p.C2 == 0 && p.C1 % 64 == 0 && p.N % 320 == 0 && p.Ho == 2 * p.Hs && p.Wo == 2 * p.Ws &&
+           (p.Ws % 16 == 0 || 16 % p.Ws == 0) && bmb % p.Ws == 0 && (p.Hs * p.Ws) % 16 == 0 &&
+           (bmb / p.Ws + 2 + bmb / p.Ws / p.Hs + 1) * (p.Ws + 2) <= 512 && (p.M / 4) % bmb == 0 && !p.R && !p.rowbias && !p.bias2 && !p.bias32 && !p.geglu;
 }
 
 constexpr long BIG_MIN_TILES = 150;
@@ -1383,7 +1424,7 @@
         PLAN_REQUIRE(p.K == p.taps * (p.C1 + p.C2), "conv: K=%d != taps*(C1+C2)", p.K);
         const bool sym3 = p.taps == 9 && p.pady == 1 && p.padx == 1;
         PLAN_REQUIRE(!p.korder || (sym3 && p.C1 % 64 == 0 && p.C2 % 64 == 0), "conv: tap-inner k order needs the 3x3 / padding-1 kernel and 64-channel slabs");
-        PLAN_REQUIRE(!p.W32 || sym3, "conv: the LDS-patch weight copy is for the 3x3 / padding-1 kernel");
+        PLAN_REQUIRE((!p.W32 && !p.W4) || sym3, "conv: the LDS-patch weight copy is for the 3x3 / padding-1 kernel");
     }
     uv_gemm_bytes(p, mode, &pl.bytes, &pl.aux_bytes);
     const int nk = (p.K + 63) / 64;
@@ -1411,7 +1452,9 @@
         if (sp >= 2 && nblk * sp >= 128) bsplits = sp;
     }
     const bool fills = nblk >= BIG_MIN_TILES || bsplits > 1;
-    const bool use_patch = mode == 1 && fills && uv_conv_patch_eligible(p, use192 ? 192 : 256);
+    const bool patch_ok = mode == 1 && fills && uv_conv_patch_eligible(p, use192 ? 192 : 256);
+    const bool try_phase = patch_ok && bsplits <= 1 && uv_conv_patch_phase_eligible(p, use192 ? 192 : 256);
+    const bool use_patch = patch_ok && (p.W32 || try_phase);
     PLAN_REQUIRE(p.W || use_patch, "conv: only the [Cin/32][9][32] weight copy was given but the problem is not eligible for the LDS-patch kernel "
                  "(3x3, stride 1, whole image rows per 256/192-row tile, >= 150 tiles or a reduction long enough for split-K)");
     if (fills && big_shape_ok(p.N, p.K, xmax, ragged, conv_rag ? 256 : 640)) {
@@ -1439,6 +1482,8 @@
                          (!p.stats_out || (!p.geglu && p.N % 160 == 0)), "linear: LayerNorm fold on a problem the direct 256x320 path does not take");
             PLAN_REQUIRE(!(p.ln_stats && p.stats_out), "linear: a LayerNorm-folded linear cannot also emit row statistics");
         }
+        pl.phase = try_phase && pl.epi_lds == 1 && pl.splits == 1;
+        PLAN_REQUIRE(!use_patch || p.W32 || pl.phase, "conv: only the phase weight copy was given but the launch cannot take the phase form (16-byte aligned Y / bias rows)");
         pl.cls = mode == 0 ? UV_CLS_GEMM_BIG : (use_patch ? UV_CLS_CONV_PATCH : UV_CLS_CONV_BIG);
         pl.prof_sym = true;
         if (use_patch) snprintf(pl.sym, sizeof pl.sym, "conv_patch_kernel<%d>", mj);
@@ -1498,6 +1543,7 @@
     q.tile_gm = pl.tile_gm;
     if (!pl.gn_emit) q.gn_out = nullptr;
     else if (q.gn_emitted) *q.gn_emitted = 1;
+    if (!pl.phase) q.W4 = nullptr;
     const bool own_ws = pl.ws_bytes && !(q.partial && q.partial_bytes >= pl.ws_bytes);
     if (own_ws) UV_HIP(hipMallocAsync((void**)&q.partial, pl.ws_bytes, stream));
     uv_prof_begin(pl.cls, pl.flops, pl.bytes, stream, pl.prof_sym ? pl.sym : nullptr, pl.aux_bytes);
@@ -1528,6 +1574,13 @@
     return UV_OK;
 }
 
+int uv_launch_conv_up2_phase_weights(const half_t* w_oihw, half_t* w4, int Co, int Ci, hipStream_t stream) {
+    UV_REQUIRE(w_oihw && w4 && Co > 0 && Ci > 0 && Ci % 32 == 0, "conv_up2_phase_weights: needs Cin %% 32 == 0 (Co=%d Ci=%d)", Co, Ci);
+    hipLaunchKernelGGL(conv_up2_phase_weight_kernel, dim3((unsigned)(((long)Co * Ci * 16 + 255) / 256)), dim3(256), 0, stream, w_oihw, w4, Co, Ci);
+    UV_LAUNCH_CHECK();
+    return UV_OK;
+}
+
 int uv_launch_linear_small(const half_t* x, const half_t* W, const half_t* b, half_t* y, int M, int N, int K,
                            int silu_in, hipStream_t stream) {
     UV_REQUIRE(M >= 1 && M <= 8, "linear_small: M=%d must be in 1..8", M);
diff --git a/univst_amd/csrc/kernels.h b/univst_amd/csrc/kernels.h
--- a/univst_amd/csrc/kernels.h
+++ b/univst_amd/csrc/kernels.h
@@ -42,6 +42,7 @@
     float ln_eps = 0.f;
     const float* ln_wsum = nullptr;
     const float* ln_bias = nullptr;
+    const half_t* W4 = nullptr;
 };
 
 struct AttnParams {
@@ -113,6 +114,7 @@
     bool prof_sym = false;
     int splits = 1, ktps = 0, epi_lds = 0, tile_gn = 0, tile_gm = 0;
     bool gn_emit = false;
+    bool phase = false;
     size_t ws_bytes = 0;
     unsigned reduce_grid = 0;
 };
@@ -126,6 +128,7 @@
 
 int uv_num_cus();
 int uv_launch_gemm(const GemmParams& p, int mode, hipStream_t stream);
+int uv_launch_conv_up2_phase_weights(const half_t* w_oihw, half_t* w4, int Co, int Ci, hipStream_t stream);
 bool uv_linear_takes_big_direct(long M, int N, int K, long ldx = 0);
 bool uv_linear_fold_producer_ok(long M, int N, int K);
 bool uv_linear_fold_consumer_ok(long M, int N, int K, bool geglu);
diff --git a/univst_amd/csrc/unet.hip b/univst_amd/csrc/unet.hip
--- a/univst_amd/csrc/unet.hip
+++ b/univst_amd/csrc/unet.hip
@@ -231,6 +231,11 @@
                 half_t* d3;
                 UV_RUN(derive(k + "#t32", {Co, Ci / 32, 9, 32}, &d3));
                 hipLaunchKernelGGL(permute_conv_weight_t32_kernel, dim3(nb((long)Co * Ci * 9)), dim3(256), 0, s, t.ptr, d3, Co, Ci);
+                if (k.find("upsamplers") != std::string::npos) {
+                    half_t* d4;
+                    UV_RUN(derive(k + "#ph4", {4, Co, Ci / 32, 4, 32}, &d4));
+                    UV_RUN(uv_launch_conv_up2_phase_weights(t.ptr, d4, Co, Ci, s));
+                }
             }
         } else if (ends(k, ".attn1.to_q.weight")) {
             std::string p = k.substr(0, k.size() - strlen("to_q.weight"));
@@ -532,6 +537,7 @@
         g.korder = (taps == 9 && g.C1 % 64 == 0 && g.C2 % 64 == 0 && u.find(p + ".weight#ti")) ? 1 : 0;
         g.W = W(p + (g.korder ? ".weight#ti" : ".weight#nhwc"));
         if (taps == 9 && stride == 1 && u.find(p + ".weight#t32")) g.W32 = W(p + ".weight#t32");
+        if (taps == 9 && stride == 1 && up == 1 && !b && u.find(p + ".weight#ph4")) g.W4 = W(p + ".weight#ph4");
         g.bias = W(p + ".bias");
         g.rowbias = rowbias;
         g.ldrb = ldrb;
```

After: 5.982 frames/s, median of 6. 1.02x the previous value.
